# tpy001/VFMSeg

Hardware: AMD Instinct MI355X
Metric: train images/sec @512x512 DINOv2-L+LoRA (dg_lora_dinov2_ms_masked, 1024^2 sample = LR+HR 512^2 passes) (higher is better)
Workload: dtype bf16; 1 GPU; configs[1]: dg_lora_dinov2_ms_masked.py, synthetic 1024^2 19-class samples -> 2x512^2 passes, bs=2/GPU, full train step (fwd+bwd+allreduce+AdamW), LoRA dropout on; global_batch=2, parallelism=dp1

## Files before the change

include/vfmseg_hip.h:

```cpp
#ifndef VFMSEG_HIP_H
#define VFMSEG_HIP_H
#include <stdint.h>

#ifdef __cplusplus
extern "C" {
#endif

enum { VFM_F32 = 0, VFM_BF16 = 1, VFM_U8 = 2, VFM_I64 = 3,
       VFM_SPLIT3 = 4  };
enum { VFM_OK = 0, VFM_E_INVAL = -1, VFM_E_SHAPE = -2, VFM_E_ALIGN = -3, VFM_E_HIP = -4, VFM_E_UNSUPPORTED = -5 };
enum { VFM_EP_NONE = 0, VFM_EP_GELU = 1, VFM_EP_RELU = 2, VFM_EP_MUL_GELU_GRAD = 3, VFM_EP_MUL = 4,
       VFM_EP_QGELU = 5 , VFM_EP_MUL_QGELU_GRAD = 6,
       VFM_EP_GELU_DGELU = 7  };
enum { VFM_ACT_NONE = 0, VFM_ACT_GELU = 1, VFM_ACT_RELU = 2, VFM_ACT_QGELU = 3 };

const char* vfm_last_error(void);
int vfm_abi_version(void);
int vfm_half_kind(void);

int vfm_cast(const void* src, int src_dt, long ld_src, void* dst, int dst_dt, long ld_dst, long rows, long cols,
             const float* colscale, void* stream);
int vfm_split3(const float* src, long stride_r, long stride_c, void* dst, long ld_dst, long rows, long K, int pattern, void* stream);
int vfm_transpose(const void* src, int src_dt, long ld_src, void* dst, int dst_dt, long ld_dst, long rows, long cols,
                  long pad_rows, void* stream);
int vfm_strided_copy(const void* src, int src_dt, void* dst, int dst_dt, long n0, long n1, long n2, long n3, long s0,
                     long s1, long s2, long s3, long d0, long d1, long d2, long d3, int accumulate, void* stream);
typedef struct vfm_copy_job {
  const float* src; void* dst; long dst_dt; long accumulate;
  long n[4], s[4], d[4];
  long nsum, sum_stride;
} vfm_copy_job;
int vfm_strided_copy_batch(const vfm_copy_job* table_dev, int njobs, long max_elems, void* stream);
int vfm_axpby(const float* x, float a, float* y, float b, long n, void* stream);
int vfm_scale_by_device_scalar(float* y, const float* scalar, long n, void* stream);
int vfm_colsum(const void* x, int dt, long ld, long rows, long cols, float* out, int accumulate, float* ws, void* stream);
typedef struct vfm_lora_site {
  const float* A; const float* B;
  void* a; void* at; void* w; void* wt;
  long r, K, N, Kw, ld_a, ld_at, ld_w, ld_wt;
} vfm_lora_site;
int vfm_lora_pack(const vfm_lora_site* table_dev, int nsites, long max_elems, int dt, void* stream);
int vfm_slab_reduce(const float* slabs, int kch, long P, long Q, long rows_used, float alpha, float* dst, long sp, long sq,
                    int accumulate, void* stream);
int vfm_dropout_mask(void* out, int dt, long n, float p, uint64_t seed, uint64_t offset, void* stream);
int vfm_mul_mask(const void* src, int src_dt, long ld_src, const void* mask, int mask_dt, long mask_ld,
                 long rows_per_group, void* dst, int dst_dt, long ld_dst, long rows, long cols, void* stream);
int vfm_geglu_fwd(const void* h, int h_dt, long ld_h, void* out, int out_dt, long ld_out, long rows, long C, void* stream);
int vfm_geglu_bwd(const void* h, int h_dt, long ld_h, const void* dout, int do_dt, long ld_do, void* dh, int dh_dt,
                  long ld_dh, long rows, long C, void* stream);
int vfm_swiglu_fwd(const void* h, int h_dt, long ld_h, void* out, int out_dt, long ld_out, long rows, long C, void* stream);
int vfm_swiglu_bwd(const void* h, int h_dt, long ld_h, const void* dout, int do_dt, long ld_do, void* dh, int dh_dt,
                   long ld_dh, long rows, long C, void* stream);
int vfm_rope(void* x, int dt, long ld, long rows, int np, int ncols, int d, const float* cos_t, const float* sin_t,
             int inverse, void* stream);
int vfm_act_grad_mul(const void* dy, int dy_dt, long ld_dy, const void* pre, int pre_dt, long ld_pre, void* out, int out_dt,
                     long ld_out, long rows, long cols, int act, void* stream);
int vfm_mask_token_fwd(const float* x, const uint8_t* keep, const float* token, float* out, long rows, long C, void* stream);
int vfm_mask_token_bwd(const float* dout, const uint8_t* keep, float* dx, float* dtoken, float* ws ,
                       long rows, long C, void* stream);

int vfm_layernorm_fwd(const float* x, long ld_x, const float* w, const float* b, float eps, void* y, int y_dt, long ld_y,
                      float* stats, long rows, long C, void* stream);
int vfm_layernorm_fwd_split3(const float* x, long ld_x, const float* w, const float* b, float eps, float* y, long ld_y, void* y3, long ld3,
                             long plane, float* stats, long rows, long C, void* stream);
int vfm_layernorm_dropout_fwd(const float* x, long ld_x, const float* w, const float* b, float eps, void* y, long ld_y,
                              float* stats, void* y_drop, long ld_yd, void* mask, long ld_mask, float p, uint64_t seed,
                              uint64_t offset, long rows, long C, void* stream);
int vfm_layernorm_bwd_scaled(const void* dy, int dy_dt, long ld_dy, const float* x, long ld_x, const float* w,
                             const float* stats, float* dx, long ld_dx, int accumulate_dx, void* t_out, long ld_t,
                             const float* t_scale, long rows, long C, void* stream);
int vfm_layernorm_bwd(const void* dy, int dy_dt, long ld_dy, const float* x, long ld_x, const float* w,
                      const float* stats, float* dx, long ld_dx, int accumulate_dx, float* dw, float* db, float* ws,
                      long rows, long C, void* stream);
int vfm_groupnorm_fwd(const float* x, const float* w, const float* b, float eps, int G, int act, void* y, int y_dt,
                      float* stats, float* ws, long B, long P, long C, void* stream);
int vfm_groupnorm_bwd(const void* dy, int dy_dt, const float* x, const float* w, const float* b, const float* stats,
                      int G, int act, float* dx, float* dw, float* db, float* ws, long B, long P, long C, void* stream);
int vfm_bn_moments(const float* x, long rows, long C, float* sums, float* ws, void* stream);
int vfm_bn_finalize(const float* sums, float count, float* mean_var, float* running_mean, float* running_var,
                    float momentum, long C, void* stream);
int vfm_bn_apply(const float* x, const float* mean_var, const float* w, const float* b, float eps, int act, void* y,
                 int y_dt, long rows, long C, void* stream);
int vfm_bn_bwd_reduce(const void* dy, int dy_dt, const float* x, const float* mean_var, const float* w, const float* b,
                      float eps, int act, float* sums_dy, float* ws, long rows, long C, void* stream);
int vfm_bn_bwd_apply(const void* dy, int dy_dt, const float* x, const float* mean_var, const float* w, const float* b,
                     float eps, int act, const float* sums_dy, float total_rows, float* dx, long rows, long C,
                     void* stream);

typedef struct vfm_gemm_desc {
  const void* A; const void* B; void* C;
  int in_dt; int c_dt;
  long M, N, K;
  long sa_m, sa_k, sb_n, sb_k, ldc;
  float alpha;
  const float* bias; long bias_mod;
  const float* colscale;
  const void* residual; int r_dt; long ldr;
  int ep_mode; const void* aux; int aux_dt; long ld_aux;
  void* C2; int c2_dt; long ldc2;
  long batch, stride_a, stride_b, stride_c;
  long c_plane;
  long kb_rows;
} vfm_gemm_desc;
int vfm_gemm(const vfm_gemm_desc* d, void* stream);
int vfm_tune(const char* key, int value);

typedef struct vfm_attn_desc {
  const void* q; const void* k; const void* v; void* o;
  int dt; long ldq, ldk, ldv, ldo;
  int B, H, d;
  int nq_main, nq_extra, nk_main, nk_extra;
  float scale;
  float* lse;
  const void* dout; long ld_do;
  void* dq; void* dk; void* dv; long ld_dq, ld_dk, ld_dv;
  float* delta;
} vfm_attn_desc;
int vfm_attn_fwd(const vfm_attn_desc* d, void* stream);
int vfm_attn_bwd(const vfm_attn_desc* d, void* stream);
int vfm_attn_fwd_x3(const vfm_attn_desc* d, long lo_off, void* stream);
int vfm_attn_fwd_x3_split(const vfm_attn_desc* d, long lo_off, void* o3, long ld3, long plane, void* stream);
int vfm_attn_bwd_x3(const vfm_attn_desc* d, const void* q3, const void* k3, const void* v3, long ld3, long lo_off, const void* do3,
                    long ld_do3, long lo_off_do3, void* stream);

int vfm_sam_relpos_table(const float* rel_pos, int L, int d, int S, float* out, void* stream);
int vfm_sam_attn_prep(const void* qkv, int dt, long ld, const float* bias, const float* rh, const float* rw, void* q_aug,
                      void* k_aug, void* v_win, int nimg, int G, int S, int H, int d, int Dq, int NP,
                      int rows_per_batch , float scale, void* stream);
int vfm_softmax_rows(const float* scores, long ld_s, void* out, int out_dt, long ld_o, long rows, int n, int npad, void* stream);
int vfm_sam_attn_merge(const void* o_win, int dt, void* out, long ld, int nimg, int G, int S, int H, int d, int NP, void* stream);
int vfm_sam_attn_bwd_prep(const void* dao, long ld_dao, const void* qkv, long ld_qkv, const float* bias, int dt, void* dow,
                          void* dowT, void* vp, void* qsT, int nimg, int G, int S, int H, int d, int dp, int NP, float scale,
                          void* stream);
int vfm_softmax_rows_batched(const float* scores, long ld_s, void* out, int out_dt, long ld_o, long rows, int n, int npad,
                             int rows_per_batch, int valid_rows, void* stream);
int vfm_softmax_rows_bwd(const void* p, const float* dp, long ld_dp, void* ds, int dt, long ld_p, long rows, int n, int npad,
                         int rows_per_batch, int valid_rows, void* stream);
int vfm_sam_attn_bwd_merge(const void* dqa, const void* dkT, const void* dvT, int dt, const float* rh, const float* rw, void* dqkv,
                           long ld, int nimg, int G, int S, int H, int d, int dp, int NP, int Dq, float scale, void* stream);

int vfm_rein_mix_fwd(const float* x, long ld_x, const void* t, const void* vt, void* u, long ld_u, void* p, long ld_p, void* x16,
                     long ld_x16, long rows, int D, int m, float c, void* stream);
int vfm_rein_mix_bwd(const void* du, long ld_du, const void* p, long ld_p, const void* v, const void* tt, void* ds, long ld_ds,
                     float* dx, long ld_dx, long rows, int D, int m, float c, void* stream);

int vfm_sam_attn_flash_fwd(const void* qkv, long ld, const float* bias, const void* tbl_h, const void* tbl_w, void* out, long ldo,
                           int nimg, int G, int S, int H, int d, float scale, void* stream);
int vfm_sam_attn_flash_fwd_train(const void* qkv, long ld, const float* bias, const void* tbl_h, const void* tbl_w, void* out, long ldo,
                                 int nimg, int G, int S, int H, int d, float scale, float* lse, void* qext, void* stream);
long vfm_sam_attn_flash_stat_rows(int nimg, int G, int S, int H);
int vfm_sam_attn_flash_bwd(const void* qkv, long ld, const float* bias, const void* tbl_h, const void* tbl_w, const void* out,
                           const void* dout, long ldo, const float* lse, const void* qext, float* dsum, void* dqkv, long ldg,
                           int nimg, int G, int S, int H, int d, float scale, void* stream);

int vfm_patchify(const float* img, long stride_b, long stride_c, long stride_y, int y0, int x0, int h, int w, int P,
                 void* out, int out_dt, long ld_out, int B, void* stream);
int vfm_assemble_tokens(const float* patch_tok, const float* cls, const float* pos, float* x, int B, int np, int C,
                        void* stream);

int vfm_resize_bilinear(const void* in, int in_dt, int in_nchw, int B, int Hi, int Wi, int C, long in_ld_c, void* out,
                        int out_dt, int out_mode, long out_ld_c, int Hv, int Wv, int y0, int x0, int hc, int wc,
                        float scale_y, float scale_x, void* stream);
int vfm_resize_bicubic(const float* in, int Hi, int Wi, int C, float* out, int Ho, int Wo, float scale_y, float scale_x,
                       void* stream);
int vfm_label_resize(const int64_t* in, int B, int Hi, int Wi, int64_t* out, int Hv, int Wv, int y0, int x0, int hc,
                     int wc, void* stream);
int vfm_unblock(const float* x, float* y, int B, int H, int W, int C, int levels, int inverse, void* stream);
int vfm_upsample_ce(const float* logits_low, const int64_t* label, int B, int h, int w, int C, int H, int W,
                    int ignore_index, float* loss_parts, int32_t* counts, float* dlogits, void* stream);
int vfm_ce_finish(const float* loss_parts, long n, float scale, int32_t* counts, float eps, float* loss, float* acc, void* stream);
int vfm_reduce_sum(const float* x, long n, float scale, float* out, void* stream);

int vfm_preprocess_u8(const uint8_t* img, int H, int W, float* out, int Hp, int Wp, const float* mean3, const float* std3,
                      int bgr_to_rgb, float pad_val, void* stream);
int vfm_conf_gate(const float* logits, int B, int C, int H, int W, int y0, int x0, int hc, int wc, float thr,
                  int32_t* count, void* stream);
int vfm_slide_accumulate(const float* crop, int crop_nchw, int B, int h, int w, int C, float* preds, float* count,
                         int H, int W, int y0, int x0, int hc, int wc, void* stream);
typedef struct vfm_slide_win {
  const float* crop;
  int nchw, h, w;
  int y0, x0, hc, wc;
} vfm_slide_win;
int vfm_slide_gather(const vfm_slide_win* wins, int nwin, int B, int C, float* preds, int H, int W, void* stream);
int vfm_conf_gate_windows(const float* logits, int B, int C, int H, int W, const int* boxes, int nwin, float thr, int32_t* counts,
                          void* stream);
int vfm_slide_finalize(float* preds, const float* count, uint8_t* argmax, int B, int C, int H, int W, void* stream);

int vfm_confusion_hist(const uint8_t* pred, const void* label, int label_dt, long n, int num_classes, int ignore_index,
                       int64_t* hist, void* stream);

int vfm_adamw(float* p, float* g, float* m, float* v, long n, const long* seg_start, const float* seg_lr_mult,
              const float* seg_wd, int n_seg, float lr, float beta1, float beta2, float eps, int step, float grad_scale,
              int zero_grad, int vec4, void* stream);
int vfm_adamw_guarded(float* p, float* g, float* m, float* v, long n, const long* seg_start, const float* seg_lr_mult,
                      const float* seg_wd, int n_seg, float lr, float beta1, float beta2, float eps, int step, float grad_scale,
                      int zero_grad, int vec4, const int* skip, const float* amp_state, void* stream);
int vfm_amp_update(const int* flag, float* amp_state, float growth, float backoff, int interval, int dynamic, void* stream);

enum { VFM_OP_GEMM = 0, VFM_OP_LN_FWD = 1, VFM_OP_LN_DROPOUT_FWD = 2, VFM_OP_LN_BWD_SCALED = 3, VFM_OP_ATTN_FWD = 4, VFM_OP_ATTN_BWD = 5,
       VFM_OP_CAST = 6, VFM_OP_STRIDED_COPY = 7 };
enum { VFM_PROF_NONE = 0, VFM_PROF_GEMM = 1, VFM_PROF_GEMM_TN = 2, VFM_PROF_ATTN_FWD = 3, VFM_PROF_ATTN_BWD = 4 };
typedef struct vfm_plan_op {
  int kind;
  int prof_kind;
  double flops;
  union {
    vfm_gemm_desc gemm;
    vfm_attn_desc attn;
    struct { const float* x; long ld_x; const float* w; const float* b; float eps; void* y; int y_dt; long ld_y; float* stats;
             long rows, C; } ln_fwd;
    struct { const float* x; long ld_x; const float* w; const float* b; float eps; void* y; long ld_y; float* stats; void* y_drop;
             long ld_yd; void* mask; long ld_mask; float p; uint64_t offset; long rows, C; } ln_drop;
    struct { const void* dy; int dy_dt; long ld_dy; const float* x; long ld_x; const float* w; const float* stats; float* dx;
             long ld_dx; int accumulate_dx; void* t_out; long ld_t; const float* t_scale; long rows, C; } ln_bwd;
    struct { const void* src; int src_dt; long ld_src; void* dst; int dst_dt; long ld_dst; long rows, cols; const float* colscale; } cast;
    struct { const void* src; int src_dt; void* dst; int dst_dt; long n[4]; long ss[4]; long ds[4]; int accumulate; } copy;
  } u;
} vfm_plan_op;
int vfm_run_plan(const vfm_plan_op* ops, int n, uint64_t seed, uint64_t rng_base, void* stream);
int vfm_prof_config(int every);
int vfm_prof_read(double* out, int cap);

#ifdef __cplusplus
}
#endif
#endif
```

vfmseg_amd/backbones.py:

```python
import math

import os

import torch
import torch.nn as nn

from .precision import is_half
from . import ops
from .precision import compute_dtype
from .registry import MODELS

R_PAD = 64

BACKWARD_EVENTS = {"heads_done": None, "block_done": None, "backbone_done": None}
_PENDING_BACKWARD = [0]


class _Lin(nn.Module):
    def __init__(self, i, o, bias=True):
        super().__init__()
        self.in_features, self.out_features = i, o
        self.weight = nn.Parameter(torch.empty(o, i))
        self.bias = nn.Parameter(torch.zeros(o)) if bias else None
        nn.init.trunc_normal_(self.weight, std=0.02)
# ... 171 lines not shown
                raise NotImplementedError(f"init_cfg type {init_cfg.get('type')!r}: only dict(type='Pretrained', checkpoint=...) is read")
            self.load_pretrained_base(ck)

    def load_pretrained_base(self, checkpoint):
        sd = torch.load(checkpoint, map_location="cpu") if isinstance(checkpoint, (str, os.PathLike)) else checkpoint
        sd = sd.get("state_dict", sd) if isinstance(sd, dict) else sd
        missing, _ = self.load_state_dict(sd, strict=False)
        missing = [k for k in missing if not k.startswith("reins.")]
        if missing:
            raise RuntimeError(f"pretrained backbone {checkpoint if isinstance(checkpoint, (str, os.PathLike)) else '<state dict>'}: "
                               f"{len(missing)} base parameters not found (first: {missing[:3]}; the file holds e.g. {list(sd)[:3]})")
        self.pretrained = checkpoint if isinstance(checkpoint, (str, os.PathLike)) else "<state dict>"
        self.engine().invalidate()

    def train(self, mode=True):
        nn.Module.train(self, False)
        self._rein_train = bool(mode)
        if mode:
            for n, p in self.named_parameters():
                p.requires_grad = "reins" in n
            for p in self.reins.inert_params():
                p.requires_grad = False
            self.reins.train(True)
        return self

    def adapter_training(self):
        return self._rein_train

    def state_dict(self, *args, destination=None, prefix="", keep_vars=False):
        if args:
            args = list(args) + [None] * (3 - len(args))
            destination, prefix, keep_vars = args[0], args[1] or "", bool(args[2])
        state = super().state_dict(destination=destination, prefix=prefix, keep_vars=keep_vars)
        for k in [k for k in state.keys() if k.startswith(prefix) and "rein" not in k[len(prefix):]]:
            state.pop(k)
        return state

    def forward(self, x):
        xcat, (hp, wp) = self.forward_tokens([(x, None)], training=self._rein_train)
        b, d = x.shape[0], self.embed_dim
        v = xcat.view(b, hp, wp, len(self.out_indices), d)
        return tuple(v[:, :, :, i].permute(0, 3, 1, 2) for i in range(len(self.out_indices)))


class _Holder(nn.Module):
    def __init__(self, m):
        super().__init__()
        self.model = m


class _PeftModel(nn.Module):
    def __init__(self, m):
        super().__init__()
        self.base_model = _Holder(m)


@MODELS.register_module()
class LoRABackbone(nn.Module):

    def __init__(self, backbone, checkpoint=None, Lora_config=None, init_cfg=None, **kw):
        super().__init__()
        vit = MODELS.build(backbone)
        cfg = Lora_config or {}
        self.lora_targets = list(cfg.get("target_modules", ["qkv"]))
        for name, mod in list(vit.named_modules()):
            if isinstance(mod, _Lin) and any(name == t or name.endswith("." + t) for t in self.lora_targets):
                parent = vit
                parts = name.split(".")
                for p_ in parts[:-1]:
                    parent = getattr(parent, p_)
                setattr(parent, parts[-1], LoraLinear(mod, cfg.get("r", 32), cfg.get("lora_alpha", 32), cfg.get("lora_dropout", 0.0)))
        if not vit.engine().lora_on():
            raise NotImplementedError(f"target_modules={self.lora_targets}: no adapter site the {type(vit).__name__} HIP engine fuses")
        self.model = _PeftModel(vit)
        self._lora_train = False
        if checkpoint is not None:
            self.load_pretrained_backbone(checkpoint, self.lora_targets)
        self.train(True)

    @property
    def vit(self):
        return self.model.base_model.model

    def load_pretrained_backbone(self, checkpoint, target_modules):
        sd = torch.load(checkpoint, map_location="cpu") if isinstance(checkpoint, str) else checkpoint
        new = {}
        for name, w in sd.items():
            for t in target_modules:
                if t in name:
                    name = name.replace(t, t + ".base_layer")
            new[name] = w
        self.vit.load_state_dict(new, strict=False)
        self.vit.engine().invalidate()

    def train(self, mode=True):
        super().train(False)
        self._lora_train = bool(mode)
        for n, p in self.named_parameters():
            p.requires_grad = ("lora" in n) if mode else p.requires_grad
        if mode:
            for p in getattr(self.vit.engine(), "inert_params", lambda: [])():
                p.requires_grad = False
        return self

    def forward_tokens(self, jobs, seed=None):
        return self.vit.forward_tokens(jobs, training=self._lora_train, seed=seed)

    def forward(self, x):
        xcat, (hp, wp) = self.forward_tokens([(x, None)])
        b, d, nt = x.shape[0], self.vit.embed_dim, len(self.vit.out_indices)
        v = xcat.view(b, hp, wp, nt, d)
        return tuple(v[:, :, :, i].permute(0, 3, 1, 2) for i in range(nt))


class Packed:

    def __init__(self, w_f32, cd, k_pad=None):
        n, k = w_f32.shape
        k_pad = k_pad or k
        self.n, self.k = n, k_pad
        self.w = ops.empty_ld(n, k_pad, cd, w_f32.device, zero=True)
        ops.cast(w_f32, self.w[:, :k])
        self.wt = None
        if is_half(cd):
            self.wt = ops.empty_ld(k_pad, n, cd, w_f32.device, zero=True)
            ops.transpose(w_f32, self.wt[:k], pad_rows=n)

    def fwd(self, a, out, **epi):
        return ops.gemm(a, self.w, out, **epi)

    def dgrad(self, dy, out, **epi):
        if self.wt is not None:
            return ops.gemm(dy, self.wt, out, **epi)
        return ops.gemm(dy, self.w, out, trans_b=True, **epi)


def wgrad(dy, x, grad_out, alpha=1.0, n_rows=None, accumulate=True):
    M = dy.shape[0]
    res = grad_out if accumulate else None
    if is_half(dy.dtype):
        mp = (M + 63) // 64 * 64
        dyt = torch.empty(dy.shape[1], mp, dtype=dy.dtype, device=dy.device)
        xt = torch.empty(x.shape[1], mp, dtype=x.dtype, device=x.device)
        ops.transpose(dy, dyt, pad_rows=mp)
        ops.transpose(x, xt, pad_rows=mp)
        ops.gemm(dyt, xt, grad_out, alpha=alpha, residual=res)
    else:
        ops.gemm(dy, x, grad_out, alpha=alpha, residual=res, trans_a=True, trans_b=True)
    return grad_out


class _DinoTrainPlan:

    def __init__(self, eng, P, nimg, Np):
        v = eng.vit
        cd, dev = P["cd"], P["dev"]
        D, H = v.embed_dim, v.num_heads
        nL = len(v.blocks)
        M, Mp = nimg * Np + nimg, nimg * Np
        Lp0 = P["layers"][0]
        kq, hid = Lp0["qkv"].k, Lp0["fc1"].n
        q0 = v.blocks[0].attn.qkv
        self.eng, self.P, self.nimg, self.Np, self.M, self.Mp, self.nL, self.D, self.H = eng, P, nimg, Np, M, Mp, nL, D, H
        self.busy = False
        e = lambda *sh, dt=cd: torch.empty(*sh, dtype=dt, device=dev)
        f32 = torch.float32
        self.X = e(nL + 1, M, D, dt=f32)
        self.A1, self.XD, self.MASK = e(nL, M, kq), e(nL, M, D), e(nL, M, D)
        self.ST1, self.ST2 = e(nL, M, 2, dt=f32), e(nL, M, 2, dt=f32)
        self.QKV, self.AO = e(nL, M, 3 * D), e(nL, M, D)
        self.LSE = e(nL, nimg, H, Np + 1, dt=f32)
        self.XMID, self.A2 = e(nL, M, D, dt=f32), e(nL, M, D)
        hld = hid + ops.ld_pad(hid, cd)
        self.HPRE = e(nL, M, hld)[:, :, :hid]
        self.G = e(M, hld)[:, :hid]
        self.hid, self.kq = hid, kq
        hd = D // H
        scale = hd ** -0.5
        f = self.fwd = ops.Plan("backbone")
        self.tap_ops = []
        self.nt = len(v.out_indices)
        xcat0 = e(Mp, self.nt * D)
        for li, (blk, Lp) in enumerate(zip(v.blocks, P["layers"])):
            q = blk.attn.qkv
            x, a1 = self.X[li], self.A1[li]
            f.layernorm_dropout_fwd(x, Lp["n1w"], Lp["n1b"], 1e-6, a1[:, :D], self.ST1[li], self.XD[li], self.MASK[li], q.p, li * M * D)
            f.gemm(self.XD[li], Lp["a"], a1[:, D:D + R_PAD], alpha=q.scaling)
            f.gemm(a1, Lp["qkv"].w, self.QKV[li], bias=Lp["qkv_b"])
            qkv = self.QKV[li]
            f.attn_fwd(qkv[:, :D], qkv[:, D:2 * D], qkv[:, 2 * D:], self.AO[li], self.LSE[li], nimg, H, hd, Np, 1, Np, 1, scale)
            f.gemm(self.AO[li], Lp["proj"].w, self.XMID[li], bias=Lp["proj_b"], colscale=Lp["g1"], residual=x)
            f.layernorm_fwd(self.XMID[li], Lp["n2w"], Lp["n2b"], 1e-6, self.A2[li], self.ST2[li])
            f.gemm(self.A2[li], Lp["fc1"].w, self.G, bias=Lp["fc1_b"], ep_mode=ops.EP_GELU_DGELU, c2=self.HPRE[li])
            f.gemm(self.G, Lp["fc2"].w, self.X[li + 1], bias=Lp["fc2_b"], colscale=Lp["g2"], residual=self.XMID[li])
            for i, oi in enumerate(v.out_indices):
                if oi == li:
                    self.tap_ops.append((f.cast(self.X[li + 1][:Mp], xcat0[:, i * D:(i + 1) * D]), i * D))
        self.bwd = None

    def eligible_backward(self):
        from .functional import direct_grad_target
        v = self.eng.vit
        return (os.environ.get("VFMSEG_LORA_WGRAD_BATCHED", "1") != "0" and
                all(direct_grad_target(b.attn.qkv.lora_A["default"].weight) is not None and
                    direct_grad_target(b.attn.qkv.lora_B["default"].weight) is not None for b in v.blocks))

    def run_forward(self, xcat, seed, rng0):
        esz = xcat.element_size()
        for idx, col in self.tap_ops:
            self.fwd.entry(idx).u.cast.dst = xcat.data_ptr() + col * esz
        self.fwd.run(seed, rng0)

    def _build_backward(self, dxcat):
        v, P = self.eng.vit, self.P
        cd, dev = P["cd"], P["dev"]
        D, H, nL, M, Mp, nimg, Np = self.D, self.H, self.nL, self.M, self.Mp, self.nimg, self.Np
        hd = D // H
        scale = hd ** -0.5
        e = lambda *sh, dt=cd: torch.empty(*sh, dtype=dt, device=dev)
        self.DX = e(M, D, dt=torch.float32)
        self.T, self.DN, self.DAO = e(M, D), e(M, D), e(M, D)
        self.DH = e(M, self.hid + ops.ld_pad(self.hid, cd))[:, :self.hid]
        self.DQKV, self.DA1 = e(nL, M, 3 * D), e(nL, M, self.kq)
        half = nL // 2
        skip_l0 = os.environ.get("VFMSEG_PLAN_SKIP_L0", "1") != "0"
        self.half = half
        self.dx_sig = (tuple(dxcat.shape), tuple(dxcat.stride()), dxcat.dtype)
        plans, self.tap_src = [], []

        def add_tap(pl, pn, li):
            for i, oi in enumerate(v.out_indices):
                if oi == li:
                    src = dxcat[:, i * D:(i + 1) * D]
                    self.tap_src.append((pn, pl.strided_copy(src, self.DX, (Mp, D), (src.stride(0), 1), (D, 1), accumulate=True), i * D))

        for pn, (hi, lo) in enumerate(((nL, half), (half, 0)) if half > 0 else ((nL, 0),)):
            pl = ops.Plan("backbone")
            for li in range(hi - 1, lo - 1, -1):
                blk, Lp = v.blocks[li], P["layers"][li]
                q = blk.attn.qkv
                if li == nL - 1:
                    add_tap(pl, pn, li)
                    pl.cast(self.DX, self.T, Lp["g2"])
                pl.gemm(self.T, Lp["fc2"].wt, self.DH, ep_mode=ops.EP_MUL, aux=self.HPRE[li])
                pl.gemm(self.DH, Lp["fc1"].wt, self.DN)
                pl.layernorm_bwd_scaled(self.DN, self.XMID[li], Lp["n2w"], self.ST2[li], self.DX, self.T, Lp["g1"], accumulate_dx=True)
                pl.gemm(self.T, Lp["proj"].wt, self.DAO)
                qkv, dqkv, da1 = self.QKV[li], self.DQKV[li], self.DA1[li]
                pl.attn_bwd(qkv[:, :D], qkv[:, D:2 * D], qkv[:, 2 * D:], self.AO[li], self.LSE[li], self.DAO, dqkv[:, :D], dqkv[:, D:2 * D],
                            dqkv[:, 2 * D:], nimg, H, hd, Np, 1, Np, 1, scale)
                if li == 0 and skip_l0:
                    pl.gemm(dqkv, Lp["qkv"].wt[D:D + R_PAD], da1[:, D:D + R_PAD])
                    continue
                pl.gemm(dqkv, Lp["qkv"].wt, da1)
                pl.gemm(da1[:, D:D + R_PAD], Lp["at"], da1[:, :D], alpha=q.scaling, residual=da1[:, :D], ep_mode=ops.EP_MUL, aux=self.MASK[li])
                if li > 0:
                    add_tap(pl, pn, li - 1)
                    pl.layernorm_bwd_scaled(da1[:, :D], self.X[li], Lp["n1w"], self.ST1[li], self.DX, self.T, P["layers"][li - 1]["g2"],
                                            accumulate_dx=True)
                else:
                    pl.layernorm_bwd_scaled(da1[:, :D], self.X[li], Lp["n1w"], self.ST1[li], self.DX, self.T, Lp["g2"], accumulate_dx=True)
            plans.append((pl, lo, hi))
        self.bwd = plans

    def run_backward(self, ctx, dxcat):
        sig = (tuple(dxcat.shape), tuple(dxcat.stride()), dxcat.dtype)
        if self.bwd is None or self.dx_sig != sig:
            self._build_backward(dxcat)
        esz = dxcat.element_size()
        for pn, idx, col in self.tap_src:
            self.bwd[pn][0].entry(idx).u.copy.src = dxcat.data_ptr() + col * esz
        self.DX.zero_()
        for pl, lo, hi in self.bwd:
            pl.run()
            self.eng._lora_wgrads_batched(self.P, ctx, self.DA1, self.DQKV, lo, hi, self.M, self.D)
            if BACKWARD_EVENTS["block_done"] is not None:
                for lj in range(hi - 1, lo - 1, -1):
                    BACKWARD_EVENTS["block_done"](lj)


class DinoEngine:
    def __init__(self, vit):
        self.vit = vit
        self._packed = None
        self._pos_cache = {}

    def invalidate(self):
        self._packed = None
        self._pos_cache = {}

    def lora_on(self):
        return isinstance(self.vit.blocks[0].attn.qkv, LoraLinear)

    def rein_on(self):
        return getattr(self.vit, "reins", None) is not None

    def trainable(self):
        out = []
        if self.lora_on():
            for blk in self.vit.blocks:
                out += [blk.attn.qkv.lora_A["default"].weight, blk.attn.qkv.lora_B["default"].weight]
        if self.rein_on():
            out += self.vit.reins.live_params()
        return out

    def packed(self):
        cd = compute_dtype()
        dev = self.vit.pos_embed.device
        if self._packed is not None and self._packed["cd"] == cd and self._packed["dev"] == dev:
            return self._packed
        v = self.vit
        D = v.embed_dim
        P = dict(cd=cd, dev=dev, layers=[])
        with torch.no_grad():
            pw = v.patch_embed.proj.weight.detach().reshape(D, -1)
            P["pe"] = Packed(pw, cd)
            P["pe_b"] = v.patch_embed.proj.bias.detach().float().contiguous()
            P["cls"] = v.cls_token.detach().reshape(D).float().contiguous()
            for blk in v.blocks:
                qkv = blk.attn.qkv
                base = qkv.base_layer if isinstance(qkv, LoraLinear) else qkv
                kq = D + (R_PAD if isinstance(qkv, LoraLinear) else 0)
                Lp = dict(
                    qkv=Packed(base.weight.detach(), cd, k_pad=kq),
                    qkv_b=base.bias.detach().float().contiguous() if base.bias is not None else None,
                    proj=Packed(blk.attn.proj.weight.detach(), cd),
                    proj_b=blk.attn.proj.bias.detach().float().contiguous() if blk.attn.proj.bias is not None else None,
                    fc1=Packed(blk.mlp.fc1.weight.detach(), cd),
                    fc1_b=blk.mlp.fc1.bias.detach().float().contiguous() if blk.mlp.fc1.bias is not None else None,
                    fc2=Packed(blk.mlp.fc2.weight.detach(), cd),
                    fc2_b=blk.mlp.fc2.bias.detach().float().contiguous() if blk.mlp.fc2.bias is not None else None,
                    g1=blk.ls1.gamma.detach().float().contiguous(), g2=blk.ls2.gamma.detach().float().contiguous(),
                    n1w=blk.norm1.weight.detach().float().contiguous(), n1b=blk.norm1.bias.detach().float().contiguous(),
                    n2w=blk.norm2.weight.detach().float().contiguous(), n2b=blk.norm2.bias.detach().float().contiguous(),
                )
                if isinstance(qkv, LoraLinear):
                    Lp["a"] = torch.zeros(R_PAD, D, dtype=cd, device=dev)
                    Lp["at"] = torch.zeros(D, R_PAD, dtype=cd, device=dev)
                P["layers"].append(Lp)
        self._packed = P
        return P

    def refresh_lora(self, P):
        D = self.vit.embed_dim
        sites = []
        for blk, Lp in zip(self.vit.blocks, P["layers"]):
            q = blk.attn.qkv
            if isinstance(q, LoraLinear):
                A, Bm = q.lora_A["default"].weight.detach(), q.lora_B["default"].weight.detach()
                sites.append((A, Bm, Lp["a"], Lp["at"], Lp["qkv"].w, Lp["qkv"].wt, q.r, A.shape[1], Bm.shape[0], D))
        _refresh_sites(P, sites)

    def merged_qkv(self, P):
        from .optim import PARAM_EPOCH
        key = [PARAM_EPOCH[0]]
        for blk in self.vit.blocks:
            q = blk.attn.qkv
            A, Bm = q.lora_A["default"].weight, q.lora_B["default"].weight
            key += [A._version, Bm._version, A.data_ptr(), Bm.data_ptr()]
        key = tuple(key)
        if P.get("merged_key") == key:
            return P["merged"]
        D, cd, dev = self.vit.embed_dim, P["cd"], P["dev"]
        merged = []
        with torch.no_grad():
            for blk in self.vit.blocks:
                q = blk.attn.qkv
                A, Bm = q.lora_A["default"].weight.detach().float(), q.lora_B["default"].weight.detach().float()
                w = q.base_layer.weight.detach().float()
                weff = torch.empty_like(w)
                ops.gemm(Bm.contiguous(), A.contiguous(), weff, alpha=q.scaling, residual=w, trans_b=True)
                wp = ops.empty_ld(w.shape[0], D, cd, dev)
                ops.cast(weff, wp)
                merged.append(wp)
        P["merged"], P["merged_key"] = merged, key
        return merged

    def pos_tokens(self, hp, wp):
        v = self.vit
        n = v.pos_embed.shape[1] - 1
        s = int(math.sqrt(n))
        if hp == s and wp == s:
            return v.pos_embed.detach().reshape(n + 1, -1).float().contiguous()
        key = (hp, wp)
        if key not in self._pos_cache:
            D = v.embed_dim
            pe = v.pos_embed.detach().reshape(n + 1, D).float().contiguous()
            out = torch.empty(1 + hp * wp, D, dtype=torch.float32, device=pe.device)
            ops.cast(pe[:1], out[:1])
            sy, sx = s / (hp + 0.1), s / (wp + 0.1)
            assert int(s * ((hp + 0.1) / s)) == hp and int(s * ((wp + 0.1) / s)) == wp
            ops.resize_bicubic(pe[1:], s, s, D, out[1:], hp, wp, sy, sx)
            self._pos_cache[key] = out
        return self._pos_cache[key]

    def forward(self, jobs, training, seed, need_grad=False):
        v, P = self.vit, self.packed()
        cd = P["cd"]
        dev = P["dev"]
        D, H, ps = v.embed_dim, v.num_heads, v.patch_size
        lora = self.lora_on()
        rein = self._rein_pack(P) if self.rein_on() else None
        merged = None
        from .precision import split3 as _x3_mode
        x3 = _x3_mode() and not is_half(cd)
        if (lora and not training and not torch.is_grad_enabled() and (is_half(cd) or x3)
                and os.environ.get("VFMSEG_MERGE_LORA_EVAL", "1") != "0"):
            merged = self.merged_qkv(P)
        elif lora:
            self.refresh_lora(P)
        sizes = []
        for img, box in jobs:
            y0, y1, x0, x1 = box if box is not None else (0, img.shape[2], 0, img.shape[3])
            sizes.append(((y1 - y0) // ps, (x1 - x0) // ps))
        hp, wp = sizes[0]
        assert all(s == (hp, wp) for s in sizes), "all jobs of one backbone call must share the token grid"
        Np = hp * wp
        nimg = sum(j[0].shape[0] for j in jobs)
        Mp, M = nimg * Np, nimg * Np + nimg
        kpe = 3 * ps * ps
        A0 = torch.empty(Mp, kpe, dtype=cd, device=dev)
        r0 = 0
        for img, box in jobs:
            b = img.shape[0]
            ops.patchify(img, A0[r0 * Np:(r0 + b) * Np], box=box, patch=ps)
            r0 += b
        ptok = torch.empty(Mp, D, dtype=torch.float32, device=dev)
        P["pe"].fwd(A0, ptok, bias=P["pe_b"])
        plan = self._train_plan(P, nimg, Np, training, merged) if need_grad else None
        x = plan.X[0] if plan is not None else torch.empty(M, D, dtype=torch.float32, device=dev)
        ops.assemble_tokens(ptok, P["cls"], self.pos_tokens(hp, wp), x, nimg, Np, D)
        del ptok, A0
        nt = len(v.out_indices)
        from .precision import eval_heads_fp32
        tap_dt = torch.float32 if (not training and not need_grad and eval_heads_fp32()) else cd
        xcat = torch.empty(Mp, nt * D, dtype=tap_dt, device=dev)
        saved = []
        if lora and training:
            from .functional import draw_seed
            seed, rng0 = draw_seed(seed, len(v.blocks) * M * D)
        else:
            seed, rng0 = 0, 0
        if plan is not None:
            plan.run_forward(xcat, seed, rng0)
            plan.busy = True
            ctx = dict(saved=None, plan=plan, nimg=nimg, Np=Np, M=M, Mp=Mp, P=P, training=training, A1all=plan.A1, XDall=plan.XD)
            return xcat, (hp, wp), ctx
        nL = len(v.blocks)
        batched = lora and training and is_half(cd) and merged is None
        A1all = torch.empty(nL, M, P["layers"][0]["qkv"].k, dtype=cd, device=dev) if batched else None
        XDall = None
        hd = D // H
        scale = hd ** -0.5
        for li, (blk, Lp) in enumerate(zip(v.blocks, P["layers"])):
            S = {"x_in": x}
            kq = D if merged is not None else Lp["qkv"].k
            a1 = A1all[li] if batched else torch.empty(M, kq, dtype=cd, device=dev)
            st1 = torch.empty(M, 2, dtype=torch.float32, device=dev)
            q = blk.attn.qkv if lora else None
            fused_drop = lora and training and q.p > 0 and is_half(cd) and D % 256 == 0
            if fused_drop:
                mask = torch.empty(M, D, dtype=cd, device=dev)
                if batched and XDall is None:
                    XDall = torch.empty(nL, M, D, dtype=cd, device=dev)
                xd = XDall[li] if batched else torch.empty(M, D, dtype=cd, device=dev)
                ops.layernorm_dropout_fwd(x, Lp["n1w"], Lp["n1b"], 1e-6, a1[:, :D], st1, xd, mask, q.p, seed, offset=rng0 + li * M * D)
            else:
                so = "only" if (x3 and not training and not need_grad and kq == D) else None
                ops.layernorm_fwd(x, Lp["n1w"], Lp["n1b"], 1e-6, a1 if kq == D else a1[:, :D], st1, split_out=so)
            if lora and merged is None:
                if not fused_drop:
                    xd, mask = a1[:, :D], None
                    if training and q.p > 0:
                        mask = torch.empty(M, D, dtype=cd, device=dev)
                        ops.dropout_mask(mask, q.p, seed, offset=rng0 + li * M * D)
                        xd = torch.empty(M, D, dtype=cd, device=dev)
                        ops.mul_mask(a1[:, :D], mask, xd)
                ops.gemm(xd, Lp["a"], a1[:, D:D + R_PAD], alpha=q.scaling)
                S.update(xd=xd if mask is not None else None, mask=mask)
            qkv = torch.empty(M, 3 * D, dtype=cd, device=dev)
            if merged is not None:
                ops.gemm(a1, merged[li], qkv, bias=Lp["qkv_b"])
            else:
                Lp["qkv"].fwd(a1, qkv, bias=Lp["qkv_b"])
            ao = torch.empty(M, D, dtype=cd, device=dev)
            lse = torch.empty(nimg, H, Np + 1, dtype=torch.float32, device=dev)
            so = "only" if (x3 and not training and not need_grad) else None
            ops.attn_fwd(qkv[:, :D], qkv[:, D:2 * D], qkv[:, 2 * D:], ao, lse, nimg, H, hd, Np, 1, Np, 1, scale, keep_split=training, o_split=so)
            xm = torch.empty(M, D, dtype=torch.float32, device=dev)
            Lp["proj"].fwd(ao, xm, bias=Lp["proj_b"], colscale=Lp["g1"], residual=x)
            a2 = torch.empty(M, D, dtype=cd, device=dev)
            st2 = torch.empty(M, 2, dtype=torch.float32, device=dev)
            ops.layernorm_fwd(xm, Lp["n2w"], Lp["n2b"], 1e-6, a2, st2, split_out=so)
            hid = Lp["fc1"].n
            g = ops.empty_ld(M, hid, cd, dev)
            if training and (lora or (rein is not None and need_grad)):
                hpre = torch.empty(M, hid, dtype=cd, device=dev)
                Lp["fc1"].fwd(a2, g, bias=Lp["fc1_b"], ep_mode=ops.EP_GELU_DGELU, c2=hpre)
            else:
                hpre = None
                Lp["fc1"].fwd(a2, g, bias=Lp["fc1_b"], ep_mode=ops.EP_GELU, **({"c_split": so} if so else {}))
            xo = torch.empty(M, D, dtype=torch.float32, device=dev)
            Lp["fc2"].fwd(g, xo, bias=Lp["fc2_b"], colscale=Lp["g2"], residual=xm)
            S.update(a1=a1, st1=st1, qkv=qkv, ao=ao, lse=lse, x_mid=xm, a2=a2, st2=st2, hpre=hpre, g=g)
            saved.append(S)
            x = xo
            if rein is not None:
                x = self._rein_forward(rein, li, x, Mp, S if (training and need_grad) else None)
            for i, oi in enumerate(v.out_indices):
                if oi == li:
                    ops.cast(x[:Mp], xcat[:, i * D:(i + 1) * D])
        ctx = dict(saved=saved, nimg=nimg, Np=Np, M=M, Mp=Mp, P=P, training=training, A1all=A1all, XDall=XDall, rein=rein)
        return xcat, (hp, wp), ctx

    def _train_plan(self, P, nimg, Np, training, merged):
        v = self.vit
        if (not training or merged is not None or not self.lora_on() or self.rein_on() or not is_half(P["cd"])
                or os.environ.get("VFMSEG_PLAN", "1") == "0" or v.embed_dim % 256 != 0):
            return None
        q0 = v.blocks[0].attn.qkv
        if not all(isinstance(b.attn.qkv, LoraLinear) and b.attn.qkv.p > 0 and b.attn.qkv.p == q0.p and b.attn.qkv.scaling == q0.scaling
                   for b in v.blocks):
            return None
        plans = P.setdefault("plans", {})
        pl = plans.get((nimg, Np))
        if pl is None:
            pl = plans[(nimg, Np)] = _DinoTrainPlan(self, P, nimg, Np)
        if pl.busy or not pl.eligible_backward():
            return None
        return pl

    def backward(self, ctx, dxcat):
        if ctx.get("plan") is not None:
            plan = ctx["plan"]
            try:
                plan.run_backward(ctx, dxcat)
            finally:
                plan.busy = False
            return [None] * (2 * len(self.vit.blocks))
        v, P = self.vit, ctx["P"]
        cd, dev = P["cd"], P["dev"]
        D, H = v.embed_dim, v.num_heads
        hd = D // H
        scale = hd ** -0.5
        M, Mp, nimg, Np = ctx["M"], ctx["Mp"], ctx["nimg"], ctx["Np"]
        dx = torch.zeros(M, D, dtype=torch.float32, device=dev)
        grads = [None] * (2 * len(v.blocks) if self.lora_on() else 0)
        nL = len(v.blocks)
        rein = ctx.get("rein")
        rein_acc = self._rein_backward_begin(rein) if rein is not None else None
        from .functional import direct_grad_target
        wg_batched = (ctx.get("A1all") is not None and self.lora_on() and os.environ.get("VFMSEG_LORA_WGRAD_BATCHED", "1") != "0" and
                      all(direct_grad_target(b.attn.qkv.lora_A["default"].weight) is not None and
                          direct_grad_target(b.attn.qkv.lora_B["default"].weight) is not None for b in v.blocks) and
                      (ctx.get("XDall") is not None or all(S_["mask"] is None for S_ in ctx["saved"])))
        if wg_batched:
            kq_all = ctx["A1all"].shape[2]
            DA1all = torch.empty(nL, M, kq_all, dtype=cd, device=dev)
            DQKVall = torch.empty(nL, M, 3 * D, dtype=cd, device=dev)
        half = nL // 2
        fuse_t = is_half(cd) and D % 256 == 0
        fuse_t1 = fuse_t and rein is None
        def add_tap(li):
            for i, oi in enumerate(v.out_indices):
                if oi == li:
                    src = dxcat[:, i * D:(i + 1) * D]
                    ops.strided_copy(src, dx, (Mp, D), (src.stride(0), 1), (D, 1), accumulate=True)
        t = None
        for li in range(len(v.blocks) - 1, -1, -1):
            blk, Lp, S = v.blocks[li], P["layers"][li], ctx["saved"][li]
            q = blk.attn.qkv
            if t is None:
                add_tap(li)
                if rein is not None:
                    self._rein_backward(rein, rein_acc, li, dx, Mp, S)
                t = torch.empty(M, D, dtype=cd, device=dev)
                ops.cast(dx, t, Lp["g2"])
            hid = Lp["fc1"].n
            dh = ops.empty_ld(M, hid, cd, dev)
            Lp["fc2"].dgrad(t, dh, ep_mode=ops.EP_MUL, aux=S["hpre"])
            dn = torch.empty(M, D, dtype=cd, device=dev)
            Lp["fc1"].dgrad(dh, dn)
            if fuse_t:
                ops.layernorm_bwd_scaled(dn, S["x_mid"], Lp["n2w"], S["st2"], dx, t, Lp["g1"], accumulate_dx=True)
            else:
                ops.layernorm_bwd(dn, S["x_mid"], Lp["n2w"], S["st2"], dx, accumulate_dx=True)
                ops.cast(dx, t, Lp["g1"])
            del dh
            dao = torch.empty(M, D, dtype=cd, device=dev)
            Lp["proj"].dgrad(t, dao)
            dqkv = DQKVall[li] if wg_batched else torch.empty(M, 3 * D, dtype=cd, device=dev)
            qkv = S["qkv"]
            ops.attn_bwd(qkv[:, :D], qkv[:, D:2 * D], qkv[:, 2 * D:], S["ao"], S["lse"], dao, dqkv[:, :D], dqkv[:, D:2 * D],
                         dqkv[:, 2 * D:], nimg, H, hd, Np, 1, Np, 1, scale)
            kq = Lp["qkv"].k
            da1 = DA1all[li] if wg_batched else torch.empty(M, kq, dtype=cd, device=dev)
            Lp["qkv"].dgrad(dqkv, da1)
            if isinstance(q, LoraLinear) and wg_batched:
                ep = dict(ep_mode=ops.EP_MUL, aux=S["mask"]) if S["mask"] is not None else {}
                ops.gemm(da1[:, D:D + R_PAD], Lp["at"], da1[:, :D], alpha=q.scaling, residual=da1[:, :D], **ep)
            elif isinstance(q, LoraLinear):
                r = q.r
                A, Bm = q.lora_A["default"].weight, q.lora_B["default"].weight
                a1 = S["a1"]
                xd = S["xd"] if S["xd"] is not None else a1[:, :D]
                from .functional import direct_grad_target
                tB, tA = direct_grad_target(Bm), direct_grad_target(A)
                gBt = torch.empty(R_PAD, Bm.shape[0], dtype=torch.float32, device=dev)
                gAp = torch.empty(R_PAD, A.shape[1], dtype=torch.float32, device=dev)
                doneB = _wgrad_small_t(a1[:, D:D + R_PAD], dqkv, gBt, scatter=None if tB is None else (tB, r, 1, r))
                doneA = _wgrad_small_t(da1[:, D:D + R_PAD], xd, gAp, alpha=q.scaling,
                                       scatter=None if tA is None else (tA, r, A.shape[1], 1))
                if doneB is True:
                    pass
                elif tB is not None:
                    ops.strided_copy(gBt, tB, (Bm.shape[0], r), (1, gBt.stride(0)), (r, 1), accumulate=True)
                else:
                    gB = torch.empty_like(Bm, dtype=torch.float32)
                    ops.strided_copy(gBt, gB, (Bm.shape[0], r), (1, gBt.stride(0)), (r, 1))
                    grads[2 * li + 1] = gB
                if doneA is True:
                    pass
                elif tA is not None:
                    ops.axpby(gAp[:r].reshape(-1), 1.0, tA.view(-1), 1.0)
                else:
                    grads[2 * li] = gAp[:r]
                ep = dict(ep_mode=ops.EP_MUL, aux=S["mask"]) if S["mask"] is not None else {}
                ops.gemm(da1[:, D:D + R_PAD], Lp["at"], da1[:, :D], alpha=q.scaling, residual=da1[:, :D], **ep)
            if fuse_t1 and li > 0:
                add_tap(li - 1)
                ops.layernorm_bwd_scaled(da1[:, :D], S["x_in"], Lp["n1w"], S["st1"], dx, t, P["layers"][li - 1]["g2"],
                                         accumulate_dx=True)
            else:
                ops.layernorm_bwd(da1[:, :D], S["x_in"], Lp["n1w"], S["st1"], dx, accumulate_dx=True)
                t = None
            ctx["saved"][li] = None
            if wg_batched:
                if li == half or li == 0:
                    lo, hi = (half, nL) if li == half and half > 0 else (0, half if half > 0 else nL)
                    self._lora_wgrads_batched(P, ctx, DA1all, DQKVall, lo, hi, M, D)
                    if BACKWARD_EVENTS["block_done"] is not None:
                        for lj in range(hi - 1, lo - 1, -1):
                            BACKWARD_EVENTS["block_done"](lj)
            elif BACKWARD_EVENTS["block_done"] is not None:
                BACKWARD_EVENTS["block_done"](li)
        if rein is not None:
            grads += self._rein_backward_end(rein, rein_acc)
        return grads

    def _rein_fused(self, P):
        r = self.vit.reins
        return (is_half(P["cd"]) and os.environ.get("VFMSEG_REIN_FUSED", "0") == "1" and self.vit.embed_dim % 256 == 0
                and r.token_length <= ops.REIN_TOK)

    def _rein_pack(self, P):
        from .optim import PARAM_EPOCH
        r = self.vit.reins
        cd, dev = P["cd"], P["dev"]
        D, nL, m = self.vit.embed_dim, r.num_layers, r.token_length
        live = r.live_params()
        key = (PARAM_EPOCH[0], self._rein_fused(P)) + tuple(x for p_ in live for x in (p_._version, p_.data_ptr()))
        R = P.get("rein")
        if R is not None and R["key"] == key:
            return R
        TP = (max(m, ops.REIN_TOK) + 63) // 64 * 64
        if R is None or R["TP"] != TP:
            z = lambda *sh, dt=cd: torch.zeros(*sh, dtype=dt, device=dev)
            R = P["rein"] = dict(TP=TP, T32=z(nL, TP, D, dt=torch.float32), T=z(nL, TP, D), V=z(nL, TP, D), TT=None, VT=None,
                                 scalevec=torch.empty(D, dtype=torch.float32, device=dev))
        R["key"], R["m"], R["c"], R["fused"] = key, m, float(D) ** -0.5, self._rein_fused(P)
        with torch.no_grad():
            T32 = R["T32"]
            toks = [p_.detach() for p_ in r.token_params()]
            if len(toks) == 2:
                ops.gemm(toks[0], toks[1], T32[:, :m], trans_b=True)
            else:
                ops.strided_copy(toks[0], T32, (nL, m, D), (m * D, D, 1), (TP * D, D, 1))
            if cd != torch.float32:
                ops.cast(T32.view(nL * TP, D), R["T"].view(nL * TP, D))
            else:
                R["T"] = T32
            Wt, Wd = r.mlp_token2feat, r.mlp_delta_f
            R["wt"], R["wd"] = Packed(Wt.weight.detach(), cd), Packed(Wd.weight.detach(), cd)
            R["bt"], R["bd"] = Wt.bias.detach(), Wd.bias.detach()
            vtmp = torch.empty(nL * TP, D, dtype=torch.float32, device=dev)
            R["wt"].fwd(R["T"].view(nL * TP, D), vtmp, bias=R["bt"])
            vt3 = vtmp.view(nL, TP, D)
            ops.strided_copy(vt3[:, 1:m], R["V"][:, 1:m], (nL, m - 1, D), (TP * D, D, 1), (TP * D, D, 1))
            if R["fused"]:
                if R["TT"] is None:
                    R["TT"], R["VT"] = torch.zeros(nL, D, TP, dtype=cd, device=dev), torch.zeros(nL, D, TP, dtype=cd, device=dev)
                ops.strided_copy(T32, R["TT"], (nL, D, m), (TP * D, 1, D), (D * TP, TP, 1))
                ops.strided_copy(vt3[:, 1:m], R["VT"][:, :, 1:m], (nL, D, m - 1), (TP * D, 1, D), (D * TP, TP, 1))
            ops.strided_copy(r.scale.detach().reshape(1), R["scalevec"], (D,), (0,), (1,))
        return R

    def _rein_forward(self, R, li, x, Mp, S):
        cd, dev = R["T"].dtype, x.device
        D, m, TP = x.shape[1], R["m"], R["TP"]
        xp = x[:Mp]
        u = torch.empty(Mp, D, dtype=cd, device=dev)
        p = torch.empty(Mp, TP, dtype=cd, device=dev) if S is not None else None
        x16 = None
        if R["fused"]:
            x16 = torch.empty(Mp, D, dtype=cd, device=dev) if S is not None else None
            ops.rein_mix_fwd(xp, R["T"][li], R["VT"][li], u, m, R["c"], p=p, x16=x16)
        else:
            if cd != torch.float32:
                x16 = torch.empty(Mp, D, dtype=cd, device=dev)
                ops.cast(xp, x16)
            sc = torch.empty(Mp, TP, dtype=torch.float32, device=dev)
            ops.gemm(x16 if x16 is not None else xp, R["T"][li], sc, alpha=R["c"])
            if p is None:
                p = torch.empty(Mp, TP, dtype=cd, device=dev)
            ops.softmax_rows(sc, p, m)
            ops.gemm(p, R["V"][li], u, residual=xp, trans_b=True)
        if S is None:
            xn = x
        else:
            xn = torch.empty_like(x)
            ops.cast(x[Mp:], xn[Mp:])
            S.update(rein_u=u, rein_p=p, rein_x=x16 if x16 is not None else xp)
        R["wd"].fwd(u, xn[:Mp], bias=R["bd"], colscale=R["scalevec"], residual=xp)
        return xn

    def _rein_backward_begin(self, R):
        dev = R["T"].device
        nL, TP, D = R["T"].shape
        z = lambda *sh: torch.zeros(*sh, dtype=torch.float32, device=dev)
        return dict(dT=z(nL, TP, D), dV=z(nL, TP, D), Gm=z(D, D), gb=z(D))

    @staticmethod
    def _tn(xs, y, out, alpha=1.0, accumulate=False):
        if is_half(xs.dtype):
            ops.gemm_tn_batched(xs.unsqueeze(0), y.unsqueeze(0), out.unsqueeze(0), xs.shape[0], alpha=alpha, accumulate=accumulate)
        else:
            ops.gemm(xs, y, out, alpha=alpha, residual=out if accumulate else None, trans_a=True, trans_b=True)

    def _rein_backward(self, R, acc, li, dx, Mp, S):
        cd, dev = R["T"].dtype, dx.device
        D, m, TP, c = dx.shape[1], R["m"], R["TP"], R["c"]
        u, p, xs = S["rein_u"], S["rein_p"], S["rein_x"]
        g = torch.empty(Mp, D, dtype=cd, device=dev)
        ops.cast(dx[:Mp], g)
        self._tn(g, u, acc["Gm"], accumulate=True)
        ops.colsum(g, acc["gb"], accumulate=True)
        du = torch.empty(Mp, D, dtype=cd, device=dev)
        R["wd"].dgrad(g, du, colscale=R["scalevec"])
        ds = torch.empty(Mp, TP, dtype=cd, device=dev)
        if R["fused"]:
            ops.rein_mix_bwd(du, p, R["V"][li], R["TT"][li], ds, dx[:Mp], m, c)
            a = 1.0
        else:
            dp = torch.empty(Mp, TP, dtype=torch.float32, device=dev)
            ops.gemm(du, R["V"][li], dp)
            ops.softmax_rows_bwd(p, dp, ds, m, 1, 1)
            ops.gemm(ds, R["T"][li], dx[:Mp], alpha=c, residual=dx[:Mp], trans_b=True)
            ops.strided_copy(du, dx[:Mp], (Mp, D), (du.stride(0), 1), (dx.stride(0), 1), accumulate=True)
            a = c
        self._tn(ds, xs, acc["dT"][li], alpha=a)
        self._tn(p, du, acc["dV"][li])
        S["rein_u"] = S["rein_p"] = S["rein_x"] = None

    def _rein_backward_end(self, R, acc):
        from .functional import direct_grad_target
        r = self.vit.reins
        cd, dev = R["T"].dtype, R["T"].device
        nL, TP, D = R["T"].shape
        m = R["m"]
        z = lambda *sh, dt=torch.float32: torch.zeros(*sh, dtype=dt, device=dev)
        dvz = z(nL, TP, D, dt=cd)
        ops.strided_copy(acc["dV"][:, 1:m], dvz[:, 1:m], (nL, m - 1, D), (TP * D, D, 1), (TP * D, D, 1))
        dvz2, T2 = dvz.view(nL * TP, D), R["T"].view(nL * TP, D)
        gWt, gbt = z(D, D), z(D)
        self._tn(dvz2, T2, gWt)
        ops.colsum(dvz2, gbt)
        back = torch.empty(nL * TP, D, dtype=torch.float32, device=dev)
        R["wt"].dgrad(dvz2, back)
        dT = acc["dT"]
        ops.strided_copy(back.view(nL, TP, D)[:, 1:m], dT[:, 1:m], (nL, m - 1, D), (TP * D, D, 1), (TP * D, D, 1), accumulate=True)
        toks = r.token_params()
        if len(toks) == 2:
# ... 168 lines not shown
```

vfmseg_amd/csrc/elementwise.hip:

```cpp
#include "common.h"

thread_local char g_vfm_err[512] = {0};

extern "C" const char* vfm_last_error(void) { return g_vfm_err; }
extern "C" int vfm_abi_version(void) { return 4; }
extern "C" int vfm_half_kind(void) { return VFM_HALF_KIND; }

template <typename TI, typename TO>
__global__ void k_cast(const TI* __restrict__ src, long ld_src, TO* __restrict__ dst, long ld_dst, long rows, long cols,
                       const float* __restrict__ colscale) {
  const long cols4 = cols >> 2;
  const long total = rows * cols4;
  for (long i = blockIdx.x * (long)blockDim.x + threadIdx.x; i < total; i += (long)gridDim.x * blockDim.x) {
    const long r = i / cols4, c = (i - r * cols4) << 2;
    float v[4];
#pragma unroll
    for (int j = 0; j < 4; ++j) v[j] = ld_f32(src + r * ld_src + c + j);
    if (colscale) {
#pragma unroll
      for (int j = 0; j < 4; ++j) v[j] *= colscale[c + j];
    }
#pragma unroll
    for (int j = 0; j < 4; ++j) st_f32(dst + r * ld_dst + c + j, v[j]);
  }
  const long tail0 = cols4 << 2;
  const long ntail = cols - tail0;
  if (ntail) {
    for (long i = blockIdx.x * (long)blockDim.x + threadIdx.x; i < rows * ntail; i += (long)gridDim.x * blockDim.x) {
      const long r = i / ntail, c = tail0 + (i - r * ntail);
      float v = ld_f32(src + r * ld_src + c);
      if (colscale) v *= colscale[c];
      st_f32(dst + r * ld_dst + c, v);
    }
  }
}

extern "C" int vfm_cast(const void* src, int src_dt, long ld_src, void* dst, int dst_dt, long ld_dst, long rows, long cols,
                        const float* colscale, void* stream) {
  VFM_CHECK(rows >= 0 && cols >= 0 && ld_src >= cols && ld_dst >= cols, VFM_E_SHAPE, "vfm_cast: bad shape");
  if (rows == 0 || cols == 0) return VFM_OK;
  hipStream_t s = (hipStream_t)stream;
  const long total = rows * ((cols + 3) / 4);
  const int grid = (int)((total + 255) / 256 > 4096 ? 4096 : (total + 255) / 256);
#define L(TI, TO) hipLaunchKernelGGL((k_cast<TI, TO>), dim3(grid), dim3(256), 0, s, (const TI*)src, ld_src, (TO*)dst, ld_dst, rows, cols, colscale)
  if (src_dt == VFM_F32 && dst_dt == VFM_F32) L(float, float);
  else if (src_dt == VFM_F32 && dst_dt == VFM_BF16) L(float, bf16_t);
  else if (src_dt == VFM_BF16 && dst_dt == VFM_F32) L(bf16_t, float);
  else if (src_dt == VFM_BF16 && dst_dt == VFM_BF16) L(bf16_t, bf16_t);
  else VFM_FAIL(VFM_E_INVAL, "vfm_cast: dtype");
#undef L
  VFM_LAUNCH_CHECK();
  return VFM_OK;
}

__global__ void k_split3(const float* __restrict__ src, long sr, long sc, bf16_t* __restrict__ dst, long ld_dst, long rows, long K, long Kp,
                         int pattern) {
  const long per_row = Kp / 4;
  const long total = rows * per_row;
  for (long i = (long)blockIdx.x * blockDim.x + threadIdx.x; i < total; i += (long)gridDim.x * blockDim.x) {
    const long r = i / per_row, c = (i % per_row) * 4;
    float v[4];
    if (sc == 1 && c + 3 < K && ((reinterpret_cast<uintptr_t>(src + r * sr + c) & 15) == 0)) {
      const float4 f = *reinterpret_cast<const float4*>(src + r * sr + c);
      v[0] = f.x, v[1] = f.y, v[2] = f.z, v[3] = f.w;
    } else {
#pragma unroll
      for (int e = 0; e < 4; ++e) v[e] = (c + e < K) ? src[r * sr + (c + e) * sc] : 0.f;
    }
    ushort4 hi, lo;
    bf16_t* ph = &hi.x;
    bf16_t* pl = &lo.x;
#pragma unroll
    for (int e = 0; e < 4; ++e) {
      ph[e] = f32_to_bf16(v[e]);
      pl[e] = f32_to_bf16(v[e] - bf16_to_f32(ph[e]));
    }
    bf16_t* d = dst + r * ld_dst + c;
    *reinterpret_cast<ushort4*>(d) = hi;
    *reinterpret_cast<ushort4*>(d + Kp) = pattern == 0 ? hi : lo;
    *reinterpret_cast<ushort4*>(d + 2 * Kp) = pattern == 0 ? lo : hi;
  }
}

extern "C" int vfm_split3(const float* src, long stride_r, long stride_c, void* dst, long ld_dst, long rows, long K, int pattern, void* stream) {
  const long Kp = (K + 63) / 64 * 64;
  VFM_CHECK(rows >= 0 && K > 0 && ld_dst >= 3 * Kp && ld_dst % 4 == 0 && ((uintptr_t)dst % 8) == 0 && (pattern == 0 || pattern == 1), VFM_E_SHAPE,
            "vfm_split3: dst must hold rows x 3 ceil64(K) bf16 (ld %% 4 == 0, 8-byte aligned)");
  if (rows == 0) return VFM_OK;
  const long total = rows * (Kp / 4);
  const int grid = (int)((total + 255) / 256 > 8192 ? 8192 : (total + 255) / 256);
  hipLaunchKernelGGL(k_split3, dim3(grid), dim3(256), 0, (hipStream_t)stream, src, stride_r, stride_c, (bf16_t*)dst, ld_dst, rows, K, Kp, pattern);
  VFM_LAUNCH_CHECK();
  return VFM_OK;
}

template <typename TI, typename TO>
__global__ void k_transpose(const TI* __restrict__ src, long ld_src, TO* __restrict__ dst, long ld_dst, long rows, long cols,
                            long pad_rows) {
  __shared__ float tile[64][65];
  const long r0 = (long)blockIdx.y * 64, c0 = (long)blockIdx.x * 64;
  const int tx = threadIdx.x & 63, ty = threadIdx.x >> 6;
  for (int i = ty; i < 64; i += 4) {
    const long r = r0 + i, c = c0 + tx;
    tile[i][tx] = (r < rows && c < cols) ? ld_f32(src + r * ld_src + c) : 0.f;
  }
  __syncthreads();
  for (int i = ty; i < 64; i += 4) {
    const long c = c0 + i, r = r0 + tx;
    if (c < cols && r < pad_rows) st_f32(dst + c * ld_dst + r, tile[tx][i]);
  }
}

extern "C" int vfm_transpose(const void* src, int src_dt, long ld_src, void* dst, int dst_dt, long ld_dst, long rows, long cols,
                             long pad_rows, void* stream) {
  VFM_CHECK(pad_rows >= rows && ld_dst >= pad_rows && ld_src >= cols, VFM_E_SHAPE, "vfm_transpose: bad shape");
  if (cols == 0 || pad_rows == 0) return VFM_OK;
  hipStream_t s = (hipStream_t)stream;
  dim3 grid(cdiv(cols, 64), cdiv(pad_rows, 64));
#define L(TI, TO) hipLaunchKernelGGL((k_transpose<TI, TO>), grid, dim3(256), 0, s, (const TI*)src, ld_src, (TO*)dst, ld_dst, rows, cols, pad_rows)
  if (src_dt == VFM_F32 && dst_dt == VFM_F32) L(float, float);
  else if (src_dt == VFM_F32 && dst_dt == VFM_BF16) L(float, bf16_t);
  else if (src_dt == VFM_BF16 && dst_dt == VFM_F32) L(bf16_t, float);
  else if (src_dt == VFM_BF16 && dst_dt == VFM_BF16) L(bf16_t, bf16_t);
  else VFM_FAIL(VFM_E_INVAL, "vfm_transpose: dtype");
#undef L
  VFM_LAUNCH_CHECK();
  return VFM_OK;
}

template <typename TI, typename TO>
__global__ void k_strided_copy(const TI* __restrict__ src, TO* __restrict__ dst, long n0, long n1, long n2, long n3, long s0,
                               long s1, long s2, long s3, long d0, long d1, long d2, long d3, int accumulate) {
  const long total = n0 * n1 * n2 * n3;
  for (long i = blockIdx.x * (long)blockDim.x + threadIdx.x; i < total; i += (long)gridDim.x * blockDim.x) {
    long t = i;
    const long i3 = t % n3; t /= n3;
    const long i2 = t % n2; t /= n2;
    const long i1 = t % n1; t /= n1;
    const float v = ld_f32(src + t * s0 + i1 * s1 + i2 * s2 + i3 * s3);
    TO* q = dst + t * d0 + i1 * d1 + i2 * d2 + i3 * d3;
    st_f32(q, accumulate ? ld_f32(q) + v : v);
  }
}

extern "C" int vfm_strided_copy(const void* src, int src_dt, void* dst, int dst_dt, long n0, long n1, long n2, long n3,
                                long s0, long s1, long s2, long s3, long d0, long d1, long d2, long d3, int accumulate,
                                void* stream) {
  const long total = n0 * n1 * n2 * n3;
  if (total == 0) return VFM_OK;
  hipStream_t s = (hipStream_t)stream;
  const int grid = (int)((total + 255) / 256 > 4096 ? 4096 : (total + 255) / 256);
#define L(TI, TO) hipLaunchKernelGGL((k_strided_copy<TI, TO>), dim3(grid), dim3(256), 0, s, (const TI*)src, (TO*)dst, n0, n1, n2, n3, s0, s1, s2, s3, d0, d1, d2, d3, accumulate)
  if (src_dt == VFM_F32 && dst_dt == VFM_F32) L(float, float);
  else if (src_dt == VFM_F32 && dst_dt == VFM_BF16) L(float, bf16_t);
  else if (src_dt == VFM_BF16 && dst_dt == VFM_F32) L(bf16_t, float);
  else if (src_dt == VFM_BF16 && dst_dt == VFM_BF16) L(bf16_t, bf16_t);
  else VFM_FAIL(VFM_E_INVAL, "vfm_strided_copy: dtype");
#undef L
// ... 680 lines not shown
```

vfmseg_amd/csrc/norm.hip:

```cpp
#include "common.h"

__device__ __forceinline__ float act_f(float v, int act) {
  return act == VFM_ACT_GELU ? gelu_f(v) : (act == VFM_ACT_RELU ? fmaxf(v, 0.f) : v);
}
__device__ __forceinline__ float act_grad_f(float v, int act) {
  return act == VFM_ACT_GELU ? gelu_grad_f(v) : (act == VFM_ACT_RELU ? (v > 0.f ? 1.f : 0.f) : 1.f);
}

template <typename TO, int MAXPL>
__global__ void k_ln_fwd(const float* __restrict__ x, long ld_x, const float* __restrict__ w, const float* __restrict__ b,
                         float eps, TO* __restrict__ y, long ld_y, float* __restrict__ stats, long rows, int C) {
  const int lane = threadIdx.x & 63;
  const long row = (long)blockIdx.x * (blockDim.x >> 6) + (threadIdx.x >> 6);
  if (row >= rows) return;
  const float* xr = x + row * ld_x;
  float v[MAXPL];
  float s = 0.f;
#pragma unroll
  for (int i = 0; i < MAXPL; ++i) {
    const int c = i * 64 + lane;
    v[i] = c < C ? xr[c] : 0.f;
    s += v[i];
  }
  const float mean = wave_sum(s) / C;
  float q = 0.f;
#pragma unroll
  for (int i = 0; i < MAXPL; ++i) {
    const int c = i * 64 + lane;
    const float d = c < C ? v[i] - mean : 0.f;
    q += d * d;
  }
  const float rstd = rsqrtf(wave_sum(q) / C + eps);
  if (stats && lane == 0) {
    stats[row * 2] = mean;
    stats[row * 2 + 1] = rstd;
  }
#pragma unroll
  for (int i = 0; i < MAXPL; ++i) {
    const int c = i * 64 + lane;
    if (c < C) st_f32(y + row * ld_y + c, (v[i] - mean) * rstd * w[c] + b[c]);
  }
}


struct LnDrop {
  void* yd; long ld_yd; void* mask; long ld_mask; float p, keep_scale; uint64_t seed, offset;
};
struct Split3Out {
  bf16_t* y3; long ld3; long plane;
};
__device__ __forceinline__ void store_split4(const Split3Out& so, long row, int c0, float4 o) {
  const bf16_t h0 = f32_to_bf16(o.x), h1 = f32_to_bf16(o.y), h2 = f32_to_bf16(o.z), h3 = f32_to_bf16(o.w);
  const ushort4 hi = {h0, h1, h2, h3};
  const ushort4 lo = {f32_to_bf16(o.x - bf16_to_f32(h0)), f32_to_bf16(o.y - bf16_to_f32(h1)), f32_to_bf16(o.z - bf16_to_f32(h2)),
                      f32_to_bf16(o.w - bf16_to_f32(h3))};
  bf16_t* p = so.y3 + row * so.ld3 + c0;
  *reinterpret_cast<ushort4*>(p) = hi;
  *reinterpret_cast<ushort4*>(p + so.plane) = hi;
  *reinterpret_cast<ushort4*>(p + 2 * so.plane) = lo;
}
template <typename TO, int NV, bool DROP = false, bool SPLIT = false>
__global__ void k_ln_fwd_v4(const float* __restrict__ x, long ld_x, const float* __restrict__ w, const float* __restrict__ b,
                            float eps, TO* __restrict__ y, long ld_y, float* __restrict__ stats, long rows, int C, LnDrop dr = LnDrop(),
                            Split3Out so = Split3Out()) {
  const int lane = threadIdx.x & 63;
  const long row = (long)blockIdx.x * (blockDim.x >> 6) + (threadIdx.x >> 6);
  if (row >= rows) return;
  const float* xr = x + row * ld_x;
  float4 v[NV];
  float s = 0.f;
#pragma unroll
  for (int i = 0; i < NV; ++i) {
    v[i] = *reinterpret_cast<const float4*>(xr + (i * 64 + lane) * 4);
    s += (v[i].x + v[i].y) + (v[i].z + v[i].w);
  }
  const float mean = wave_sum(s) / C;
  float q = 0.f;
#pragma unroll
  for (int i = 0; i < NV; ++i) {
    const float a = v[i].x - mean, bb = v[i].y - mean, c = v[i].z - mean, d = v[i].w - mean;
    q += (a * a + bb * bb) + (c * c + d * d);
  }
  const float rstd = rsqrtf(wave_sum(q) / C + eps);
  if (stats && lane == 0) {
    stats[row * 2] = mean;
    stats[row * 2 + 1] = rstd;
  }
#pragma unroll
  for (int i = 0; i < NV; ++i) {
    const int c0 = (i * 64 + lane) * 4;
    const float4 ww = *reinterpret_cast<const float4*>(w + c0);
    const float4 bv = *reinterpret_cast<const float4*>(b + c0);
    float4 o;
    o.x = (v[i].x - mean) * rstd * ww.x + bv.x;
    o.y = (v[i].y - mean) * rstd * ww.y + bv.y;
    o.z = (v[i].z - mean) * rstd * ww.z + bv.z;
    o.w = (v[i].w - mean) * rstd * ww.w + bv.w;
    if constexpr (sizeof(TO) == 2) {
      ushort4 p = {f32_to_bf16(o.x), f32_to_bf16(o.y), f32_to_bf16(o.z), f32_to_bf16(o.w)};
      *reinterpret_cast<ushort4*>(y + row * ld_y + c0) = p;
      if constexpr (DROP) {
        const uint64_t e0 = dr.offset + (uint64_t)row * C + c0;
        const bf16_t ks = f32_to_bf16(dr.keep_scale);
        const float ksf = bf16_to_f32(ks);
        ushort4 mk, yd;
        const bool k0 = (hash_u32(dr.seed, e0) >> 8) * (1.0f / 16777216.0f) >= dr.p;
        const bool k1 = (hash_u32(dr.seed, e0 + 1) >> 8) * (1.0f / 16777216.0f) >= dr.p;
        const bool k2 = (hash_u32(dr.seed, e0 + 2) >> 8) * (1.0f / 16777216.0f) >= dr.p;
        const bool k3 = (hash_u32(dr.seed, e0 + 3) >> 8) * (1.0f / 16777216.0f) >= dr.p;
        mk.x = k0 ? ks : 0, mk.y = k1 ? ks : 0, mk.z = k2 ? ks : 0, mk.w = k3 ? ks : 0;
        yd.x = k0 ? f32_to_bf16(bf16_to_f32(p.x) * ksf) : f32_to_bf16(bf16_to_f32(p.x) * 0.f);
        yd.y = k1 ? f32_to_bf16(bf16_to_f32(p.y) * ksf) : f32_to_bf16(bf16_to_f32(p.y) * 0.f);
        yd.z = k2 ? f32_to_bf16(bf16_to_f32(p.z) * ksf) : f32_to_bf16(bf16_to_f32(p.z) * 0.f);
        yd.w = k3 ? f32_to_bf16(bf16_to_f32(p.w) * ksf) : f32_to_bf16(bf16_to_f32(p.w) * 0.f);
        *reinterpret_cast<ushort4*>((bf16_t*)dr.mask + row * dr.ld_mask + c0) = mk;
        *reinterpret_cast<ushort4*>((bf16_t*)dr.yd + row * dr.ld_yd + c0) = yd;
      }
    } else {
      if (!SPLIT || y != nullptr) *reinterpret_cast<float4*>(y + row * ld_y + c0) = o;
      if constexpr (SPLIT) store_split4(so, row, c0, o);
    }
  }
}

template <typename TD, int NV>
__global__ void k_ln_bwd_v4(const TD* __restrict__ dy, long ld_dy, const float* __restrict__ x, long ld_x,
                            const float* __restrict__ w, const float* __restrict__ stats, float* __restrict__ dx, long ld_dx,
                            int accumulate_dx, long rows, int C, bf16_t* __restrict__ t_out = nullptr, long ld_t = 0,
                            const float* __restrict__ t_scale = nullptr) {
  const int lane = threadIdx.x & 63;
  const long row = (long)blockIdx.x * (blockDim.x >> 6) + (threadIdx.x >> 6);
  if (row >= rows) return;
  const float mean = stats[row * 2], rstd = stats[row * 2 + 1];
  float4 g[NV], xh[NV];
  float s1 = 0.f, s2 = 0.f;
#pragma unroll
  for (int i = 0; i < NV; ++i) {
    const int c0 = (i * 64 + lane) * 4;
    float4 d;
    if constexpr (sizeof(TD) == 2) {
      const ushort4 p = *reinterpret_cast<const ushort4*>(dy + row * ld_dy + c0);
      d = make_float4(bf16_to_f32(p.x), bf16_to_f32(p.y), bf16_to_f32(p.z), bf16_to_f32(p.w));
    } else {
      d = *reinterpret_cast<const float4*>(dy + row * ld_dy + c0);
    }
    const float4 xv = *reinterpret_cast<const float4*>(x + row * ld_x + c0);
    const float4 ww = *reinterpret_cast<const float4*>(w + c0);
    xh[i] = make_float4((xv.x - mean) * rstd, (xv.y - mean) * rstd, (xv.z - mean) * rstd, (xv.w - mean) * rstd);
    g[i] = make_float4(d.x * ww.x, d.y * ww.y, d.z * ww.z, d.w * ww.w);
    s1 += (g[i].x + g[i].y) + (g[i].z + g[i].w);
    s2 += (g[i].x * xh[i].x + g[i].y * xh[i].y) + (g[i].z * xh[i].z + g[i].w * xh[i].w);
  }
  s1 = wave_sum(s1) / C;
  s2 = wave_sum(s2) / C;
#pragma unroll
  for (int i = 0; i < NV; ++i) {
    const int c0 = (i * 64 + lane) * 4;
    float4 o = make_float4(rstd * (g[i].x - s1 - xh[i].x * s2), rstd * (g[i].y - s1 - xh[i].y * s2),
                           rstd * (g[i].z - s1 - xh[i].z * s2), rstd * (g[i].w - s1 - xh[i].w * s2));
    float4* p = reinterpret_cast<float4*>(dx + row * ld_dx + c0);
    if (accumulate_dx) {
      const float4 old = *p;
      o.x += old.x, o.y += old.y, o.z += old.z, o.w += old.w;
    }
    *p = o;
    if (t_out) {
      const float4 ts = *reinterpret_cast<const float4*>(t_scale + c0);
      const ushort4 tv = {f32_to_bf16(o.x * ts.x), f32_to_bf16(o.y * ts.y), f32_to_bf16(o.z * ts.z), f32_to_bf16(o.w * ts.w)};
      *reinterpret_cast<ushort4*>(t_out + row * ld_t + c0) = tv;
    }
  }
}

template <typename TO, int MAXP2>
__global__ void k_ln_fwd_v2(const float* __restrict__ x, long ld_x, const float* __restrict__ w, const float* __restrict__ b, float eps,
                            TO* __restrict__ y, long ld_y, float* __restrict__ stats, long rows, int C) {
  const int lane = threadIdx.x & 63;
  const long row = (long)blockIdx.x * (blockDim.x >> 6) + (threadIdx.x >> 6);
  if (row >= rows) return;
  const float* xr = x + row * ld_x;
  float2 v[MAXP2];
  float s = 0.f;
#pragma unroll
  for (int i = 0; i < MAXP2; ++i) {
    const int c = (i * 64 + lane) * 2;
    v[i] = c < C ? *reinterpret_cast<const float2*>(xr + c) : make_float2(0.f, 0.f);
    s += v[i].x + v[i].y;
  }
  const float mean = wave_sum(s) / C;
  float q = 0.f;
#pragma unroll
  for (int i = 0; i < MAXP2; ++i) {
    const int c = (i * 64 + lane) * 2;
    if (c < C) {
      const float a = v[i].x - mean, bb = v[i].y - mean;
      q += a * a + bb * bb;
    }
  }
  const float rstd = rsqrtf(wave_sum(q) / C + eps);
  if (stats && lane == 0) {
    stats[row * 2] = mean;
    stats[row * 2 + 1] = rstd;
  }
#pragma unroll
  for (int i = 0; i < MAXP2; ++i) {
    const int c = (i * 64 + lane) * 2;
    if (c < C) {
      const float2 ww = *reinterpret_cast<const float2*>(w + c), bv = *reinterpret_cast<const float2*>(b + c);
      const float o0 = (v[i].x - mean) * rstd * ww.x + bv.x, o1 = (v[i].y - mean) * rstd * ww.y + bv.y;
      if constexpr (sizeof(TO) == 2) {
        const ushort2 pk = {f32_to_bf16(o0), f32_to_bf16(o1)};
        *reinterpret_cast<ushort2*>(y + row * ld_y + c) = pk;
      } else {
        *reinterpret_cast<float2*>(y + row * ld_y + c) = make_float2(o0, o1);
      }
    }
  }
}

template <typename TO, int MAXP4>
__global__ void k_ln_fwd_v4t(const float* __restrict__ x, long ld_x, const float* __restrict__ w, const float* __restrict__ b, float eps,
                             TO* __restrict__ y, long ld_y, float* __restrict__ stats, long rows, int C) {
  const int lane = threadIdx.x & 63;
  const long row = (long)blockIdx.x * (blockDim.x >> 6) + (threadIdx.x >> 6);
  if (row >= rows) return;
  const float* xr = x + row * ld_x;
  float v[MAXP4][4];
  float s = 0.f;
#pragma unroll
  for (int i = 0; i < MAXP4; ++i) {
    const int c = (i * 64 + lane) * 4;
    const float4 t = c < C ? *reinterpret_cast<const float4*>(xr + c) : make_float4(0.f, 0.f, 0.f, 0.f);
    v[i][0] = t.x, v[i][1] = t.y, v[i][2] = t.z, v[i][3] = t.w;
#pragma unroll
    for (int e = 0; e < 4; ++e)
      if (c + e < C) s += v[i][e];
  }
  const float mean = wave_sum(s) / C;
  float q = 0.f;
#pragma unroll
  for (int i = 0; i < MAXP4; ++i) {
    const int c = (i * 64 + lane) * 4;
#pragma unroll
    for (int e = 0; e < 4; ++e)
      if (c + e < C) q += (v[i][e] - mean) * (v[i][e] - mean);
  }
  const float rstd = rsqrtf(wave_sum(q) / C + eps);
  if (stats && lane == 0) {
    stats[row * 2] = mean;
    stats[row * 2 + 1] = rstd;
  }
#pragma unroll
  for (int i = 0; i < MAXP4; ++i) {
    const int c = (i * 64 + lane) * 4;
    if (c < C) {
      if (c + 4 <= C) {
        const float4 ww = *reinterpret_cast<const float4*>(w + c), bv = *reinterpret_cast<const float4*>(b + c);
        const float o0 = (v[i][0] - mean) * rstd * ww.x + bv.x, o1 = (v[i][1] - mean) * rstd * ww.y + bv.y;
        const float o2 = (v[i][2] - mean) * rstd * ww.z + bv.z, o3 = (v[i][3] - mean) * rstd * ww.w + bv.w;
        if constexpr (sizeof(TO) == 2) {
          const ushort4 pk = {f32_to_bf16(o0), f32_to_bf16(o1), f32_to_bf16(o2), f32_to_bf16(o3)};
          *reinterpret_cast<ushort4*>(y + row * ld_y + c) = pk;
        } else {
          *reinterpret_cast<float4*>(y + row * ld_y + c) = make_float4(o0, o1, o2, o3);
        }
      } else {
#pragma unroll
        for (int e = 0; e < 4; ++e)
          if (c + e < C) {
            const float o = (v[i][e] - mean) * rstd * w[c + e] + b[c + e];
            if constexpr (sizeof(TO) == 2) y[row * ld_y + c + e] = f32_to_bf16(o);
            else y[row * ld_y + c + e] = o;
          }
      }
    }
  }
}

extern "C" int vfm_layernorm_fwd_split3(const float* x, long ld_x, const float* w, const float* b, float eps, float* y, long ld_y, void* y3,
                                        long ld3, long plane, float* stats, long rows, long C, void* stream) {
  const int nv = (int)(C / 256);
  VFM_CHECK(C > 0 && C % 256 == 0 && (nv == 1 || nv == 2 || nv == 4 || nv == 5 || nv == 8) && ld_x >= C && ld_x % 4 == 0 && (uintptr_t)x % 16 == 0 &&
                (uintptr_t)w % 16 == 0 && (uintptr_t)b % 16 == 0,
            VFM_E_SHAPE, "vfm_layernorm_fwd_split3: C=%ld must be 256, 512, 1024, 1280 or 2048 with 16-byte aligned rows", C);
  VFM_CHECK(y3 && (uintptr_t)y3 % 8 == 0 && plane >= C && plane % 4 == 0 && ld3 >= 3 * plane && ld3 % 4 == 0 && (!y || (ld_y >= C && ld_y % 4 == 0 && (uintptr_t)y % 16 == 0)),
            VFM_E_ALIGN, "vfm_layernorm_fwd_split3: y3 [rows, >= 3 plane] bf16 with plane >= C, 8-byte aligned; y (optional fp32 copy) 16-byte aligned");
  if (rows == 0) return VFM_OK;
  hipStream_t s = (hipStream_t)stream;
  dim3 grid(cdiv(rows, 4)), blk(256);
  Split3Out so;
  so.y3 = (bf16_t*)y3, so.ld3 = ld3, so.plane = plane;
#define LVS(NV) hipLaunchKernelGGL((k_ln_fwd_v4<float, NV, false, true>), grid, blk, 0, s, x, ld_x, w, b, eps, y, ld_y, stats, rows, (int)C, LnDrop(), so)
  if (nv == 1) LVS(1); else if (nv == 2) LVS(2); else if (nv == 4) LVS(4); else if (nv == 5) LVS(5); else LVS(8);
#undef LVS
  VFM_LAUNCH_CHECK();
  return VFM_OK;
}

extern "C" int vfm_layernorm_fwd(const float* x, long ld_x, const float* w, const float* b, float eps, void* y, int y_dt,
                                 long ld_y, float* stats, long rows, long C, void* stream) {
  VFM_CHECK(C > 0 && C <= 3072 && ld_x >= C && ld_y >= C, VFM_E_SHAPE, "vfm_layernorm_fwd: C=%ld unsupported", C);
  if (rows == 0) return VFM_OK;
  hipStream_t s = (hipStream_t)stream;
  dim3 grid(cdiv(rows, 4)), blk(256);
  const int nvq = (int)(C / 256);
  const bool v4 = (C % 256 == 0) && (nvq == 1 || nvq == 2 || nvq == 4 || nvq == 5 || nvq == 8) && (ld_x % 4 == 0) && (ld_y % 4 == 0) && ((uintptr_t)x % 16 == 0) &&
                  ((uintptr_t)y % 8 == 0) && ((uintptr_t)w % 16 == 0) && ((uintptr_t)b % 16 == 0);
  if (v4) {
#define LV(TO, NV) hipLaunchKernelGGL((k_ln_fwd_v4<TO, NV>), grid, blk, 0, s, x, ld_x, w, b, eps, (TO*)y, ld_y, stats, rows, (int)C)
    const int nv = (int)(C / 256);
    if (y_dt == VFM_BF16) { if (nv == 1) LV(bf16_t, 1); else if (nv == 4) LV(bf16_t, 4); else if (nv == 5) LV(bf16_t, 5); else if (nv == 2) LV(bf16_t, 2); else LV(bf16_t, 8); }
    else if (y_dt == VFM_F32) { if (nv == 1) LV(float, 1); else if (nv == 4) LV(float, 4); else if (nv == 5) LV(float, 5); else if (nv == 2) LV(float, 2); else LV(float, 8); }
    else VFM_FAIL(VFM_E_INVAL, "vfm_layernorm_fwd: dtype");
#undef LV
    if (!(nv == 1 || nv == 2 || nv == 4 || nv == 5 || nv == 8)) VFM_FAIL(VFM_E_SHAPE, "vfm_layernorm_fwd: C=%ld", C);
    VFM_LAUNCH_CHECK();
    return VFM_OK;
  }
  if (C > 1024 && C <= 2816 && ld_x % 4 == 0 && ld_y % 4 == 0 && ld_x >= (C + 3) / 4 * 4 && ld_y >= (C + 3) / 4 * 4 && (uintptr_t)x % 16 == 0 &&
      (uintptr_t)y % 16 == 0 && (uintptr_t)w % 16 == 0 && (uintptr_t)b % 16 == 0) {
    if (y_dt == VFM_BF16) hipLaunchKernelGGL((k_ln_fwd_v4t<bf16_t, 11>), grid, blk, 0, s, x, ld_x, w, b, eps, (bf16_t*)y, ld_y, stats, rows, (int)C);
    else if (y_dt == VFM_F32) hipLaunchKernelGGL((k_ln_fwd_v4t<float, 11>), grid, blk, 0, s, x, ld_x, w, b, eps, (float*)y, ld_y, stats, rows, (int)C);
    else VFM_FAIL(VFM_E_INVAL, "vfm_layernorm_fwd: dtype");
    VFM_LAUNCH_CHECK();
    return VFM_OK;
  }
  if (C > 1024 && C % 2 == 0 && ld_x % 2 == 0 && ld_y % 2 == 0 && (uintptr_t)x % 8 == 0 && (uintptr_t)y % 8 == 0 && (uintptr_t)w % 8 == 0 &&
      (uintptr_t)b % 8 == 0) {
    if (y_dt == VFM_BF16) hipLaunchKernelGGL((k_ln_fwd_v2<bf16_t, 24>), grid, blk, 0, s, x, ld_x, w, b, eps, (bf16_t*)y, ld_y, stats, rows, (int)C);
    else if (y_dt == VFM_F32) hipLaunchKernelGGL((k_ln_fwd_v2<float, 24>), grid, blk, 0, s, x, ld_x, w, b, eps, (float*)y, ld_y, stats, rows, (int)C);
    else VFM_FAIL(VFM_E_INVAL, "vfm_layernorm_fwd: dtype");
    VFM_LAUNCH_CHECK();
    return VFM_OK;
  }
#define L(TO, PL) hipLaunchKernelGGL((k_ln_fwd<TO, PL>), grid, blk, 0, s, x, ld_x, w, b, eps, (TO*)y, ld_y, stats, rows, (int)C)
  const int pl = (int)((C + 63) / 64);
  if (y_dt == VFM_BF16) { if (pl <= 4) L(bf16_t, 4); else if (pl <= 16) L(bf16_t, 16); else if (pl <= 32) L(bf16_t, 32); else L(bf16_t, 48); }
  else if (y_dt == VFM_F32) { if (pl <= 4) L(float, 4); else if (pl <= 16) L(float, 16); else if (pl <= 32) L(float, 32); else L(float, 48); }
  else VFM_FAIL(VFM_E_INVAL, "vfm_layernorm_fwd: dtype");
#undef L
  VFM_LAUNCH_CHECK();
  return VFM_OK;
}

extern "C" int vfm_layernorm_dropout_fwd(const float* x, long ld_x, const float* w, const float* b, float eps, void* y, long ld_y,
                                         float* stats, void* y_drop, long ld_yd, void* mask, long ld_mask, float p, uint64_t seed,
                                         uint64_t offset, long rows, long C, void* stream) {
  VFM_CHECK(p >= 0.f && p < 1.f, VFM_E_INVAL, "vfm_layernorm_dropout_fwd: p");
  const long nv = C / 256;
  VFM_CHECK(C % 256 == 0 && (nv == 1 || nv == 2 || nv == 4 || nv == 5 || nv == 8), VFM_E_SHAPE, "vfm_layernorm_dropout_fwd: C=%ld", C);
  VFM_CHECK(ld_x % 4 == 0 && ld_y % 4 == 0 && ld_yd % 4 == 0 && ld_mask % 4 == 0 && (uintptr_t)x % 16 == 0 && (uintptr_t)y % 8 == 0 &&
                (uintptr_t)y_drop % 8 == 0 && (uintptr_t)mask % 8 == 0 && (uintptr_t)w % 16 == 0 && (uintptr_t)b % 16 == 0,
            VFM_E_ALIGN, "vfm_layernorm_dropout_fwd: alignment");
  if (rows == 0) return VFM_OK;
  hipStream_t s = (hipStream_t)stream;
  dim3 blk(256), grid(cdiv(rows, 4));
  LnDrop dr{y_drop, ld_yd, mask, ld_mask, p, 1.0f / (1.0f - p), seed, offset};
#define LVD(NV) hipLaunchKernelGGL((k_ln_fwd_v4<bf16_t, NV, true>), grid, blk, 0, s, x, ld_x, w, b, eps, (bf16_t*)y, ld_y, stats, rows, (int)C, dr)
  if (nv == 1) LVD(1); else if (nv == 2) LVD(2); else if (nv == 4) LVD(4); else if (nv == 5) LVD(5); else LVD(8);
#undef LVD
  VFM_LAUNCH_CHECK();
  return VFM_OK;
}

template <typename TD, int MAXPL, bool NEED_W>
__global__ void k_ln_bwd(const TD* __restrict__ dy, long ld_dy, const float* __restrict__ x, long ld_x,
                         const float* __restrict__ w, const float* __restrict__ stats, float* __restrict__ dx, long ld_dx,
                         int accumulate_dx, float* __restrict__ ws, long rows, int C) {
  const int lane = threadIdx.x & 63, wv = threadIdx.x >> 6, nw = blockDim.x >> 6;
  float pdw[NEED_W ? MAXPL : 1], pdb[NEED_W ? MAXPL : 1];
#pragma unroll
  for (int i = 0; i < (NEED_W ? MAXPL : 1); ++i) pdw[i] = pdb[i] = 0.f;
  for (long row = (long)blockIdx.x * nw + wv; row < rows; row += (long)gridDim.x * nw) {
    const float mean = stats[row * 2], rstd = stats[row * 2 + 1];
    float g[MAXPL], xh[MAXPL];
    float s1 = 0.f, s2 = 0.f;
#pragma unroll
    for (int i = 0; i < MAXPL; ++i) {
      const int c = i * 64 + lane;
      if (c < C) {
        const float d = ld_f32(dy + row * ld_dy + c);
        xh[i] = (x[row * ld_x + c] - mean) * rstd;
        g[i] = d * w[c];
        s1 += g[i];
        s2 += g[i] * xh[i];
        if constexpr (NEED_W) {
          pdw[i] += d * xh[i];
          pdb[i] += d;
        }
      } else {
        g[i] = xh[i] = 0.f;
      }
    }
    s1 = wave_sum(s1) / C;
    s2 = wave_sum(s2) / C;
#pragma unroll
    for (int i = 0; i < MAXPL; ++i) {
      const int c = i * 64 + lane;
      if (c < C) {
        const float v = rstd * (g[i] - s1 - xh[i] * s2);
        float* p = dx + row * ld_dx + c;
        *p = accumulate_dx ? *p + v : v;
      }
    }
  }
  if constexpr (NEED_W) {
    extern __shared__ float sh[];
#pragma unroll
    for (int i = 0; i < MAXPL; ++i) {
      const int c = i * 64 + lane;
      if (c < C) {
        sh[(wv * 2 + 0) * C + c] = pdw[i];
        sh[(wv * 2 + 1) * C + c] = pdb[i];
      }
    }
    __syncthreads();
    for (int c = threadIdx.x; c < 2 * C; c += blockDim.x) {
      const int which = c / C, cc = c - which * C;
      float a = 0.f;
      for (int k = 0; k < nw; ++k) a += sh[(k * 2 + which) * C + cc];
      ws[((long)blockIdx.x * 2 + which) * C + cc] = a;
    }
  }
}
__global__ void k_ln_bwd_fin(const float* __restrict__ ws, int parts, int C, float* __restrict__ dw, float* __restrict__ db) {
  __shared__ float sh[2][4][64];
  const int tx = threadIdx.x & 63, ty = threadIdx.x >> 6;
  const int c = blockIdx.x * 64 + tx;
  float a = 0.f, b = 0.f;
  if (c < C) {
#pragma unroll 8
    for (int p = ty; p < parts; p += 4) {
      a += ws[((long)p * 2 + 0) * C + c];
      b += ws[((long)p * 2 + 1) * C + c];
    }
  }
  sh[0][ty][tx] = a, sh[1][ty][tx] = b;
  __syncthreads();
  if (ty == 0 && c < C) {
    if (dw) dw[c] += (sh[0][0][tx] + sh[0][1][tx]) + (sh[0][2][tx] + sh[0][3][tx]);
    if (db) db[c] += (sh[1][0][tx] + sh[1][1][tx]) + (sh[1][2][tx] + sh[1][3][tx]);
  }
}

template <typename TD, int MAXP4>
__global__ void k_ln_bwd_v4t(const TD* __restrict__ dy, long ld_dy, const float* __restrict__ x, long ld_x, const float* __restrict__ w,
                             const float* __restrict__ stats, float* __restrict__ dx, long ld_dx, int accumulate_dx, long rows, int C) {
  const int lane = threadIdx.x & 63;
  const long row = (long)blockIdx.x * (blockDim.x >> 6) + (threadIdx.x >> 6);
  if (row >= rows) return;
  const float mean = stats[row * 2], rstd = stats[row * 2 + 1];
  float g[MAXP4][4], xh[MAXP4][4];
  float s1 = 0.f, s2 = 0.f;
#pragma unroll
  for (int i = 0; i < MAXP4; ++i) {
    const int c = (i * 64 + lane) * 4;
#pragma unroll
    for (int e = 0; e < 4; ++e) g[i][e] = xh[i][e] = 0.f;
    if (c < C) {
      float d[4];
      if constexpr (sizeof(TD) == 2) {
        const ushort4 pp = *reinterpret_cast<const ushort4*>(dy + row * ld_dy + c);
        d[0] = bf16_to_f32(pp.x), d[1] = bf16_to_f32(pp.y), d[2] = bf16_to_f32(pp.z), d[3] = bf16_to_f32(pp.w);
      } else {
        const float4 t = *reinterpret_cast<const float4*>(dy + row * ld_dy + c);
        d[0] = t.x, d[1] = t.y, d[2] = t.z, d[3] = t.w;
      }
      const float4 xv4 = *reinterpret_cast<const float4*>(x + row * ld_x + c);
      const float xv[4] = {xv4.x, xv4.y, xv4.z, xv4.w};
      float wv[4] = {0.f, 0.f, 0.f, 0.f};
      if (c + 4 <= C) {
        const float4 ww = *reinterpret_cast<const float4*>(w + c);
        wv[0] = ww.x, wv[1] = ww.y, wv[2] = ww.z, wv[3] = ww.w;
      } else {
#pragma unroll
        for (int e = 0; e < 4; ++e)
          if (c + e < C) wv[e] = w[c + e];
      }
#pragma unroll
      for (int e = 0; e < 4; ++e)
        if (c + e < C) {
          xh[i][e] = (xv[e] - mean) * rstd;
          g[i][e] = d[e] * wv[e];
          s1 += g[i][e];
          s2 += g[i][e] * xh[i][e];
        }
    }
  }
  s1 = wave_sum(s1) / C;
  s2 = wave_sum(s2) / C;
#pragma unroll
  for (int i = 0; i < MAXP4; ++i) {
    const int c = (i * 64 + lane) * 4;
    if (c < C) {
      float o[4];
#pragma unroll
      for (int e = 0; e < 4; ++e) o[e] = rstd * (g[i][e] - s1 - xh[i][e] * s2);
      if (c + 4 <= C) {
        float4* pp = reinterpret_cast<float4*>(dx + row * ld_dx + c);
        if (accumulate_dx) {
          const float4 old = *pp;
          o[0] += old.x, o[1] += old.y, o[2] += old.z, o[3] += old.w;
        }
        *pp = make_float4(o[0], o[1], o[2], o[3]);
      } else {
#pragma unroll
        for (int e = 0; e < 4; ++e)
          if (c + e < C) dx[row * ld_dx + c + e] = accumulate_dx ? dx[row * ld_dx + c + e] + o[e] : o[e];
      }
    }
  }
}

static int ln_bwd_impl(const void* dy, int dy_dt, long ld_dy, const float* x, long ld_x, const float* w, const float* stats,
                       float* dx, long ld_dx, int accumulate_dx, float* dw, float* db, float* ws, long rows, long C, void* t_out,
                       long ld_t, const float* t_scale, void* stream);
extern "C" int vfm_layernorm_bwd(const void* dy, int dy_dt, long ld_dy, const float* x, long ld_x, const float* w,
                                 const float* stats, float* dx, long ld_dx, int accumulate_dx, float* dw, float* db,
                                 float* ws, long rows, long C, void* stream) {
  return ln_bwd_impl(dy, dy_dt, ld_dy, x, ld_x, w, stats, dx, ld_dx, accumulate_dx, dw, db, ws, rows, C, nullptr, 0, nullptr, stream);
}
extern "C" int vfm_layernorm_bwd_scaled(const void* dy, int dy_dt, long ld_dy, const float* x, long ld_x, const float* w,
                                        const float* stats, float* dx, long ld_dx, int accumulate_dx, void* t_out, long ld_t,
                                        const float* t_scale, long rows, long C, void* stream) {
  VFM_CHECK(t_out && t_scale && ld_t % 4 == 0 && (uintptr_t)t_out % 8 == 0 && (uintptr_t)t_scale % 16 == 0, VFM_E_INVAL,
            "vfm_layernorm_bwd_scaled: t_out / t_scale");
  return ln_bwd_impl(dy, dy_dt, ld_dy, x, ld_x, w, stats, dx, ld_dx, accumulate_dx, nullptr, nullptr, nullptr, rows, C, t_out, ld_t,
                     t_scale, stream);
}
template <typename TD, int MAXP2>
__global__ void k_ln_bwd_v2(const TD* __restrict__ dy, long ld_dy, const float* __restrict__ x, long ld_x, const float* __restrict__ w,
                            const float* __restrict__ stats, float* __restrict__ dx, long ld_dx, int accumulate_dx, long rows, int C) {
  const int lane = threadIdx.x & 63;
  const long row = (long)blockIdx.x * (blockDim.x >> 6) + (threadIdx.x >> 6);
  if (row >= rows) return;
  const float mean = stats[row * 2], rstd = stats[row * 2 + 1];
  float2 g[MAXP2], xh[MAXP2];
  float s1 = 0.f, s2 = 0.f;
#pragma unroll
  for (int i = 0; i < MAXP2; ++i) {
    const int c = (i * 64 + lane) * 2;
    g[i] = xh[i] = make_float2(0.f, 0.f);
    if (c < C) {
      float2 d;
      if constexpr (sizeof(TD) == 2) {
        const ushort2 pp = *reinterpret_cast<const ushort2*>(dy + row * ld_dy + c);
        d = make_float2(bf16_to_f32(pp.x), bf16_to_f32(pp.y));
      } else {
        d = *reinterpret_cast<const float2*>(dy + row * ld_dy + c);
      }
      const float2 xv = *reinterpret_cast<const float2*>(x + row * ld_x + c);
      const float2 ww = *reinterpret_cast<const float2*>(w + c);
      xh[i] = make_float2((xv.x - mean) * rstd, (xv.y - mean) * rstd);
      g[i] = make_float2(d.x * ww.x, d.y * ww.y);
      s1 += g[i].x + g[i].y;
      s2 += g[i].x * xh[i].x + g[i].y * xh[i].y;
    }
  }
  s1 = wave_sum(s1) / C;
  s2 = wave_sum(s2) / C;
#pragma unroll
  for (int i = 0; i < MAXP2; ++i) {
    const int c = (i * 64 + lane) * 2;
    if (c < C) {
      float2 o = make_float2(rstd * (g[i].x - s1 - xh[i].x * s2), rstd * (g[i].y - s1 - xh[i].y * s2));
      float2* pp = reinterpret_cast<float2*>(dx + row * ld_dx + c);
      if (accumulate_dx) {
        const float2 old = *pp;
        o.x += old.x, o.y += old.y;
      }
      *pp = o;
    }
  }
}

static int ln_bwd_impl(const void* dy, int dy_dt, long ld_dy, const float* x, long ld_x, const float* w, const float* stats,
                       float* dx, long ld_dx, int accumulate_dx, float* dw, float* db, float* ws, long rows, long C, void* t_out,
                       long ld_t, const float* t_scale, void* stream) {
  VFM_CHECK(C > 0 && (C <= 1024 || (C <= 3072 && !(dw || db))), VFM_E_SHAPE, "vfm_layernorm_bwd: C=%ld unsupported", C);
  VFM_CHECK(!(dw || db) || ws, VFM_E_INVAL, "vfm_layernorm_bwd: ws required for dw/db");
  if (rows == 0) return VFM_OK;
  hipStream_t s = (hipStream_t)stream;
  const bool need_w = (dw || db);
  const int nv = (int)(C / 256);
  const bool v4 = !need_w && (C % 256 == 0) && (nv == 1 || nv == 2 || nv == 4 || nv == 5) && (ld_x % 4 == 0) && (ld_dx % 4 == 0) &&
                  (ld_dy % 4 == 0) && ((uintptr_t)x % 16 == 0) && ((uintptr_t)dx % 16 == 0) && ((uintptr_t)dy % 8 == 0) &&
                  ((uintptr_t)w % 16 == 0);
  if (v4) {
    dim3 grid(cdiv(rows, 4)), blk(256);
#define LV(TD, NV) hipLaunchKernelGGL((k_ln_bwd_v4<TD, NV>), grid, blk, 0, s, (const TD*)dy, ld_dy, x, ld_x, w, stats, dx, ld_dx, accumulate_dx, rows, (int)C, (bf16_t*)t_out, ld_t, t_scale)
    if (dy_dt == VFM_BF16) { if (nv == 1) LV(bf16_t, 1); else if (nv == 2) LV(bf16_t, 2); else if (nv == 4) LV(bf16_t, 4); else LV(bf16_t, 5); }
    else if (dy_dt == VFM_F32) { if (nv == 1) LV(float, 1); else if (nv == 2) LV(float, 2); else if (nv == 4) LV(float, 4); else LV(float, 5); }
    else VFM_FAIL(VFM_E_INVAL, "vfm_layernorm_bwd: dtype");
#undef LV
    VFM_LAUNCH_CHECK();
    return VFM_OK;
  }
  VFM_CHECK(!t_out, VFM_E_UNSUPPORTED, "vfm_layernorm_bwd_scaled: needs the vectorised path (C %% 256 == 0, aligned operands, no dw/db)");
  {
    const long cp = (C + 3) / 4 * 4;
    if (!need_w && C > 1024 && C <= 2816 && ld_x % 4 == 0 && ld_dx % 4 == 0 && ld_dy % 4 == 0 && ld_x >= cp && ld_dx >= cp && ld_dy >= cp &&
        (uintptr_t)x % 16 == 0 && (uintptr_t)dx % 16 == 0 && (uintptr_t)dy % 16 == 0 && (uintptr_t)w % 16 == 0) {
      dim3 grid(cdiv(rows, 4)), blk(256);
      if (dy_dt == VFM_BF16)
        hipLaunchKernelGGL((k_ln_bwd_v4t<bf16_t, 11>), grid, blk, 0, s, (const bf16_t*)dy, ld_dy, x, ld_x, w, stats, dx, ld_dx, accumulate_dx, rows, (int)C);
      else if (dy_dt == VFM_F32)
        hipLaunchKernelGGL((k_ln_bwd_v4t<float, 11>), grid, blk, 0, s, (const float*)dy, ld_dy, x, ld_x, w, stats, dx, ld_dx, accumulate_dx, rows, (int)C);
      else VFM_FAIL(VFM_E_INVAL, "vfm_layernorm_bwd: dtype");
      VFM_LAUNCH_CHECK();
      return VFM_OK;
    }
  }
  if (!need_w && C > 1024 && C % 2 == 0 && ld_x % 2 == 0 && ld_dx % 2 == 0 && ld_dy % 2 == 0 && (uintptr_t)x % 8 == 0 &&
      (uintptr_t)dx % 8 == 0 && (uintptr_t)dy % 8 == 0 && (uintptr_t)w % 8 == 0) {
    dim3 grid(cdiv(rows, 4)), blk(256);
    if (dy_dt == VFM_BF16)
      hipLaunchKernelGGL((k_ln_bwd_v2<bf16_t, 24>), grid, blk, 0, s, (const bf16_t*)dy, ld_dy, x, ld_x, w, stats, dx, ld_dx, accumulate_dx, rows, (int)C);
    else if (dy_dt == VFM_F32)
      hipLaunchKernelGGL((k_ln_bwd_v2<float, 24>), grid, blk, 0, s, (const float*)dy, ld_dy, x, ld_x, w, stats, dx, ld_dx, accumulate_dx, rows, (int)C);
    else VFM_FAIL(VFM_E_INVAL, "vfm_layernorm_bwd: dtype");
    VFM_LAUNCH_CHECK();
    return VFM_OK;
  }
  const int parts = need_w ? 128 : cdiv(rows, 4);
  const size_t shm = need_w ? (size_t)4 * 2 * C * sizeof(float) : 0;
  float* wsp = need_w ? ws : nullptr;
#define L(TD, PL, NW) hipLaunchKernelGGL((k_ln_bwd<TD, PL, NW>), dim3(parts), dim3(256), shm, s, (const TD*)dy, ld_dy, x, ld_x, w, stats, dx, ld_dx, accumulate_dx, wsp, rows, (int)C)
  const int pl = (int)((C + 63) / 64);
  if (need_w) {
    if (dy_dt == VFM_BF16) { if (pl <= 4) L(bf16_t, 4, true); else L(bf16_t, 16, true); }
    else if (dy_dt == VFM_F32) { if (pl <= 4) L(float, 4, true); else L(float, 16, true); }
    else VFM_FAIL(VFM_E_INVAL, "vfm_layernorm_bwd: dtype");
  } else {
    if (dy_dt == VFM_BF16) { if (pl <= 4) L(bf16_t, 4, false); else if (pl <= 16) L(bf16_t, 16, false); else L(bf16_t, 48, false); }
    else if (dy_dt == VFM_F32) { if (pl <= 4) L(float, 4, false); else if (pl <= 16) L(float, 16, false); else L(float, 48, false); }
    else VFM_FAIL(VFM_E_INVAL, "vfm_layernorm_bwd: dtype");
  }
#undef L
  if (need_w) hipLaunchKernelGGL(k_ln_bwd_fin, dim3(cdiv(C, 64)), dim3(256), 0, s, ws, parts, (int)C, dw, db);
  VFM_LAUNCH_CHECK();
  return VFM_OK;
}

template <int MODE, typename TD>
__global__ void k_chan_moments(const float* __restrict__ x, const TD* __restrict__ dy, const float* __restrict__ w,
                               const float* __restrict__ bb, const float* __restrict__ stats, int G, float eps, int act,
                               float* __restrict__ ws, long P, int C, int rows_per_chunk) {
  __shared__ float sh[2][4][64];
  const int tx = threadIdx.x & 63, ty = threadIdx.x >> 6;
  const int c = blockIdx.x * 64 + tx;
  const long b = blockIdx.z;
  const long r0 = (long)blockIdx.y * rows_per_chunk;
  long r1 = r0 + rows_per_chunk;
  if (r1 > P) r1 = P;
  float a1 = 0.f, a2 = 0.f;
  if (c < C) {
    float mean = 0.f, rstd = 1.f, wc = 1.f, bc = 0.f;
    if (MODE == 1) {
      if (G > 0) {
        const int g = c / (C / G);
        mean = stats[(b * G + g) * 2];
        rstd = stats[(b * G + g) * 2 + 1];
      } else {
        mean = stats[c];
        rstd = rsqrtf(stats[C + c] + eps);
      }
      wc = w[c];
      bc = bb[c];
    }
    const float* xp = x + (b * P) * C + c;
    for (long r = r0 + ty; r < r1; r += 4) {
      const float xv = xp[r * C];
      if (MODE == 0) {
        a1 += xv;
        a2 += xv * xv;
      } else {
        const float xh = (xv - mean) * rstd;
        float d = ld_f32(dy + (b * P + r) * C + c);
        if (act != VFM_ACT_NONE) d *= act_grad_f(xh * wc + bc, act);
        a1 += d;
        a2 += d * xh;
      }
    }
  }
  sh[0][ty][tx] = a1;
  sh[1][ty][tx] = a2;
  __syncthreads();
  if (ty == 0 && c < C) {
    const long slot = b * gridDim.y + blockIdx.y;
    ws[(slot * 2 + 0) * C + c] = sh[0][0][tx] + sh[0][1][tx] + sh[0][2][tx] + sh[0][3][tx];
    ws[(slot * 2 + 1) * C + c] = sh[1][0][tx] + sh[1][1][tx] + sh[1][2][tx] + sh[1][3][tx];
  }
}

static inline int pick_chunks(long P) {
  int n = (int)((P + 63) / 64);
  if (n > 64) n = 64;
  if (n < 1) n = 1;
  return n;
}

__device__ __forceinline__ double wave_sum_f64(double v) {
#pragma unroll
  for (int o = 32; o > 0; o >>= 1) v += __shfl_xor(v, o, 64);
  return v;
}
__global__ void k_gn_fin_fwd(const float* __restrict__ ws, int nchunk, int C, int G, long P, float eps,
                             float* __restrict__ stats, int BG) {
  const int i = blockIdx.x * (blockDim.x >> 6) + (threadIdx.x >> 6), lane = threadIdx.x & 63;
  if (i >= BG) return;
  const int b = i / G, g = i - b * G, cg = C / G;
  double s = 0.0, q = 0.0;
  for (int e = lane; e < nchunk * cg; e += 64) {
    const int k = e / cg, j = e - k * cg;
    const long slot = (long)b * nchunk + k;
    s += ws[(slot * 2 + 0) * C + g * cg + j];
    q += ws[(slot * 2 + 1) * C + g * cg + j];
  }
  s = wave_sum_f64(s), q = wave_sum_f64(q);
  if (lane) return;
  const double n = (double)P * cg;
  const double mean = s / n;
  double var = q / n - mean * mean;
  if (var < 0) var = 0;
  stats[i * 2] = (float)mean;
  stats[i * 2 + 1] = (float)(1.0 / sqrt(var + (double)eps));
}
template <typename TO>
__global__ void k_gn_apply(const float* __restrict__ x, const float* __restrict__ w, const float* __restrict__ b,
                           const float* __restrict__ stats, int G, int act, TO* __restrict__ y, long B, long P, int C) {
  const long total = B * P * C;
  const int cg = C / G;
  for (long i = blockIdx.x * (long)blockDim.x + threadIdx.x; i < total; i += (long)gridDim.x * blockDim.x) {
    const int c = (int)(i % C);
    const long bi = i / ((long)P * C);
    const int g = c / cg;
    const float mean = stats[(bi * G + g) * 2], rstd = stats[(bi * G + g) * 2 + 1];
    st_f32(y + i, act_f((x[i] - mean) * rstd * w[c] + b[c], act));
  }
}
extern "C" int vfm_groupnorm_fwd(const float* x, const float* w, const float* b, float eps, int G, int act, void* y, int y_dt,
                                 float* stats, float* ws_in, long B, long P, long C, void* stream) {
  VFM_CHECK(G > 0 && C % G == 0 && ws_in, VFM_E_SHAPE, "vfm_groupnorm_fwd: C %% G / ws");
  if (B * P * C == 0) return VFM_OK;
  hipStream_t s = (hipStream_t)stream;
  const int nchunk = pick_chunks(P);
  const int rpc = (int)((P + nchunk - 1) / nchunk);
  float* ws = ws_in + B * G * 2;
  hipLaunchKernelGGL((k_chan_moments<0, float>), dim3(cdiv(C, 64), nchunk, (unsigned)B), dim3(256), 0, s, x, (const float*)nullptr,
                     (const float*)nullptr, (const float*)nullptr, (const float*)nullptr, 0, 0.f, 0, ws, P, (int)C, rpc);
  hipLaunchKernelGGL(k_gn_fin_fwd, dim3(cdiv(B * G, 4)), dim3(256), 0, s, ws, nchunk, (int)C, G, P, eps, stats, (int)(B * G));
  const long total = B * P * C;
  const int grid = (int)((total + 255) / 256 > 8192 ? 8192 : (total + 255) / 256);
  if (y_dt == VFM_BF16) hipLaunchKernelGGL(k_gn_apply<bf16_t>, dim3(grid), dim3(256), 0, s, x, w, b, stats, G, act, (bf16_t*)y, B, P, (int)C);
  else if (y_dt == VFM_F32) hipLaunchKernelGGL(k_gn_apply<float>, dim3(grid), dim3(256), 0, s, x, w, b, stats, G, act, (float*)y, B, P, (int)C);
  else VFM_FAIL(VFM_E_INVAL, "vfm_groupnorm_fwd: dtype");
  VFM_LAUNCH_CHECK();
  return VFM_OK;
}

__global__ void k_gn_fin_bwd(const float* __restrict__ ws, int nchunk, int C, int G, const float* __restrict__ w,
                             float* __restrict__ gs, int BG) {
  const int i = blockIdx.x * (blockDim.x >> 6) + (threadIdx.x >> 6), lane = threadIdx.x & 63;
  if (i >= BG) return;
  const int b = i / G, g = i - b * G, cg = C / G;
  double s1 = 0.0, s2 = 0.0;
  for (int e = lane; e < nchunk * cg; e += 64) {
    const int k = e / cg, j = e - k * cg;
    const long slot = (long)b * nchunk + k;
    const int c = g * cg + j;
    s1 += (double)w[c] * ws[(slot * 2 + 0) * C + c];
    s2 += (double)w[c] * ws[(slot * 2 + 1) * C + c];
  }
  s1 = wave_sum_f64(s1), s2 = wave_sum_f64(s2);
  if (lane) return;
  gs[i * 2] = (float)s1;
  gs[i * 2 + 1] = (float)s2;
}
__global__ void k_chan_fin_wb(const float* __restrict__ ws, int slots, int C, float* __restrict__ dw, float* __restrict__ db) {
  __shared__ float sh[2][4][64];
  const int tx = threadIdx.x & 63, ty = threadIdx.x >> 6;
  const int c = blockIdx.x * 64 + tx;
  float a = 0.f, b = 0.f;
  if (c < C) {
#pragma unroll 8
    for (int k = ty; k < slots; k += 4) {
      b += ws[((long)k * 2 + 0) * C + c];
      a += ws[((long)k * 2 + 1) * C + c];
    }
  }
  sh[0][ty][tx] = a, sh[1][ty][tx] = b;
  __syncthreads();
// ... 165 lines not shown
```

vfmseg_amd/csrc/plan.hip:

```cpp
#include <vector>

#include "common.h"

namespace {
struct ProfRec {
  int kind;
  double flops;
  hipEvent_t e0, e1;
};
int g_prof_every = 0;
long g_prof_count = 0;
std::vector<ProfRec> g_prof_recs;
std::vector<hipEvent_t> g_prof_pool;

hipEvent_t prof_event() {
  if (!g_prof_pool.empty()) {
    hipEvent_t e = g_prof_pool.back();
    g_prof_pool.pop_back();
    return e;
  }
  hipEvent_t e = nullptr;
  if (hipEventCreate(&e) != hipSuccess) return nullptr;
  return e;
}

int run_one(const vfm_plan_op& o, uint64_t seed, uint64_t rng_base, void* s) {
  switch (o.kind) {
    case VFM_OP_GEMM: return vfm_gemm(&o.u.gemm, s);
    case VFM_OP_ATTN_FWD: return vfm_attn_fwd(&o.u.attn, s);
    case VFM_OP_ATTN_BWD: return vfm_attn_bwd(&o.u.attn, s);
    case VFM_OP_LN_FWD: {
      const auto& a = o.u.ln_fwd;
      return vfm_layernorm_fwd(a.x, a.ld_x, a.w, a.b, a.eps, a.y, a.y_dt, a.ld_y, a.stats, a.rows, a.C, s);
    }
    case VFM_OP_LN_DROPOUT_FWD: {
      const auto& a = o.u.ln_drop;
      return vfm_layernorm_dropout_fwd(a.x, a.ld_x, a.w, a.b, a.eps, a.y, a.ld_y, a.stats, a.y_drop, a.ld_yd, a.mask, a.ld_mask, a.p, seed,
                                       rng_base + a.offset, a.rows, a.C, s);
    }
    case VFM_OP_LN_BWD_SCALED: {
      const auto& a = o.u.ln_bwd;
      return vfm_layernorm_bwd_scaled(a.dy, a.dy_dt, a.ld_dy, a.x, a.ld_x, a.w, a.stats, a.dx, a.ld_dx, a.accumulate_dx, a.t_out, a.ld_t,
                                      a.t_scale, a.rows, a.C, s);
    }
    case VFM_OP_CAST: {
      const auto& a = o.u.cast;
      return vfm_cast(a.src, a.src_dt, a.ld_src, a.dst, a.dst_dt, a.ld_dst, a.rows, a.cols, a.colscale, s);
    }
    case VFM_OP_STRIDED_COPY: {
      const auto& a = o.u.copy;
      return vfm_strided_copy(a.src, a.src_dt, a.dst, a.dst_dt, a.n[0], a.n[1], a.n[2], a.n[3], a.ss[0], a.ss[1], a.ss[2], a.ss[3], a.ds[0],
                              a.ds[1], a.ds[2], a.ds[3], a.accumulate, s);
    }
    default: VFM_FAIL(VFM_E_INVAL, "vfm_run_plan: unknown op kind %d", o.kind);
  }
}
}

extern "C" int vfm_run_plan(const vfm_plan_op* ops, int n, uint64_t seed, uint64_t rng_base, void* stream) {
  VFM_CHECK(ops != nullptr || n == 0, VFM_E_INVAL, "vfm_run_plan: null plan");
  hipStream_t hs = (hipStream_t)stream;
  for (int i = 0; i < n; ++i) {
    const vfm_plan_op& o = ops[i];
    bool timed = false;
    ProfRec rec;
    if (g_prof_every > 0 && o.prof_kind != VFM_PROF_NONE && (++g_prof_count % g_prof_every) == 0 && g_prof_recs.size() < 65536) {
      rec.kind = o.prof_kind, rec.flops = o.flops, rec.e0 = prof_event(), rec.e1 = prof_event();
      timed = rec.e0 && rec.e1 && hipEventRecord(rec.e0, hs) == hipSuccess;
    }
    const int rc = run_one(o, seed, rng_base, stream);
    if (timed) {
      if (hipEventRecord(rec.e1, hs) == hipSuccess) g_prof_recs.push_back(rec);
    }
    if (rc != VFM_OK) {
      char msg[400];
      snprintf(msg, sizeof(msg), "%s", g_vfm_err);
      VFM_FAIL(rc, "vfm_run_plan: entry %d (kind %d) failed: %s", i, o.kind, msg);
    }
  }
  return VFM_OK;
}

extern "C" int vfm_prof_config(int every) {
  VFM_CHECK(every >= 0, VFM_E_INVAL, "vfm_prof_config: every >= 0");
  g_prof_every = every;
  g_prof_count = 0;
  return VFM_OK;
}

extern "C" int vfm_prof_read(double* out, int cap) {
  VFM_CHECK(out != nullptr || cap == 0, VFM_E_INVAL, "vfm_prof_read: null buffer");
  int n = 0;
  for (const ProfRec& r : g_prof_recs) {
    float ms = 0.f;
    if (hipEventSynchronize(r.e1) == hipSuccess && hipEventElapsedTime(&ms, r.e0, r.e1) == hipSuccess && n < cap) {
      out[3 * n] = (double)r.kind, out[3 * n + 1] = r.flops, out[3 * n + 2] = (double)ms;
      ++n;
    }
    g_prof_pool.push_back(r.e0), g_prof_pool.push_back(r.e1);
  }
  g_prof_recs.clear();
  return n;
}
```

vfmseg_amd/lib.py:

```python
import ctypes as C
import os

import torch

_HERE = os.path.dirname(os.path.abspath(__file__))
LIB_PATH = os.path.join(_HERE, "csrc", "libvfmseg_hip.so")
LIB_PATH_F16 = os.path.join(_HERE, "csrc", "libvfmseg_hip_f16.so")

F32, BF16, U8, I64, SPLIT3 = 0, 1, 2, 3, 4
ABI_VERSION = 4
EP_NONE, EP_GELU, EP_RELU, EP_MUL_GELU_GRAD, EP_MUL, EP_QGELU, EP_MUL_QGELU_GRAD, EP_GELU_DGELU = 0, 1, 2, 3, 4, 5, 6, 7
ACT_NONE, ACT_GELU, ACT_RELU, ACT_QGELU = 0, 1, 2, 3

vp, ci, cl, cf, u64 = C.c_void_p, C.c_int, C.c_long, C.c_float, C.c_uint64


class GemmDesc(C.Structure):
    _fields_ = [
        ("A", vp), ("B", vp), ("C", vp),
        ("in_dt", ci), ("c_dt", ci),
        ("M", cl), ("N", cl), ("K", cl),
        ("sa_m", cl), ("sa_k", cl), ("sb_n", cl), ("sb_k", cl), ("ldc", cl),
        ("alpha", cf),
        ("bias", vp), ("bias_mod", cl),
        ("colscale", vp),
        ("residual", vp), ("r_dt", ci), ("ldr", cl),
        ("ep_mode", ci), ("aux", vp), ("aux_dt", ci), ("ld_aux", cl),
        ("C2", vp), ("c2_dt", ci), ("ldc2", cl),
        ("batch", cl), ("stride_a", cl), ("stride_b", cl), ("stride_c", cl),
        ("c_plane", cl),
        ("kb_rows", cl),
    ]


class AttnDesc(C.Structure):
    _fields_ = [
        ("q", vp), ("k", vp), ("v", vp), ("o", vp),
        ("dt", ci), ("ldq", cl), ("ldk", cl), ("ldv", cl), ("ldo", cl),
        ("B", ci), ("H", ci), ("d", ci),
        ("nq_main", ci), ("nq_extra", ci), ("nk_main", ci), ("nk_extra", ci),
        ("scale", cf),
        ("lse", vp),
        ("dout", vp), ("ld_do", cl),
        ("dq", vp), ("dk", vp), ("dv", vp), ("ld_dq", cl), ("ld_dk", cl), ("ld_dv", cl),
        ("delta", vp),
    ]


class _LnFwd(C.Structure):
    _fields_ = [("x", vp), ("ld_x", cl), ("w", vp), ("b", vp), ("eps", cf), ("y", vp), ("y_dt", ci), ("ld_y", cl), ("stats", vp),
                ("rows", cl), ("C", cl)]


class _LnDrop(C.Structure):
    _fields_ = [("x", vp), ("ld_x", cl), ("w", vp), ("b", vp), ("eps", cf), ("y", vp), ("ld_y", cl), ("stats", vp), ("y_drop", vp),
                ("ld_yd", cl), ("mask", vp), ("ld_mask", cl), ("p", cf), ("offset", u64), ("rows", cl), ("C", cl)]


class _LnBwd(C.Structure):
    _fields_ = [("dy", vp), ("dy_dt", ci), ("ld_dy", cl), ("x", vp), ("ld_x", cl), ("w", vp), ("stats", vp), ("dx", vp), ("ld_dx", cl),
                ("accumulate_dx", ci), ("t_out", vp), ("ld_t", cl), ("t_scale", vp), ("rows", cl), ("C", cl)]


class _CastOp(C.Structure):
    _fields_ = [("src", vp), ("src_dt", ci), ("ld_src", cl), ("dst", vp), ("dst_dt", ci), ("ld_dst", cl), ("rows", cl), ("cols", cl),
                ("colscale", vp)]


class _CopyOp(C.Structure):
    _fields_ = [("src", vp), ("src_dt", ci), ("dst", vp), ("dst_dt", ci), ("n", cl * 4), ("ss", cl * 4), ("ds", cl * 4), ("accumulate", ci)]


class _PlanU(C.Union):
    _fields_ = [("gemm", GemmDesc), ("attn", AttnDesc), ("ln_fwd", _LnFwd), ("ln_drop", _LnDrop), ("ln_bwd", _LnBwd), ("cast", _CastOp),
                ("copy", _CopyOp)]


class PlanOp(C.Structure):
    _fields_ = [("kind", ci), ("prof_kind", ci), ("flops", C.c_double), ("u", _PlanU)]


OP_GEMM, OP_LN_FWD, OP_LN_DROPOUT_FWD, OP_LN_BWD_SCALED, OP_ATTN_FWD, OP_ATTN_BWD, OP_CAST, OP_STRIDED_COPY = range(8)
PROF_NONE, PROF_GEMM, PROF_GEMM_TN, PROF_ATTN_FWD, PROF_ATTN_BWD = range(5)
PROF_NAMES = {PROF_GEMM: "gemm", PROF_GEMM_TN: "gemm_tn", PROF_ATTN_FWD: "attn_fwd", PROF_ATTN_BWD: "attn_bwd"}


class SlideWin(C.Structure):
    _fields_ = [("crop", vp), ("nchw", ci), ("h", ci), ("w", ci), ("y0", ci), ("x0", ci), ("hc", ci), ("wc", ci)]


SIGNATURES = {
    "vfm_cast": [vp, ci, cl, vp, ci, cl, cl, cl, vp, vp],
    "vfm_split3": [vp, cl, cl, vp, cl, cl, cl, ci, vp],
    "vfm_transpose": [vp, ci, cl, vp, ci, cl, cl, cl, cl, vp],
    "vfm_strided_copy": [vp, ci, vp, ci] + [cl] * 12 + [ci, vp],
    "vfm_strided_copy_batch": [vp, ci, cl, vp],
    "vfm_axpby": [vp, cf, vp, cf, cl, vp],
    "vfm_scale_by_device_scalar": [vp, vp, cl, vp],
    "vfm_colsum": [vp, ci, cl, cl, cl, vp, ci, vp, vp],
    "vfm_preprocess_u8": [vp, ci, ci, vp, ci, ci, C.POINTER(C.c_float), C.POINTER(C.c_float), ci, cf, vp],
    "vfm_lora_pack": [vp, ci, cl, ci, vp],
    "vfm_slab_reduce": [vp, ci, cl, cl, cl, cf, vp, cl, cl, ci, vp],
    "vfm_dropout_mask": [vp, ci, cl, cf, u64, u64, vp],
    "vfm_mul_mask": [vp, ci, cl, vp, ci, cl, cl, vp, ci, cl, cl, cl, vp],
    "vfm_geglu_fwd": [vp, ci, cl, vp, ci, cl, cl, cl, vp],
    "vfm_geglu_bwd": [vp, ci, cl, vp, ci, cl, vp, ci, cl, cl, cl, vp],
    "vfm_swiglu_fwd": [vp, ci, cl, vp, ci, cl, cl, cl, vp],
    "vfm_swiglu_bwd": [vp, ci, cl, vp, ci, cl, vp, ci, cl, cl, cl, vp],
    "vfm_rope": [vp, ci, cl, cl, ci, ci, ci, vp, vp, ci, vp],
    "vfm_act_grad_mul": [vp, ci, cl, vp, ci, cl, vp, ci, cl, cl, cl, ci, vp],
    "vfm_mask_token_fwd": [vp, vp, vp, vp, cl, cl, vp],
    "vfm_mask_token_bwd": [vp, vp, vp, vp, vp, cl, cl, vp],
    "vfm_layernorm_fwd": [vp, cl, vp, vp, cf, vp, ci, cl, vp, cl, cl, vp],
    "vfm_layernorm_fwd_split3": [vp, cl, vp, vp, cf, vp, cl, vp, cl, cl, vp, cl, cl, vp],
    "vfm_layernorm_dropout_fwd": [vp, cl, vp, vp, cf, vp, cl, vp, vp, cl, vp, cl, cf, u64, u64, cl, cl, vp],
    "vfm_layernorm_bwd_scaled": [vp, ci, cl, vp, cl, vp, vp, vp, cl, ci, vp, cl, vp, cl, cl, vp],
    "vfm_layernorm_bwd": [vp, ci, cl, vp, cl, vp, vp, vp, cl, ci, vp, vp, vp, cl, cl, vp],
    "vfm_groupnorm_fwd": [vp, vp, vp, cf, ci, ci, vp, ci, vp, vp, cl, cl, cl, vp],
    "vfm_groupnorm_bwd": [vp, ci, vp, vp, vp, vp, ci, ci, vp, vp, vp, vp, cl, cl, cl, vp],
    "vfm_bn_moments": [vp, cl, cl, vp, vp, vp],
    "vfm_bn_finalize": [vp, cf, vp, vp, vp, cf, cl, vp],
    "vfm_bn_apply": [vp, vp, vp, vp, cf, ci, vp, ci, cl, cl, vp],
    "vfm_bn_bwd_reduce": [vp, ci, vp, vp, vp, vp, cf, ci, vp, vp, cl, cl, vp],
    "vfm_bn_bwd_apply": [vp, ci, vp, vp, vp, vp, cf, ci, vp, cf, vp, cl, cl, vp],
    "vfm_gemm": [C.POINTER(GemmDesc), vp],
    "vfm_tune": [C.c_char_p, ci],
    "vfm_attn_fwd": [C.POINTER(AttnDesc), vp],
    "vfm_attn_fwd_x3": [C.POINTER(AttnDesc), cl, vp],
    "vfm_attn_fwd_x3_split": [C.POINTER(AttnDesc), cl, vp, cl, cl, vp],
    "vfm_attn_bwd": [C.POINTER(AttnDesc), vp],
    "vfm_attn_bwd_x3": [C.POINTER(AttnDesc), vp, vp, vp, cl, cl, vp, cl, cl, vp],
    "vfm_sam_relpos_table": [vp, ci, ci, ci, vp, vp],
    "vfm_sam_attn_prep": [vp, ci, cl, vp, vp, vp, vp, vp, vp, ci, ci, ci, ci, ci, ci, ci, ci, cf, vp],
    "vfm_softmax_rows": [vp, cl, vp, ci, cl, cl, ci, ci, vp],
    "vfm_sam_attn_merge": [vp, ci, vp, cl, ci, ci, ci, ci, ci, ci, vp],
    "vfm_sam_attn_bwd_prep": [vp, cl, vp, cl, vp, ci, vp, vp, vp, vp, ci, ci, ci, ci, ci, ci, ci, cf, vp],
    "vfm_softmax_rows_batched": [vp, cl, vp, ci, cl, cl, ci, ci, ci, ci, vp],
    "vfm_softmax_rows_bwd": [vp, vp, cl, vp, ci, cl, cl, ci, ci, ci, ci, vp],
    "vfm_rein_mix_fwd": [vp, cl, vp, vp, vp, cl, vp, cl, vp, cl, cl, ci, ci, cf, vp],
    "vfm_rein_mix_bwd": [vp, cl, vp, cl, vp, vp, vp, cl, vp, cl, cl, ci, ci, cf, vp],
    "vfm_sam_attn_bwd_merge": [vp, vp, vp, ci, vp, vp, vp, cl, ci, ci, ci, ci, ci, ci, ci, ci, cf, vp],
    "vfm_sam_attn_flash_fwd": [vp, cl, vp, vp, vp, vp, cl, ci, ci, ci, ci, ci, cf, vp],
    "vfm_sam_attn_flash_fwd_train": [vp, cl, vp, vp, vp, vp, cl, ci, ci, ci, ci, ci, cf, vp, vp, vp],
    "vfm_sam_attn_flash_bwd": [vp, cl, vp, vp, vp, vp, vp, cl, vp, vp, vp, vp, cl, ci, ci, ci, ci, ci, cf, vp],
    "vfm_patchify": [vp, cl, cl, cl, ci, ci, ci, ci, ci, vp, ci, cl, ci, vp],
    "vfm_assemble_tokens": [vp, vp, vp, vp, ci, ci, ci, vp],
    "vfm_resize_bilinear": [vp, ci, ci, ci, ci, ci, ci, cl, vp, ci, ci, cl, ci, ci, ci, ci, ci, ci, cf, cf, vp],
    "vfm_resize_bicubic": [vp, ci, ci, ci, vp, ci, ci, cf, cf, vp],
    "vfm_label_resize": [vp, ci, ci, ci, vp, ci, ci, ci, ci, ci, ci, vp],
    "vfm_unblock": [vp, vp, ci, ci, ci, ci, ci, ci, vp],
    "vfm_upsample_ce": [vp, vp, ci, ci, ci, ci, ci, ci, ci, vp, vp, vp, vp],
    "vfm_reduce_sum": [vp, cl, cf, vp, vp],
    "vfm_ce_finish": [vp, cl, cf, vp, cf, vp, vp, vp],
    "vfm_conf_gate": [vp, ci, ci, ci, ci, ci, ci, ci, ci, cf, vp, vp],
    "vfm_slide_accumulate": [vp, ci, ci, ci, ci, ci, vp, vp, ci, ci, ci, ci, ci, ci, vp],
    "vfm_slide_finalize": [vp, vp, vp, ci, ci, ci, ci, vp],
    "vfm_slide_gather": [vp, ci, ci, ci, vp, ci, ci, vp],
    "vfm_conf_gate_windows": [vp, ci, ci, ci, ci, vp, ci, cf, vp, vp],
    "vfm_confusion_hist": [vp, vp, ci, cl, ci, ci, vp, vp],
    "vfm_adamw": [vp, vp, vp, vp, cl, vp, vp, vp, ci, cf, cf, cf, cf, ci, cf, ci, ci, vp],
    "vfm_adamw_guarded": [vp, vp, vp, vp, cl, vp, vp, vp, ci, cf, cf, cf, cf, ci, cf, ci, ci, vp, vp, vp],
    "vfm_amp_update": [vp, vp, cf, cf, ci, ci, vp],
    "vfm_run_plan": [C.POINTER(PlanOp), ci, u64, u64, vp],
    "vfm_prof_config": [ci],
    "vfm_prof_read": [C.POINTER(C.c_double), ci],
}

_lib = None
_libs = {}
_half = 0
HALF_DTYPES = (torch.bfloat16, torch.float16)


class HipLibraryMissing(RuntimeError):
    pass


def _open(kind):
    path = LIB_PATH_F16 if kind else LIB_PATH
    if not os.path.exists(path):
        raise HipLibraryMissing(
            f"{path} not found: build it with `python -m vfmseg_amd.csrc.build` (hipcc --offload-arch=gfx950)")
    lib = C.CDLL(path)
    lib.vfm_last_error.restype = C.c_char_p
    lib.vfm_abi_version.restype = ci
    lib.vfm_half_kind.restype = ci
    if lib.vfm_abi_version() < ABI_VERSION:
        raise HipLibraryMissing(f"{path} has ABI version {lib.vfm_abi_version()}, this binding needs {ABI_VERSION}: rebuild (python -m vfmseg_amd.csrc.build)")
    if lib.vfm_half_kind() != kind:
        raise HipLibraryMissing(f"{path} reports half kind {lib.vfm_half_kind()}, expected {kind}: stale build")
    for name, args in SIGNATURES.items():
        fn = getattr(lib, name)
        fn.argtypes = args
        fn.restype = ci
    return lib


def load():
    global _lib
    if _lib is not None:
        return _lib
    if _half not in _libs:
        _libs[_half] = _open(_half)
    _lib = _libs[_half]
    return _lib


def set_half(kind):
    global _half, _lib
    kind = {torch.bfloat16: 0, torch.float16: 1, "bf16": 0, "fp16": 1, "f16": 1}.get(kind, kind)
    assert kind in (0, 1)
    if kind != _half:
        _half, _lib = kind, None


def half_dtype():
    return torch.float16 if _half else torch.bfloat16


class HipError(RuntimeError):
    pass


def check(rc, name):
    if rc != 0:
        raise HipError(f"{name} failed ({rc}): {load().vfm_last_error().decode()}")


_raw_stream = getattr(torch._C, "_cuda_getCurrentRawStream", None)
_dev_index = None


def stream():
    global _dev_index
    if _raw_stream is not None:
        if _dev_index is None:
            _dev_index = torch.cuda.current_device()
        return _raw_stream(_dev_index)
    return torch.cuda.current_stream().cuda_stream


def set_device_index(i):
    global _dev_index
    _dev_index = i


def dt_of(t):
    if t.dtype == torch.float32:
        return F32
    if t.dtype == torch.bfloat16 or t.dtype == torch.float16:
        if (t.dtype == torch.float16) != bool(_half):
            raise TypeError(f"{t.dtype} tensor handed to the {'fp16' if _half else 'bf16'} library (precision mode and tensors disagree)")
        return BF16
    if t.dtype == torch.uint8 or t.dtype == torch.bool:
        return U8
    if t.dtype == torch.int64:
        return I64
    raise TypeError(f"unsupported dtype {t.dtype}")


def torch_dt(code):
    return torch.float32 if code == F32 else half_dtype()


def ptr(t):
    if t is None:
        return None
    if not t.is_cuda:
        raise HipError("vfmseg_amd ops need GPU tensors (no CPU fallback in the product path)")
    return t.data_ptr()
# ... 1 lines not shown
```

vfmseg_amd/ops.py:

```python
import ctypes as C
import os

import torch

from .precision import is_half
from . import lib as L
from .lib import (ACT_GELU, ACT_NONE, ACT_QGELU, ACT_RELU, BF16, EP_GELU, EP_GELU_DGELU, EP_MUL, EP_MUL_GELU_GRAD,
                  EP_MUL_QGELU_GRAD, EP_NONE, EP_QGELU, EP_RELU, F32)

_ws_cache = {}

PROFILE = None
REGION = ["heads"]


class region:
    def __init__(self, name):
        self.name = name

    def __enter__(self):
        REGION.append(self.name)

    def __exit__(self, *a):
        REGION.pop()
# ... 78 lines not shown
        self.table = torch.frombuffer(buf, dtype=torch.uint8).clone().to(jobs[0][1].device) if jobs else None

    def run(self):
        if self.n:
            lib = L.load()
            L.check(lib.vfm_strided_copy_batch(L.ptr(self.table), self.n, self.max_elems, L.stream()), "vfm_strided_copy_batch")


def permute_copy(src, perm, dst):
    v = src.permute(*perm)
    strided_copy(src, dst, list(v.shape), list(v.stride()), list(torch.empty(v.shape, device="meta").stride()))
    return dst


def axpby(x, a, y, b):
    lib = L.load()
    assert x.is_contiguous() and y.is_contiguous() and x.dtype == y.dtype == torch.float32 and x.numel() == y.numel()
    L.check(lib.vfm_axpby(L.ptr(x), float(a), L.ptr(y), float(b), x.numel(), L.stream()), "vfm_axpby")
    return y


def scale_by_device_scalar(y, scalar):
    lib = L.load()
    assert y.is_contiguous() and y.dtype == torch.float32
    L.check(lib.vfm_scale_by_device_scalar(L.ptr(y), L.ptr(scalar), y.numel(), L.stream()), "vfm_scale_by_device_scalar")
    return y


def colsum(x, out, accumulate=False):
    lib = L.load()
    rows, cols = x.shape
    ws = workspace(64 * cols, x.device)
    L.check(lib.vfm_colsum(L.ptr(x), L.dt_of(x), _ld(x), rows, cols, L.ptr(out), int(accumulate), L.ptr(ws), L.stream()),
            "vfm_colsum")
    return out


def dropout_mask(out, p, seed, offset=0):
    lib = L.load()
    assert out.is_contiguous()
    L.check(lib.vfm_dropout_mask(L.ptr(out), L.dt_of(out), out.numel(), float(p), int(seed), int(offset), L.stream()),
            "vfm_dropout_mask")
    return out


def mul_mask(src, mask, dst, rows_per_group=1):
    lib = L.load()
    L.check(lib.vfm_mul_mask(L.ptr(src), L.dt_of(src), _ld(src), L.ptr(mask), L.dt_of(mask), _ld(mask), rows_per_group,
                             L.ptr(dst), L.dt_of(dst), _ld(dst), src.shape[0], src.shape[1], L.stream()), "vfm_mul_mask")
    return dst


def geglu_fwd(h, out):
    lib = L.load()
    rows, c2 = h.shape
    L.check(lib.vfm_geglu_fwd(L.ptr(h), L.dt_of(h), _ld(h), L.ptr(out), L.dt_of(out), _ld(out), rows, c2 // 2, L.stream()),
            "vfm_geglu_fwd")
    return out


def geglu_bwd(h, dout, dh):
    lib = L.load()
    rows, c2 = h.shape
    L.check(lib.vfm_geglu_bwd(L.ptr(h), L.dt_of(h), _ld(h), L.ptr(dout), L.dt_of(dout), _ld(dout), L.ptr(dh), L.dt_of(dh),
                              _ld(dh), rows, c2 // 2, L.stream()), "vfm_geglu_bwd")
    return dh


def swiglu_fwd(h, out, C_):
    lib = L.load()
    L.check(lib.vfm_swiglu_fwd(L.ptr(h), L.dt_of(h), _ld(h), L.ptr(out), L.dt_of(out), _ld(out), h.shape[0], C_, L.stream()),
            "vfm_swiglu_fwd")
    return out


def swiglu_bwd(h, dout, dh, C_):
    lib = L.load()
    L.check(lib.vfm_swiglu_bwd(L.ptr(h), L.dt_of(h), _ld(h), L.ptr(dout), L.dt_of(dout), _ld(dout), L.ptr(dh), L.dt_of(dh),
                               _ld(dh), h.shape[0], C_, L.stream()), "vfm_swiglu_bwd")
    return dh


def rope(x, rows, np_, ncols, d, cos_t, sin_t, inverse=False):
    lib = L.load()
    L.check(lib.vfm_rope(L.ptr(x), L.dt_of(x), _ld(x), rows, np_, ncols, d, L.ptr(cos_t), L.ptr(sin_t), int(inverse), L.stream()),
            "vfm_rope")
    return x


def act_grad_mul(dy, pre, out, act):
    lib = L.load()
    L.check(lib.vfm_act_grad_mul(L.ptr(dy), L.dt_of(dy), _ld(dy), L.ptr(pre), L.dt_of(pre), _ld(pre), L.ptr(out),
                                 L.dt_of(out), _ld(out), dy.shape[0], dy.shape[1], act, L.stream()), "vfm_act_grad_mul")
    return out


def mask_token_fwd(x, keep, token, out):
    lib = L.load()
    L.check(lib.vfm_mask_token_fwd(L.ptr(x), L.ptr(keep), L.ptr(token), L.ptr(out), x.shape[0], x.shape[1], L.stream()),
            "vfm_mask_token_fwd")
    return out


def mask_token_bwd(dout, keep, dx, dtoken):
    lib = L.load()
    ws = workspace(64 * dout.shape[1], dout.device)
    L.check(lib.vfm_mask_token_bwd(L.ptr(dout), L.ptr(keep), L.ptr(dx), L.ptr(dtoken), L.ptr(ws), dout.shape[0], dout.shape[1],
                                   L.stream()), "vfm_mask_token_bwd")


def _split_key(t):
    return (t.data_ptr(), tuple(t.shape), tuple(t.stride()), t._version)


def _register_split_out(t, t3):
    try:
        t._vfm_split3_out = (_split_key(t), t3)
    except AttributeError:
        pass


def layernorm_fwd(x, w, b, eps, y, stats=None, split_out=None):
    lib = L.load()
    rows, c = x.shape
    if split_out and _split3_on() and y.dtype == torch.float32 and c % 256 == 0 and c // 256 in (1, 2, 4, 5, 8) and y.shape[1] == c:
        kp = (c + 63) // 64 * 64
        y3 = torch.empty(rows, 3 * kp, dtype=L.half_dtype(), device=x.device)
        L.check(lib.vfm_layernorm_fwd_split3(L.ptr(x), _ld(x), L.ptr(w), L.ptr(b), float(eps), None if split_out == "only" else L.ptr(y), _ld(y),
                                             L.ptr(y3), y3.stride(0), kp, L.ptr(stats), rows, c, L.stream()), "vfm_layernorm_fwd_split3")
        _register_split_out(y, y3)
        return y
    L.check(lib.vfm_layernorm_fwd(L.ptr(x), _ld(x), L.ptr(w), L.ptr(b), float(eps), L.ptr(y), L.dt_of(y), _ld(y),
                                  L.ptr(stats), rows, c, L.stream()), "vfm_layernorm_fwd")
    return y


def layernorm_dropout_fwd(x, w, b, eps, y, stats, y_drop, mask, p, seed, offset=0):
    lib = L.load()
    rows, c = x.shape
    assert is_half(y.dtype) and is_half(y_drop.dtype) and is_half(mask.dtype)
    L.check(lib.vfm_layernorm_dropout_fwd(L.ptr(x), _ld(x), L.ptr(w), L.ptr(b), float(eps), L.ptr(y), _ld(y), L.ptr(stats),
                                          L.ptr(y_drop), _ld(y_drop), L.ptr(mask), _ld(mask), float(p), int(seed), int(offset),
                                          rows, c, L.stream()), "vfm_layernorm_dropout_fwd")
    return y


def layernorm_bwd_scaled(dy, x, w, stats, dx, t_out, t_scale, accumulate_dx=False):
    lib = L.load()
    rows, c = x.shape
    assert is_half(t_out.dtype) and t_scale.dtype == torch.float32
    L.check(lib.vfm_layernorm_bwd_scaled(L.ptr(dy), L.dt_of(dy), _ld(dy), L.ptr(x), _ld(x), L.ptr(w), L.ptr(stats), L.ptr(dx),
                                         _ld(dx), int(accumulate_dx), L.ptr(t_out), _ld(t_out), L.ptr(t_scale), rows, c,
                                         L.stream()), "vfm_layernorm_bwd_scaled")
    return dx


def layernorm_bwd(dy, x, w, stats, dx, accumulate_dx=False, dw=None, db=None):
    lib = L.load()
    rows, c = x.shape
    ws = workspace(2 * 128 * c, x.device) if (dw is not None or db is not None) else None
    L.check(lib.vfm_layernorm_bwd(L.ptr(dy), L.dt_of(dy), _ld(dy), L.ptr(x), _ld(x), L.ptr(w), L.ptr(stats), L.ptr(dx),
                                  _ld(dx), int(accumulate_dx), L.ptr(dw), L.ptr(db), L.ptr(ws), rows, c, L.stream()),
            "vfm_layernorm_bwd")
    return dx


def groupnorm_fwd(x, w, b, eps, groups, act, y, stats, B, P):
    lib = L.load()
    c = x.shape[1]
    ws = workspace(B * groups * 2 + B * 64 * 2 * c, x.device)
    L.check(lib.vfm_groupnorm_fwd(L.ptr(x), L.ptr(w), L.ptr(b), float(eps), groups, act, L.ptr(y), L.dt_of(y), L.ptr(stats),
                                  L.ptr(ws), B, P, c, L.stream()), "vfm_groupnorm_fwd")
    return y


def groupnorm_bwd(dy, x, w, b, stats, groups, act, dx, dw, db, B, P):
    lib = L.load()
    c = x.shape[1]
    ws = workspace(B * groups * 2 + B * 64 * 2 * c, x.device)
    L.check(lib.vfm_groupnorm_bwd(L.ptr(dy), L.dt_of(dy), L.ptr(x), L.ptr(w), L.ptr(b), L.ptr(stats), groups, act, L.ptr(dx),
                                  L.ptr(dw), L.ptr(db), L.ptr(ws), B, P, c, L.stream()), "vfm_groupnorm_bwd")
    return dx


def bn_moments(x, sums):
    lib = L.load()
    rows, c = x.shape
    ws = workspace(64 * 2 * c, x.device)
    L.check(lib.vfm_bn_moments(L.ptr(x), rows, c, L.ptr(sums), L.ptr(ws), L.stream()), "vfm_bn_moments")
    return sums


def bn_finalize(sums, count, mean_var, running_mean=None, running_var=None, momentum=0.1):
    lib = L.load()
    L.check(lib.vfm_bn_finalize(L.ptr(sums), float(count), L.ptr(mean_var), L.ptr(running_mean), L.ptr(running_var),
                                float(momentum), sums.shape[1], L.stream()), "vfm_bn_finalize")
    return mean_var


def bn_apply(x, mean_var, w, b, eps, act, y):
    lib = L.load()
    rows, c = x.shape
    L.check(lib.vfm_bn_apply(L.ptr(x), L.ptr(mean_var), L.ptr(w), L.ptr(b), float(eps), act, L.ptr(y), L.dt_of(y), rows, c,
                             L.stream()), "vfm_bn_apply")
    return y


def bn_bwd_reduce(dy, x, mean_var, w, b, eps, act, sums_dy):
    lib = L.load()
    rows, c = x.shape
    ws = workspace(64 * 2 * c, x.device)
    L.check(lib.vfm_bn_bwd_reduce(L.ptr(dy), L.dt_of(dy), L.ptr(x), L.ptr(mean_var), L.ptr(w), L.ptr(b), float(eps), act,
                                  L.ptr(sums_dy), L.ptr(ws), rows, c, L.stream()), "vfm_bn_bwd_reduce")
    return sums_dy


def bn_bwd_apply(dy, x, mean_var, w, b, eps, act, sums_dy, total_rows, dx):
    lib = L.load()
    rows, c = x.shape
    L.check(lib.vfm_bn_bwd_apply(L.ptr(dy), L.dt_of(dy), L.ptr(x), L.ptr(mean_var), L.ptr(w), L.ptr(b), float(eps), act,
                                 L.ptr(sums_dy), float(total_rows), L.ptr(dx), rows, c, L.stream()), "vfm_bn_bwd_apply")
    return dx


def split3(x, pattern, trans=False, cache=False):
    if pattern == 0 and not trans:
        hit = getattr(x, "_vfm_split3_out", None)
        if hit is not None and hit[0] == _split_key(x):
            return hit[1]
    if cache:
        from .optim import PARAM_EPOCH
        key = (PARAM_EPOCH[0], x._version, x.data_ptr(), pattern, trans, tuple(x.shape), tuple(x.stride()))
        hit = getattr(x, "_vfm_split3", None)
        if hit is not None and hit[0] == key:
            return hit[1]
    rows, K = (x.shape[1], x.shape[0]) if trans else (x.shape[0], x.shape[1])
    sr, sc = (x.stride(1), x.stride(0)) if trans else (x.stride(0), x.stride(1))
    kp = (K + 63) // 64 * 64
    out = torch.empty(rows, 3 * kp, dtype=L.half_dtype(), device=x.device)
    L.check(L.load().vfm_split3(L.ptr(x), sr, sc, L.ptr(out), out.stride(0), rows, K, pattern, L.stream()), "vfm_split3")
    if cache:
        try:
            x._vfm_split3 = (key, out)
        except AttributeError:
            pass
    return out


def gemm(a, b, c, *, alpha=1.0, bias=None, bias_mod=0, colscale=None, residual=None, ep_mode=EP_NONE, aux=None, c2=None,
         trans_a=False, trans_b=False, kb_rows=0, c_split=None):
    if a.dtype == torch.float32 and b.dtype == torch.float32 and a.dim() == 2 and not kb_rows and _split3_on():
        a3 = split3(a, 0, trans=trans_a)
        b3 = split3(b, 1, trans=trans_b, cache=not b.requires_grad)
        c3 = None
        if (c_split == "only" and c.dtype == torch.float32 and c.dim() == 2 and c.shape[1] % 64 == 0 and residual is None and c2 is None
                and ep_mode in (EP_NONE, EP_GELU)):
            c3 = torch.empty(c.shape[0], 3 * c.shape[1], dtype=L.half_dtype(), device=c.device)
        gemm(a3, b3, c, alpha=alpha, bias=bias, bias_mod=bias_mod, colscale=colscale, residual=residual, ep_mode=ep_mode, aux=aux, c2=c2, c_split=c3)
        if c3 is not None:
            _register_split_out(c, c3)
        return c
    lib = L.load()
    d = gemm_desc(a, b, c, alpha=alpha, bias=bias, bias_mod=bias_mod, colscale=colscale, residual=residual, ep_mode=ep_mode, aux=aux, c2=c2,
                  trans_a=trans_a, trans_b=trans_b, kb_rows=kb_rows)
    if torch.is_tensor(c_split):
        d.C, d.c_dt, d.ldc, d.c_plane = L.ptr(c_split), L.SPLIT3, c_split.stride(0), c.shape[1]
    fin = PROFILE("gemm", 2.0 * d.M * d.N * d.K * d.batch, REGION[-1]) if (PROFILE is not None and is_half(a.dtype)) else None
    L.check(lib.vfm_gemm(C.byref(d), L.stream()), "vfm_gemm")
    if fin is not None:
        fin()
    return c


def gemm_desc(a, b, c, *, alpha=1.0, bias=None, bias_mod=0, colscale=None, residual=None, ep_mode=EP_NONE, aux=None, c2=None,
              trans_a=False, trans_b=False, kb_rows=0, d=None):
    d = L.GemmDesc() if d is None else d
    batched = a.dim() == 3
    a2 = a[0] if batched else a
    b2 = b[0] if batched else b
    c2d = c[0] if batched else c
    if trans_a:
        K, M = a2.shape
        d.sa_m, d.sa_k = a2.stride(1), a2.stride(0)
    else:
        M, K = a2.shape
        d.sa_m, d.sa_k = a2.stride(0), a2.stride(1)
    if trans_b:
        Kb, N = b2.shape
        d.sb_n, d.sb_k = b2.stride(1), b2.stride(0)
    else:
        N, Kb = b2.shape
        d.sb_n, d.sb_k = b2.stride(0), b2.stride(1)
    if kb_rows:
        assert trans_b and Kb == kb_rows and K >= Kb, "kb_rows: b holds the first kb_rows of the K (token) dimension"
        d.kb_rows = int(kb_rows)
    else:
        assert K == Kb, f"gemm K mismatch {K} vs {Kb}"
    assert a.dtype == b.dtype
    assert c2d.shape[0] == M and c2d.shape[1] == N and c2d.stride(1) == 1
    d.A, d.B, d.C = L.ptr(a), L.ptr(b), L.ptr(c)
    d.in_dt, d.c_dt = L.dt_of(a), L.dt_of(c)
    d.M, d.N, d.K = M, N, K
    d.ldc = c2d.stride(0)
    d.alpha = float(alpha)
    d.bias, d.bias_mod = L.ptr(bias), int(bias_mod)
    d.colscale = L.ptr(colscale)
    if residual is not None:
        r2 = residual[0] if batched else residual
        d.residual, d.r_dt, d.ldr = L.ptr(residual), L.dt_of(residual), r2.stride(0)
    d.ep_mode = ep_mode
    if aux is not None:
        d.aux, d.aux_dt, d.ld_aux = L.ptr(aux), L.dt_of(aux), aux.stride(0)
    if c2 is not None:
        d.C2, d.c2_dt, d.ldc2 = L.ptr(c2), L.dt_of(c2), c2.stride(0)
    if batched:
        d.batch, d.stride_a, d.stride_b, d.stride_c = a.shape[0], a.stride(0), b.stride(0), c.stride(0)
    else:
        d.batch = 1
    return d


class Plan:

    def __init__(self, region="backbone"):
        self.ops, self.keep, self.arr, self.region = [], [], None, region

    def _new(self, kind, prof=L.PROF_NONE, flops=0.0, *tensors):
        op = L.PlanOp()
        op.kind, op.prof_kind, op.flops = kind, prof, float(flops)
        self.ops.append(op)
        self.keep.extend(t for t in tensors if t is not None)
        self.arr = None
        return op

    def gemm(self, a, b, c, **kw):
        op = self._new(L.OP_GEMM, L.PROF_GEMM if is_half(a.dtype) else L.PROF_NONE, 0.0, a, b, c, kw.get("bias"), kw.get("colscale"),
                       kw.get("residual"), kw.get("aux"), kw.get("c2"))
        d = gemm_desc(a, b, c, d=op.u.gemm, **kw)
        op.flops = 2.0 * d.M * d.N * d.K * d.batch
        return len(self.ops) - 1

    def layernorm_fwd(self, x, w, b, eps, y, stats):
        op = self._new(L.OP_LN_FWD, L.PROF_NONE, 0.0, x, w, b, y, stats)
        u = op.u.ln_fwd
        u.x, u.ld_x, u.w, u.b, u.eps, u.y, u.y_dt, u.ld_y, u.stats = L.ptr(x), _ld(x), L.ptr(w), L.ptr(b), float(eps), L.ptr(y), L.dt_of(y), _ld(y), L.ptr(stats)
        u.rows, u.C = x.shape
        return len(self.ops) - 1

    def layernorm_dropout_fwd(self, x, w, b, eps, y, stats, y_drop, mask, p, offset):
        assert is_half(y.dtype) and is_half(y_drop.dtype) and is_half(mask.dtype)
        op = self._new(L.OP_LN_DROPOUT_FWD, L.PROF_NONE, 0.0, x, w, b, y, stats, y_drop, mask)
        u = op.u.ln_drop
        u.x, u.ld_x, u.w, u.b, u.eps, u.y, u.ld_y, u.stats = L.ptr(x), _ld(x), L.ptr(w), L.ptr(b), float(eps), L.ptr(y), _ld(y), L.ptr(stats)
        u.y_drop, u.ld_yd, u.mask, u.ld_mask, u.p, u.offset = L.ptr(y_drop), _ld(y_drop), L.ptr(mask), _ld(mask), float(p), int(offset)
        u.rows, u.C = x.shape
        return len(self.ops) - 1

    def layernorm_bwd_scaled(self, dy, x, w, stats, dx, t_out, t_scale, accumulate_dx=False):
        assert is_half(t_out.dtype) and t_scale.dtype == torch.float32
        op = self._new(L.OP_LN_BWD_SCALED, L.PROF_NONE, 0.0, dy, x, w, stats, dx, t_out, t_scale)
        u = op.u.ln_bwd
        u.dy, u.dy_dt, u.ld_dy, u.x, u.ld_x, u.w, u.stats = L.ptr(dy), L.dt_of(dy), _ld(dy), L.ptr(x), _ld(x), L.ptr(w), L.ptr(stats)
        u.dx, u.ld_dx, u.accumulate_dx, u.t_out, u.ld_t, u.t_scale = L.ptr(dx), _ld(dx), int(accumulate_dx), L.ptr(t_out), _ld(t_out), L.ptr(t_scale)
        u.rows, u.C = x.shape
        return len(self.ops) - 1

    def attn_fwd(self, q, k, v, o, lse, B, H, d, nq_main, nq_extra, nk_main, nk_extra, scale):
        fl = 4.0 * B * H * (nq_main + nq_extra) * (nk_main + nk_extra) * d
        op = self._new(L.OP_ATTN_FWD, L.PROF_ATTN_FWD if is_half(q.dtype) else L.PROF_NONE, fl, q, k, v, o, lse)
        C.memmove(C.byref(op.u.attn), C.byref(_attn_desc(q, k, v, o, B, H, d, nq_main, nq_extra, nk_main, nk_extra, scale, lse)), C.sizeof(L.AttnDesc))
        return len(self.ops) - 1

    def attn_bwd(self, q, k, v, o, lse, dout, dq, dk, dv, B, H, d, nq_main, nq_extra, nk_main, nk_extra, scale):
        fl = 10.0 * B * H * (nq_main + nq_extra) * (nk_main + nk_extra) * d
        delta = _attn_bwd_delta(q, B, H, nq_main + nq_extra)
        op = self._new(L.OP_ATTN_BWD, L.PROF_ATTN_BWD if is_half(q.dtype) else L.PROF_NONE, fl, q, k, v, o, lse, dout, dq, dk, dv, delta)
        a = _attn_desc(q, k, v, o, B, H, d, nq_main, nq_extra, nk_main, nk_extra, scale, lse)
        a.dout, a.ld_do = L.ptr(dout), dout.stride(0)
        a.dq, a.dk, a.dv = L.ptr(dq), L.ptr(dk), L.ptr(dv)
        a.ld_dq, a.ld_dk, a.ld_dv = dq.stride(0), dk.stride(0), dv.stride(0)
        a.delta = L.ptr(delta)
        C.memmove(C.byref(op.u.attn), C.byref(a), C.sizeof(L.AttnDesc))
        return len(self.ops) - 1

    def cast(self, src, dst, colscale=None):
        op = self._new(L.OP_CAST, L.PROF_NONE, 0.0, src, dst, colscale)
        u = op.u.cast
        u.src, u.src_dt, u.ld_src, u.dst, u.dst_dt, u.ld_dst = L.ptr(src), L.dt_of(src), _ld(src), L.ptr(dst), L.dt_of(dst), _ld(dst)
        u.rows, u.cols = src.shape
        u.colscale = L.ptr(colscale)
        return len(self.ops) - 1

    def strided_copy(self, src, dst, shape, sstr, dstr, accumulate=False):
        op = self._new(L.OP_STRIDED_COPY, L.PROF_NONE, 0.0, src, dst)
        u = op.u.copy
        k = 4 - len(shape)
        u.src, u.src_dt, u.dst, u.dst_dt = L.ptr(src), L.dt_of(src), L.ptr(dst), L.dt_of(dst)
        for i, (n, s_, d_) in enumerate(zip([1] * k + list(shape), [0] * k + list(sstr), [0] * k + list(dstr))):
            u.n[i], u.ss[i], u.ds[i] = n, s_, d_
        u.accumulate = int(accumulate)
        return len(self.ops) - 1

    def _array(self):
        if self.arr is None:
            self.arr = (L.PlanOp * len(self.ops))()
            for i, op in enumerate(self.ops):
                C.memmove(C.byref(self.arr[i]), C.byref(op), C.sizeof(L.PlanOp))
        return self.arr

    def entry(self, i):
        return self._array()[i]

    def run(self, seed=0, rng_base=0, start=0, count=None):
        arr = self._array()
        n = len(self.ops) - start if count is None else count
        first = C.cast(C.byref(arr, start * C.sizeof(L.PlanOp)), C.POINTER(L.PlanOp))
        L.check(L.load().vfm_run_plan(first, n, int(seed), int(rng_base), L.stream()), "vfm_run_plan")

    def __len__(self):
        return len(self.ops)


def prof_config(every):
    L.check(L.load().vfm_prof_config(int(every)), "vfm_prof_config")


def prof_read(cap=65536):
    buf = (C.c_double * (3 * cap))()
    n = L.load().vfm_prof_read(buf, cap)
    if n < 0:
        L.check(n, "vfm_prof_read")
    return [(L.PROF_NAMES.get(int(buf[3 * i]), "other"), buf[3 * i + 1], buf[3 * i + 2]) for i in range(n)]


class LoraPackTable:

    def __init__(self, sites, dt_tensor):
        import struct
        buf = bytearray()
        self.max_elems = 0
        self.keep = []
        for (A, B, a, at, w, wt, r, K, N, Kw) in sites:
            assert A.dtype == torch.float32 and B.dtype == torch.float32 and A.is_contiguous() and B.is_contiguous()
            self.keep += [A, B, a, at, w, wt]
            buf += struct.pack("6Q8q", A.data_ptr(), B.data_ptr(), a.data_ptr(), at.data_ptr(), w.data_ptr(),
                               wt.data_ptr() if wt is not None else 0, r, K, N, Kw, a.stride(0), at.stride(0), w.stride(0),
                               wt.stride(0) if wt is not None else 0)
            self.max_elems = max(self.max_elems, r * (K + N))
        self.n = len(sites)
        self.dt = L.dt_of(dt_tensor)
        dev = sites[0][2].device
        self.table = torch.frombuffer(buf, dtype=torch.uint8).clone().to(dev)
        self.ptrs = [s_[0].data_ptr() for s_ in sites] + [s_[1].data_ptr() for s_ in sites]

    def valid_for(self, sites):
        return self.n == len(sites) and self.ptrs == [s_[0].data_ptr() for s_ in sites] + [s_[1].data_ptr() for s_ in sites]

    def run(self):
        lib = L.load()
        L.check(lib.vfm_lora_pack(L.ptr(self.table), self.n, self.max_elems, self.dt, L.stream()), "vfm_lora_pack")


def slab_reduce(slabs, rows_used, dst, sp, sq, alpha=1.0, accumulate=False):
    lib = L.load()
    kch, P, Q = slabs.shape
    assert slabs.is_contiguous() and slabs.dtype == torch.float32 and dst.dtype == torch.float32
    L.check(lib.vfm_slab_reduce(L.ptr(slabs), kch, P, Q, int(rows_used), float(alpha), L.ptr(dst), int(sp), int(sq), int(accumulate),
                                L.stream()), "vfm_slab_reduce")
    return dst


def gemm_splitk_bt(at, y, slabs, kch):
    lib = L.load()
    d = L.GemmDesc()
    P, mp = at.shape
    M, Q = y.shape
    ck = mp // kch
    assert ck * kch == mp and ck % 64 == 0 and slabs.shape == (kch, P, Q)
    d.A, d.B, d.C = L.ptr(at), L.ptr(y), L.ptr(slabs)
    d.in_dt, d.c_dt = L.dt_of(at), L.dt_of(slabs)
    d.M, d.N, d.K = P, Q, ck
    d.sa_m, d.sa_k = at.stride(0), 1
    d.sb_n, d.sb_k = 1, y.stride(0)
    d.ldc = slabs.stride(1)
    d.alpha = 1.0
    d.batch, d.stride_a, d.stride_b, d.stride_c = kch, ck, ck * y.stride(0), slabs.stride(0)
    d.kb_rows = int(M)
    fin = PROFILE("gemm_tn", 2.0 * P * Q * mp, REGION[-1]) if PROFILE is not None else None
    L.check(lib.vfm_gemm(C.byref(d), L.stream()), "vfm_gemm")
    if fin is not None:
        fin()
    return slabs


def gemm_splitk_tn(xs, y, slabs, kch):
    lib = L.load()
    d = L.GemmDesc()
    M, P = xs.shape
    M2, Q = y.shape
    assert M == M2 and xs.stride(1) == 1 and y.stride(1) == 1
    mp = (M + 63) // 64 * 64
    ck = mp // kch
    assert ck * kch == mp and ck % 64 == 0 and slabs.shape == (kch, P, Q)
    d.A, d.B, d.C = L.ptr(xs), L.ptr(y), L.ptr(slabs)
    d.in_dt, d.c_dt = L.dt_of(xs), L.dt_of(slabs)
    d.M, d.N, d.K = P, Q, ck
    d.sa_m, d.sa_k = 1, xs.stride(0)
    d.sb_n, d.sb_k = 1, y.stride(0)
    d.ldc = slabs.stride(1)
    d.alpha = 1.0
    d.batch, d.stride_a, d.stride_b, d.stride_c = kch, ck * xs.stride(0), ck * y.stride(0), slabs.stride(0)
    d.kb_rows = int(M)
    fin = PROFILE("gemm_tn", 2.0 * P * Q * mp, REGION[-1]) if PROFILE is not None else None
    L.check(lib.vfm_gemm(C.byref(d), L.stream()), "vfm_gemm")
    if fin is not None:
        fin()
    return slabs


# ... 428 lines not shown
```

Baseline: 128.6 images/s.

## Fuse LoRA-A projection and dropout mask regeneration into layernorm kernels

Adds a fused forward kernel that computes layernorm, dropout and the rank-64 LoRA-A projection in one pass, and a fused backward kernel that regenerates the dropout mask from the RNG seed. In the same pass the backward kernel applies the LoRA-A transpose product, runs the layernorm backward and can fold in one feature-tap gradient add. This removes the separate LoRA GEMM launches, the stored per-layer dropout mask tensors and an extra strided copy. The cost is recomputing the mask and the small rank-64 matmul inside the norm kernels, which may add register pressure. The change is on by default via an environment flag, is wired into both the plan and eager paths, and bumps the ABI version.

```diff
diff --git a/include/vfmseg_hip.h b/include/vfmseg_hip.h
--- a/include/vfmseg_hip.h
+++ b/include/vfmseg_hip.h
@@ -69,6 +69,13 @@
 int vfm_layernorm_bwd_scaled(const void* dy, int dy_dt, long ld_dy, const float* x, long ld_x, const float* w,
                              const float* stats, float* dx, long ld_dx, int accumulate_dx, void* t_out, long ld_t,
                              const float* t_scale, long rows, long C, void* stream);
+int vfm_layernorm_dropout_lora_fwd(const float* x, long ld_x, const float* w, const float* b, float eps, void* y, long ld_y,
+                                   float* stats, void* y_drop, long ld_yd, void* t, long ld_t, const void* a, long ld_a, float alpha,
+                                   float p, uint64_t seed, uint64_t offset, long rows, long C, void* stream);
+int vfm_layernorm_bwd_lora(const void* dy, long ld_dy, const void* dt, long ld_dt, const void* at, long ld_at, float alpha, float p,
+                           uint64_t seed, uint64_t offset, const float* x, long ld_x, const float* w, const float* stats, float* dx,
+                           long ld_dx, int accumulate_dx, const void* tap, long ld_tap, long tap_rows, void* t_out, long ld_t,
+                           const float* t_scale, long rows, long C, void* stream);
 int vfm_layernorm_bwd(const void* dy, int dy_dt, long ld_dy, const float* x, long ld_x, const float* w,
                       const float* stats, float* dx, long ld_dx, int accumulate_dx, float* dw, float* db, float* ws,
                       long rows, long C, void* stream);
@@ -199,7 +206,7 @@
 int vfm_amp_update(const int* flag, float* amp_state, float growth, float backoff, int interval, int dynamic, void* stream);
 
 enum { VFM_OP_GEMM = 0, VFM_OP_LN_FWD = 1, VFM_OP_LN_DROPOUT_FWD = 2, VFM_OP_LN_BWD_SCALED = 3, VFM_OP_ATTN_FWD = 4, VFM_OP_ATTN_BWD = 5,
-       VFM_OP_CAST = 6, VFM_OP_STRIDED_COPY = 7 };
+       VFM_OP_CAST = 6, VFM_OP_STRIDED_COPY = 7, VFM_OP_LN_DROPOUT_LORA_FWD = 8, VFM_OP_LN_BWD_LORA = 9 };
 enum { VFM_PROF_NONE = 0, VFM_PROF_GEMM = 1, VFM_PROF_GEMM_TN = 2, VFM_PROF_ATTN_FWD = 3, VFM_PROF_ATTN_BWD = 4 };
 typedef struct vfm_plan_op {
   int kind;
@@ -216,6 +223,11 @@
              long ld_dx; int accumulate_dx; void* t_out; long ld_t; const float* t_scale; long rows, C; } ln_bwd;
     struct { const void* src; int src_dt; long ld_src; void* dst; int dst_dt; long ld_dst; long rows, cols; const float* colscale; } cast;
     struct { const void* src; int src_dt; void* dst; int dst_dt; long n[4]; long ss[4]; long ds[4]; int accumulate; } copy;
+    struct { const float* x; long ld_x; const float* w; const float* b; float eps; void* y; long ld_y; float* stats; void* y_drop;
+             long ld_yd; void* t; long ld_t; const void* a; long ld_a; float alpha; float p; uint64_t offset; long rows, C; } ln_lora_fwd;
+    struct { const void* dy; long ld_dy; const void* dt; long ld_dt; const void* at; long ld_at; float alpha; float p; uint64_t offset;
+             const float* x; long ld_x; const float* w; const float* stats; float* dx; long ld_dx; int accumulate_dx; const void* tap;
+             long ld_tap; long tap_rows; void* t_out; long ld_t; const float* t_scale; long rows, C; } ln_lora_bwd;
   } u;
 } vfm_plan_op;
 int vfm_run_plan(const vfm_plan_op* ops, int n, uint64_t seed, uint64_t rng_base, void* stream);
diff --git a/vfmseg_amd/backbones.py b/vfmseg_amd/backbones.py
--- a/vfmseg_amd/backbones.py
+++ b/vfmseg_amd/backbones.py
@@ -347,7 +347,7 @@
 
 class _DinoTrainPlan:
 
-    def __init__(self, eng, P, nimg, Np):
+    def __init__(self, eng, P, nimg, Np, fz=0):
         v = eng.vit
         cd, dev = P["cd"], P["dev"]
         D, H = v.embed_dim, v.num_heads
@@ -361,7 +361,11 @@
         e = lambda *sh, dt=cd: torch.empty(*sh, dtype=dt, device=dev)
         f32 = torch.float32
         self.X = e(nL + 1, M, D, dt=f32)
-        self.A1, self.XD, self.MASK = e(nL, M, kq), e(nL, M, D), e(nL, M, D)
+        self.A1, self.XD = e(nL, M, kq), e(nL, M, D)
+        self.fz, self.p = fz, q0.p
+        nmask = nL if not fz & 2 else (0 if fz & 1 else 1)
+        self.MASK = e(nmask, M, D) if nmask else None
+        self.mask_of = lambda li: self.MASK[li if nmask == nL else 0]
         self.ST1, self.ST2 = e(nL, M, 2, dt=f32), e(nL, M, 2, dt=f32)
         self.QKV, self.AO = e(nL, M, 3 * D), e(nL, M, D)
         self.LSE = e(nL, nimg, H, Np + 1, dt=f32)
@@ -379,8 +383,12 @@
         for li, (blk, Lp) in enumerate(zip(v.blocks, P["layers"])):
             q = blk.attn.qkv
             x, a1 = self.X[li], self.A1[li]
-            f.layernorm_dropout_fwd(x, Lp["n1w"], Lp["n1b"], 1e-6, a1[:, :D], self.ST1[li], self.XD[li], self.MASK[li], q.p, li * M * D)
-            f.gemm(self.XD[li], Lp["a"], a1[:, D:D + R_PAD], alpha=q.scaling)
+            if fz & 1:
+                f.layernorm_dropout_lora_fwd(x, Lp["n1w"], Lp["n1b"], 1e-6, a1[:, :D], self.ST1[li], self.XD[li], a1[:, D:D + R_PAD], Lp["a"],
+                                             q.scaling, q.p, li * M * D)
+            else:
+                f.layernorm_dropout_fwd(x, Lp["n1w"], Lp["n1b"], 1e-6, a1[:, :D], self.ST1[li], self.XD[li], self.mask_of(li), q.p, li * M * D)
+                f.gemm(self.XD[li], Lp["a"], a1[:, D:D + R_PAD], alpha=q.scaling)
             f.gemm(a1, Lp["qkv"].w, self.QKV[li], bias=Lp["qkv_b"])
             qkv = self.QKV[li]
             f.attn_fwd(qkv[:, :D], qkv[:, D:2 * D], qkv[:, 2 * D:], self.AO[li], self.LSE[li], nimg, H, hd, Np, 1, Np, 1, scale)
@@ -405,6 +413,8 @@
         for idx, col in self.tap_ops:
             self.fwd.entry(idx).u.cast.dst = xcat.data_ptr() + col * esz
         self.fwd.run(seed, rng0)
+        if self.fz & 1 and not self.fz & 2:
+            ops.dropout_mask(self.MASK, self.p, seed, offset=rng0)
 
     def _build_backward(self, dxcat):
         v, P = self.eng.vit, self.P
@@ -422,12 +432,28 @@
         self.half = half
         self.dx_sig = (tuple(dxcat.shape), tuple(dxcat.stride()), dxcat.dtype)
         plans, self.tap_src = [], []
-
-        def add_tap(pl, pn, li):
+        fz = self.fz
+
+        def add_tap(pl, pn, li, keep=0):
             for i, oi in enumerate(v.out_indices):
                 if oi == li:
+                    if keep > 0:
+                        keep -= 1
+                        continue
                     src = dxcat[:, i * D:(i + 1) * D]
-                    self.tap_src.append((pn, pl.strided_copy(src, self.DX, (Mp, D), (src.stride(0), 1), (D, 1), accumulate=True), i * D))
+                    self.tap_src.append((pn, pl.strided_copy(src, self.DX, (Mp, D), (src.stride(0), 1), (D, 1), accumulate=True), i * D, "copy"))
+
+        def ln1_bwd_lora(pl, pn, li, t_scale, tap_li):
+            Lp, da1, q = P["layers"][li], self.DA1[li], v.blocks[li].attn.qkv
+            taps = [i for i, oi in enumerate(v.out_indices) if oi == tap_li] if tap_li is not None else []
+            fold = taps[0] if (taps and fz & 4) else None
+            if tap_li is not None:
+                add_tap(pl, pn, tap_li, keep=0 if fold is None else 1)
+            src = dxcat[:, fold * D:(fold + 1) * D] if fold is not None else None
+            idx = pl.layernorm_bwd_lora(da1[:, :D], da1[:, D:D + R_PAD], Lp["at"], q.scaling, q.p, li * M * D, self.X[li], Lp["n1w"],
+                                        self.ST1[li], self.DX, self.T, t_scale, accumulate_dx=True, tap=src)
+            if fold is not None:
+                self.tap_src.append((pn, idx, fold * D, "ln"))
 
         for pn, (hi, lo) in enumerate(((nL, half), (half, 0)) if half > 0 else ((nL, 0),)):
             pl = ops.Plan("backbone")
@@ -448,7 +474,13 @@
                     pl.gemm(dqkv, Lp["qkv"].wt[D:D + R_PAD], da1[:, D:D + R_PAD])
                     continue
                 pl.gemm(dqkv, Lp["qkv"].wt, da1)
-                pl.gemm(da1[:, D:D + R_PAD], Lp["at"], da1[:, :D], alpha=q.scaling, residual=da1[:, :D], ep_mode=ops.EP_MUL, aux=self.MASK[li])
+                if fz & 2:
+                    if li > 0:
+                        ln1_bwd_lora(pl, pn, li, P["layers"][li - 1]["g2"], li - 1)
+                    else:
+                        ln1_bwd_lora(pl, pn, li, Lp["g2"], None)
+                    continue
+                pl.gemm(da1[:, D:D + R_PAD], Lp["at"], da1[:, :D], alpha=q.scaling, residual=da1[:, :D], ep_mode=ops.EP_MUL, aux=self.mask_of(li))
                 if li > 0:
                     add_tap(pl, pn, li - 1)
                     pl.layernorm_bwd_scaled(da1[:, :D], self.X[li], Lp["n1w"], self.ST1[li], self.DX, self.T, P["layers"][li - 1]["g2"],
@@ -463,11 +495,15 @@
         if self.bwd is None or self.dx_sig != sig:
             self._build_backward(dxcat)
         esz = dxcat.element_size()
-        for pn, idx, col in self.tap_src:
-            self.bwd[pn][0].entry(idx).u.copy.src = dxcat.data_ptr() + col * esz
+        for pn, idx, col, kind in self.tap_src:
+            u = self.bwd[pn][0].entry(idx).u
+            if kind == "ln":
+                u.ln_lora_bwd.tap = dxcat.data_ptr() + col * esz
+            else:
+                u.copy.src = dxcat.data_ptr() + col * esz
         self.DX.zero_()
         for pl, lo, hi in self.bwd:
-            pl.run()
+            pl.run(ctx["seed"], ctx["rng0"])
             self.eng._lora_wgrads_batched(self.P, ctx, self.DA1, self.DQKV, lo, hi, self.M, self.D)
             if BACKWARD_EVENTS["block_done"] is not None:
                 for lj in range(hi - 1, lo - 1, -1):
@@ -639,7 +675,8 @@
         if plan is not None:
             plan.run_forward(xcat, seed, rng0)
             plan.busy = True
-            ctx = dict(saved=None, plan=plan, nimg=nimg, Np=Np, M=M, Mp=Mp, P=P, training=training, A1all=plan.A1, XDall=plan.XD)
+            ctx = dict(saved=None, plan=plan, nimg=nimg, Np=Np, M=M, Mp=Mp, P=P, training=training, A1all=plan.A1, XDall=plan.XD,
+                       seed=seed, rng0=rng0)
             return xcat, (hp, wp), ctx
         nL = len(v.blocks)
         batched = lora and training and is_half(cd) and merged is None
@@ -647,6 +684,7 @@
         XDall = None
         hd = D // H
         scale = hd ** -0.5
+        fz = ops.lora_ln_fused() if D in ops.LORA_LN_WIDTHS else 0
         for li, (blk, Lp) in enumerate(zip(v.blocks, P["layers"])):
             S = {"x_in": x}
             kq = D if merged is not None else Lp["qkv"].k
@@ -654,12 +692,21 @@
             st1 = torch.empty(M, 2, dtype=torch.float32, device=dev)
             q = blk.attn.qkv if lora else None
             fused_drop = lora and training and q.p > 0 and is_half(cd) and D % 256 == 0
+            fuse_lora = fused_drop and merged is None and fz & 1
             if fused_drop:
-                mask = torch.empty(M, D, dtype=cd, device=dev)
                 if batched and XDall is None:
                     XDall = torch.empty(nL, M, D, dtype=cd, device=dev)
                 xd = XDall[li] if batched else torch.empty(M, D, dtype=cd, device=dev)
-                ops.layernorm_dropout_fwd(x, Lp["n1w"], Lp["n1b"], 1e-6, a1[:, :D], st1, xd, mask, q.p, seed, offset=rng0 + li * M * D)
+                off = rng0 + li * M * D
+                S["drop"] = (q.p, seed, off)
+                mask = torch.empty(M, D, dtype=cd, device=dev) if not (fuse_lora and fz & 2 and li > 0 and rein is None) else None
+                if fuse_lora:
+                    ops.layernorm_dropout_lora_fwd(x, Lp["n1w"], Lp["n1b"], 1e-6, a1[:, :D], st1, xd, a1[:, D:D + R_PAD], Lp["a"], q.scaling,
+                                                   q.p, seed, offset=off)
+                    if mask is not None:
+                        ops.dropout_mask(mask, q.p, seed, offset=off)
+                else:
+                    ops.layernorm_dropout_fwd(x, Lp["n1w"], Lp["n1b"], 1e-6, a1[:, :D], st1, xd, mask, q.p, seed, offset=off)
             else:
                 so = "only" if (x3 and not training and not need_grad and kq == D) else None
                 ops.layernorm_fwd(x, Lp["n1w"], Lp["n1b"], 1e-6, a1 if kq == D else a1[:, :D], st1, split_out=so)
@@ -671,8 +718,9 @@
                         ops.dropout_mask(mask, q.p, seed, offset=rng0 + li * M * D)
                         xd = torch.empty(M, D, dtype=cd, device=dev)
                         ops.mul_mask(a1[:, :D], mask, xd)
-                ops.gemm(xd, Lp["a"], a1[:, D:D + R_PAD], alpha=q.scaling)
-                S.update(xd=xd if mask is not None else None, mask=mask)
+                if not fuse_lora:
+                    ops.gemm(xd, Lp["a"], a1[:, D:D + R_PAD], alpha=q.scaling)
+                S.update(xd=xd if (mask is not None or fused_drop) else None, mask=mask)
             qkv = torch.empty(M, 3 * D, dtype=cd, device=dev)
             if merged is not None:
                 ops.gemm(a1, merged[li], qkv, bias=Lp["qkv_b"])
@@ -705,7 +753,7 @@
             for i, oi in enumerate(v.out_indices):
                 if oi == li:
                     ops.cast(x[:Mp], xcat[:, i * D:(i + 1) * D])
-        ctx = dict(saved=saved, nimg=nimg, Np=Np, M=M, Mp=Mp, P=P, training=training, A1all=A1all, XDall=XDall, rein=rein)
+        ctx = dict(saved=saved, nimg=nimg, Np=Np, M=M, Mp=Mp, P=P, training=training, A1all=A1all, XDall=XDall, rein=rein, fz=fz)
         return xcat, (hp, wp), ctx
 
     def _train_plan(self, P, nimg, Np, training, merged):
@@ -718,9 +766,10 @@
                    for b in v.blocks):
             return None
         plans = P.setdefault("plans", {})
-        pl = plans.get((nimg, Np))
+        fz = ops.lora_ln_fused() if v.embed_dim in ops.LORA_LN_WIDTHS else 0
+        pl = plans.get((nimg, Np, fz))
         if pl is None:
-            pl = plans[(nimg, Np)] = _DinoTrainPlan(self, P, nimg, Np)
+            pl = plans[(nimg, Np, fz)] = _DinoTrainPlan(self, P, nimg, Np, fz)
         if pl.busy or not pl.eligible_backward():
             return None
         return pl
@@ -756,9 +805,13 @@
         half = nL // 2
         fuse_t = is_half(cd) and D % 256 == 0
         fuse_t1 = fuse_t and rein is None
-        def add_tap(li):
+        fz = ctx.get("fz", 0)
+        def add_tap(li, keep=0):
             for i, oi in enumerate(v.out_indices):
                 if oi == li:
+                    if keep > 0:
+                        keep -= 1
+                        continue
                     src = dxcat[:, i * D:(i + 1) * D]
                     ops.strided_copy(src, dx, (Mp, D), (src.stride(0), 1), (D, 1), accumulate=True)
         t = None
@@ -791,7 +844,10 @@
             kq = Lp["qkv"].k
             da1 = DA1all[li] if wg_batched else torch.empty(M, kq, dtype=cd, device=dev)
             Lp["qkv"].dgrad(dqkv, da1)
-            if isinstance(q, LoraLinear) and wg_batched:
+            ln_lora = bool(fz & 2) and isinstance(q, LoraLinear) and S.get("drop") is not None and fuse_t1 and li > 0
+            if isinstance(q, LoraLinear) and wg_batched and ln_lora:
+                pass
+            elif isinstance(q, LoraLinear) and wg_batched:
                 ep = dict(ep_mode=ops.EP_MUL, aux=S["mask"]) if S["mask"] is not None else {}
                 ops.gemm(da1[:, D:D + R_PAD], Lp["at"], da1[:, :D], alpha=q.scaling, residual=da1[:, :D], **ep)
             elif isinstance(q, LoraLinear):
@@ -820,9 +876,18 @@
                     ops.axpby(gAp[:r].reshape(-1), 1.0, tA.view(-1), 1.0)
                 else:
                     grads[2 * li] = gAp[:r]
-                ep = dict(ep_mode=ops.EP_MUL, aux=S["mask"]) if S["mask"] is not None else {}
-                ops.gemm(da1[:, D:D + R_PAD], Lp["at"], da1[:, :D], alpha=q.scaling, residual=da1[:, :D], **ep)
-            if fuse_t1 and li > 0:
+                if not ln_lora:
+                    ep = dict(ep_mode=ops.EP_MUL, aux=S["mask"]) if S["mask"] is not None else {}
+                    ops.gemm(da1[:, D:D + R_PAD], Lp["at"], da1[:, :D], alpha=q.scaling, residual=da1[:, :D], **ep)
+            if ln_lora:
+                taps = [i for i, oi in enumerate(v.out_indices) if oi == li - 1]
+                fold = taps[0] if (taps and fz & 4) else None
+                add_tap(li - 1, keep=0 if fold is None else 1)
+                p_, seed_, off_ = S["drop"]
+                ops.layernorm_bwd_lora(da1[:, :D], da1[:, D:D + R_PAD], Lp["at"], q.scaling, p_, seed_, off_, S["x_in"], Lp["n1w"], S["st1"],
+                                       dx, t, P["layers"][li - 1]["g2"], accumulate_dx=True,
+                                       tap=dxcat[:, fold * D:(fold + 1) * D] if fold is not None else None)
+            elif fuse_t1 and li > 0:
                 add_tap(li - 1)
                 ops.layernorm_bwd_scaled(da1[:, :D], S["x_in"], Lp["n1w"], S["st1"], dx, t, P["layers"][li - 1]["g2"],
                                          accumulate_dx=True)
diff --git a/vfmseg_amd/csrc/elementwise.hip b/vfmseg_amd/csrc/elementwise.hip
--- a/vfmseg_amd/csrc/elementwise.hip
+++ b/vfmseg_amd/csrc/elementwise.hip
@@ -3,7 +3,7 @@
 thread_local char g_vfm_err[512] = {0};
 
 extern "C" const char* vfm_last_error(void) { return g_vfm_err; }
-extern "C" int vfm_abi_version(void) { return 4; }
+extern "C" int vfm_abi_version(void) { return 5; }
 extern "C" int vfm_half_kind(void) { return VFM_HALF_KIND; }
 
 template <typename TI, typename TO>
diff --git a/vfmseg_amd/csrc/norm.hip b/vfmseg_amd/csrc/norm.hip
--- a/vfmseg_amd/csrc/norm.hip
+++ b/vfmseg_amd/csrc/norm.hip
@@ -59,13 +59,10 @@
   *reinterpret_cast<ushort4*>(p + so.plane) = hi;
   *reinterpret_cast<ushort4*>(p + 2 * so.plane) = lo;
 }
-template <typename TO, int NV, bool DROP = false, bool SPLIT = false>
-__global__ void k_ln_fwd_v4(const float* __restrict__ x, long ld_x, const float* __restrict__ w, const float* __restrict__ b,
-                            float eps, TO* __restrict__ y, long ld_y, float* __restrict__ stats, long rows, int C, LnDrop dr = LnDrop(),
-                            Split3Out so = Split3Out()) {
-  const int lane = threadIdx.x & 63;
-  const long row = (long)blockIdx.x * (blockDim.x >> 6) + (threadIdx.x >> 6);
-  if (row >= rows) return;
+template <typename TO, int NV, bool DROP, bool SPLIT, bool TILE>
+__device__ __forceinline__ void ln_fwd_row(const float* __restrict__ x, long ld_x, const float* __restrict__ w, const float* __restrict__ b,
+                                           float eps, TO* __restrict__ y, long ld_y, float* __restrict__ stats, const long row, const int lane,
+                                           int C, const LnDrop& dr, const Split3Out& so, bf16_t* tile) {
   const float* xr = x + row * ld_x;
   float4 v[NV];
   float s = 0.f;
@@ -113,14 +110,25 @@
         yd.y = k1 ? f32_to_bf16(bf16_to_f32(p.y) * ksf) : f32_to_bf16(bf16_to_f32(p.y) * 0.f);
         yd.z = k2 ? f32_to_bf16(bf16_to_f32(p.z) * ksf) : f32_to_bf16(bf16_to_f32(p.z) * 0.f);
         yd.w = k3 ? f32_to_bf16(bf16_to_f32(p.w) * ksf) : f32_to_bf16(bf16_to_f32(p.w) * 0.f);
-        *reinterpret_cast<ushort4*>((bf16_t*)dr.mask + row * dr.ld_mask + c0) = mk;
+        if constexpr (!TILE) *reinterpret_cast<ushort4*>((bf16_t*)dr.mask + row * dr.ld_mask + c0) = mk;
         *reinterpret_cast<ushort4*>((bf16_t*)dr.yd + row * dr.ld_yd + c0) = yd;
+        if constexpr (TILE) *reinterpret_cast<ushort4*>(tile + c0) = yd;
       }
     } else {
       if (!SPLIT || y != nullptr) *reinterpret_cast<float4*>(y + row * ld_y + c0) = o;
       if constexpr (SPLIT) store_split4(so, row, c0, o);
     }
   }
+}
+
+template <typename TO, int NV, bool DROP = false, bool SPLIT = false>
+__global__ void k_ln_fwd_v4(const float* __restrict__ x, long ld_x, const float* __restrict__ w, const float* __restrict__ b,
+                            float eps, TO* __restrict__ y, long ld_y, float* __restrict__ stats, long rows, int C, LnDrop dr = LnDrop(),
+                            Split3Out so = Split3Out()) {
+  const int lane = threadIdx.x & 63;
+  const long row = (long)blockIdx.x * (blockDim.x >> 6) + (threadIdx.x >> 6);
+  if (row >= rows) return;
+  ln_fwd_row<TO, NV, DROP, SPLIT, false>(x, ld_x, w, b, eps, y, ld_y, stats, row, lane, C, dr, so, nullptr);
 }
 
 template <typename TD, int NV>
@@ -348,7 +356,7 @@
                                          uint64_t offset, long rows, long C, void* stream) {
   VFM_CHECK(p >= 0.f && p < 1.f, VFM_E_INVAL, "vfm_layernorm_dropout_fwd: p");
   const long nv = C / 256;
-  VFM_CHECK(C % 256 == 0 && (nv == 1 || nv == 2 || nv == 4 || nv == 5 || nv == 8), VFM_E_SHAPE, "vfm_layernorm_dropout_fwd: C=%ld", C);
+  VFM_CHECK(C % 256 == 0 && (nv == 1 || nv == 2 || nv == 3 || nv == 4 || nv == 5 || nv == 8), VFM_E_SHAPE, "vfm_layernorm_dropout_fwd: C=%ld", C);
   VFM_CHECK(ld_x % 4 == 0 && ld_y % 4 == 0 && ld_yd % 4 == 0 && ld_mask % 4 == 0 && (uintptr_t)x % 16 == 0 && (uintptr_t)y % 8 == 0 &&
                 (uintptr_t)y_drop % 8 == 0 && (uintptr_t)mask % 8 == 0 && (uintptr_t)w % 16 == 0 && (uintptr_t)b % 16 == 0,
             VFM_E_ALIGN, "vfm_layernorm_dropout_fwd: alignment");
@@ -357,7 +365,7 @@
   dim3 blk(256), grid(cdiv(rows, 4));
   LnDrop dr{y_drop, ld_yd, mask, ld_mask, p, 1.0f / (1.0f - p), seed, offset};
 #define LVD(NV) hipLaunchKernelGGL((k_ln_fwd_v4<bf16_t, NV, true>), grid, blk, 0, s, x, ld_x, w, b, eps, (bf16_t*)y, ld_y, stats, rows, (int)C, dr)
-  if (nv == 1) LVD(1); else if (nv == 2) LVD(2); else if (nv == 4) LVD(4); else if (nv == 5) LVD(5); else LVD(8);
+  if (nv == 1) LVD(1); else if (nv == 2) LVD(2); else if (nv == 3) LVD(3); else if (nv == 4) LVD(4); else if (nv == 5) LVD(5); else LVD(8);
 #undef LVD
   VFM_LAUNCH_CHECK();
   return VFM_OK;
@@ -583,14 +591,14 @@
   hipStream_t s = (hipStream_t)stream;
   const bool need_w = (dw || db);
   const int nv = (int)(C / 256);
-  const bool v4 = !need_w && (C % 256 == 0) && (nv == 1 || nv == 2 || nv == 4 || nv == 5) && (ld_x % 4 == 0) && (ld_dx % 4 == 0) &&
+  const bool v4 = !need_w && (C % 256 == 0) && (nv == 1 || nv == 2 || (nv == 3 && t_out) || nv == 4 || nv == 5) && (ld_x % 4 == 0) && (ld_dx % 4 == 0) &&
                   (ld_dy % 4 == 0) && ((uintptr_t)x % 16 == 0) && ((uintptr_t)dx % 16 == 0) && ((uintptr_t)dy % 8 == 0) &&
                   ((uintptr_t)w % 16 == 0);
   if (v4) {
     dim3 grid(cdiv(rows, 4)), blk(256);
 #define LV(TD, NV) hipLaunchKernelGGL((k_ln_bwd_v4<TD, NV>), grid, blk, 0, s, (const TD*)dy, ld_dy, x, ld_x, w, stats, dx, ld_dx, accumulate_dx, rows, (int)C, (bf16_t*)t_out, ld_t, t_scale)
-    if (dy_dt == VFM_BF16) { if (nv == 1) LV(bf16_t, 1); else if (nv == 2) LV(bf16_t, 2); else if (nv == 4) LV(bf16_t, 4); else LV(bf16_t, 5); }
-    else if (dy_dt == VFM_F32) { if (nv == 1) LV(float, 1); else if (nv == 2) LV(float, 2); else if (nv == 4) LV(float, 4); else LV(float, 5); }
+    if (dy_dt == VFM_BF16) { if (nv == 1) LV(bf16_t, 1); else if (nv == 2) LV(bf16_t, 2); else if (nv == 3) LV(bf16_t, 3); else if (nv == 4) LV(bf16_t, 4); else LV(bf16_t, 5); }
+    else if (dy_dt == VFM_F32) { if (nv == 1) LV(float, 1); else if (nv == 2) LV(float, 2); else if (nv == 3) LV(float, 3); else if (nv == 4) LV(float, 4); else LV(float, 5); }
     else VFM_FAIL(VFM_E_INVAL, "vfm_layernorm_bwd: dtype");
 #undef LV
     VFM_LAUNCH_CHECK();
@@ -638,6 +646,186 @@
   }
 #undef L
   if (need_w) hipLaunchKernelGGL(k_ln_bwd_fin, dim3(cdiv(C, 64)), dim3(256), 0, s, ws, parts, (int)C, dw, db);
+  VFM_LAUNCH_CHECK();
+  return VFM_OK;
+}
+
+typedef vfm_h h16x8 __attribute__((ext_vector_type(8)));
+typedef float f32x4m __attribute__((ext_vector_type(4)));
+constexpr int LL_ROWS = 16;
+
+__device__ __forceinline__ bool drop_keep(uint64_t seed, uint64_t e, float p) {
+  return (hash_u32(seed, e) >> 8) * (1.0f / 16777216.0f) >= p;
+}
+
+template <int NV>
+__global__ __launch_bounds__(1024) void k_ln_drop_lora_fwd(const float* __restrict__ x, long ld_x, const float* __restrict__ w,
+                                                           const float* __restrict__ b, float eps, bf16_t* __restrict__ y, long ld_y,
+                                                           float* __restrict__ stats, long rows, int C, LnDrop dr, bf16_t* __restrict__ t,
+                                                           long ld_t, const bf16_t* __restrict__ A, long ld_a, float alpha) {
+  constexpr int CC = NV * 256, LDP = CC + 8, KS = 2 * NV;
+  __shared__ __attribute__((aligned(16))) bf16_t sx[LL_ROWS * LDP];
+  __shared__ f32x4m sp[16 * 64];
+  const int lane = threadIdx.x & 63, wv = threadIdx.x >> 6;
+  const long row0 = (long)blockIdx.x * LL_ROWS, row = row0 + wv;
+  const int fr = lane & 15, fq = lane >> 4, ct = wv & 3, k0 = (wv >> 2) * (CC / 4);
+  h16x8 fa[KS];
+  {
+    const bf16_t* ap = A + (long)(ct * 16 + fr) * ld_a + k0 + 8 * fq;
+#pragma unroll
+    for (int j = 0; j < KS; ++j) fa[j] = *reinterpret_cast<const h16x8*>(ap + 32 * j);
+  }
+  if (row < rows) {
+    ln_fwd_row<bf16_t, NV, true, false, true>(x, ld_x, w, b, eps, y, ld_y, stats, row, lane, C, dr, Split3Out(), sx + wv * LDP);
+  } else {
+#pragma unroll
+    for (int i = 0; i < NV; ++i) *reinterpret_cast<ushort4*>(sx + wv * LDP + (i * 64 + lane) * 4) = make_ushort4(0, 0, 0, 0);
+  }
+  __syncthreads();
+  const bf16_t* xp = sx + fr * LDP + k0 + 8 * fq;
+  f32x4m acc0 = {0.f, 0.f, 0.f, 0.f}, acc1 = {0.f, 0.f, 0.f, 0.f};
+#pragma unroll
+  for (int j = 0; j < KS; j += 2) {
+    acc0 = VFM_MFMA16S(*reinterpret_cast<const h16x8*>(xp + 32 * j), fa[j], acc0);
+    acc1 = VFM_MFMA16S(*reinterpret_cast<const h16x8*>(xp + 32 * j + 32), fa[j + 1], acc1);
+  }
+  sp[wv * 64 + lane] = acc0 + acc1;
+  __syncthreads();
+  if (wv < 4) {
+    const f32x4m sum = (sp[wv * 64 + lane] + sp[(4 + wv) * 64 + lane]) + (sp[(8 + wv) * 64 + lane] + sp[(12 + wv) * 64 + lane]);
+#pragma unroll
+    for (int r = 0; r < 4; ++r) {
+      const long orow = row0 + fq * 4 + r;
+      if (orow < rows) t[orow * ld_t + wv * 16 + fr] = f32_to_bf16(alpha * sum[r]);
+    }
+  }
+}
+
+extern "C" int vfm_layernorm_dropout_lora_fwd(const float* x, long ld_x, const float* w, const float* b, float eps, void* y, long ld_y,
+                                              float* stats, void* y_drop, long ld_yd, void* t, long ld_t, const void* a, long ld_a,
+                                              float alpha, float p, uint64_t seed, uint64_t offset, long rows, long C, void* stream) {
+  VFM_CHECK(p >= 0.f && p < 1.f, VFM_E_INVAL, "vfm_layernorm_dropout_lora_fwd: p");
+  const long nv = C / 256;
+  VFM_CHECK(C > 0 && C % 256 == 0 && nv <= 5, VFM_E_SHAPE, "vfm_layernorm_dropout_lora_fwd: C=%ld must be a multiple of 256 up to 1280", C);
+  VFM_CHECK(x && w && b && y && stats && y_drop && t && a && rows >= 0 && ld_x >= C && ld_y >= C && ld_yd >= C && ld_t >= 64 && ld_a >= C,
+            VFM_E_INVAL, "vfm_layernorm_dropout_lora_fwd: null operand or pitch below the row width");
+  VFM_CHECK(ld_x % 4 == 0 && ld_y % 4 == 0 && ld_yd % 4 == 0 && ld_a % 8 == 0 && (uintptr_t)x % 16 == 0 && (uintptr_t)y % 8 == 0 &&
+                (uintptr_t)y_drop % 8 == 0 && (uintptr_t)a % 16 == 0 && (uintptr_t)w % 16 == 0 && (uintptr_t)b % 16 == 0,
+            VFM_E_ALIGN, "vfm_layernorm_dropout_lora_fwd: alignment");
+  if (rows == 0) return VFM_OK;
+  hipStream_t s = (hipStream_t)stream;
+  dim3 blk(1024), grid(cdiv(rows, LL_ROWS));
+  LnDrop dr{y_drop, ld_yd, nullptr, 0, p, 1.0f / (1.0f - p), seed, offset};
+#define LLF(NV) hipLaunchKernelGGL((k_ln_drop_lora_fwd<NV>), grid, blk, 0, s, x, ld_x, w, b, eps, (bf16_t*)y, ld_y, stats, rows, (int)C, dr, (bf16_t*)t, ld_t, (const bf16_t*)a, ld_a, alpha)
+  if (nv == 1) LLF(1); else if (nv == 2) LLF(2); else if (nv == 3) LLF(3); else if (nv == 4) LLF(4); else LLF(5);
+#undef LLF
+  VFM_LAUNCH_CHECK();
+  return VFM_OK;
+}
+
+template <int NV>
+__global__ __launch_bounds__(1024) void k_ln_bwd_lora(const bf16_t* __restrict__ dy, long ld_dy, const bf16_t* __restrict__ dT, long ld_dt,
+                                                      const bf16_t* __restrict__ At, long ld_at, float alpha, float p, float keep_scale,
+                                                      uint64_t seed, uint64_t offset, const float* __restrict__ x, long ld_x,
+                                                      const float* __restrict__ w, const float* __restrict__ stats, float* __restrict__ dx,
+                                                      long ld_dx, int accumulate_dx, const bf16_t* __restrict__ tap, long ld_tap, long tap_rows,
+                                                      bf16_t* __restrict__ t_out, long ld_t, const float* __restrict__ t_scale, long rows, int C) {
+  constexpr int CC = NV * 256, LDL = CC + 4;
+  __shared__ __attribute__((aligned(16))) float sl[LL_ROWS * LDL];
+  const int lane = threadIdx.x & 63, wv = threadIdx.x >> 6;
+  const long row0 = (long)blockIdx.x * LL_ROWS;
+  const bool live = row0 + wv < rows;
+  const long row = live ? row0 + wv : rows - 1;
+  const bool has_tap = tap != nullptr && row < tap_rows;
+  ushort4 pq[NV], tp[NV];
+  float4 xv[NV], od[NV];
+#pragma unroll
+  for (int i = 0; i < NV; ++i) {
+    const int c0 = (i * 64 + lane) * 4;
+    pq[i] = *reinterpret_cast<const ushort4*>(dy + row * ld_dy + c0);
+    xv[i] = *reinterpret_cast<const float4*>(x + row * ld_x + c0);
+    od[i] = accumulate_dx ? *reinterpret_cast<const float4*>(dx + row * ld_dx + c0) : make_float4(0.f, 0.f, 0.f, 0.f);
+    tp[i] = has_tap ? *reinterpret_cast<const ushort4*>(tap + row * ld_tap + c0) : make_ushort4(0, 0, 0, 0);
+  }
+  {
+    const int fr = lane & 15, fq = lane >> 4;
+    long ar = row0 + fr;
+    if (ar >= rows) ar = rows - 1;
+    const bf16_t* ap = dT + ar * ld_dt + 8 * fq;
+    const h16x8 a0 = *reinterpret_cast<const h16x8*>(ap), a1 = *reinterpret_cast<const h16x8*>(ap + 32);
+#pragma unroll
+    for (int nt = 0; nt < NV; ++nt) {
+      const int col = wv * (CC / 16) + nt * 16 + fr;
+      const bf16_t* bp = At + (long)col * ld_at + 8 * fq;
+      f32x4m acc = {0.f, 0.f, 0.f, 0.f};
+      acc = VFM_MFMA16S(a0, *reinterpret_cast<const h16x8*>(bp), acc);
+      acc = VFM_MFMA16S(a1, *reinterpret_cast<const h16x8*>(bp + 32), acc);
+#pragma unroll
+      for (int r = 0; r < 4; ++r) sl[(fq * 4 + r) * LDL + col] = alpha * acc[r];
+    }
+  }
+  __syncthreads();
+  if (!live) return;
+  const float ksf = bf16_to_f32(f32_to_bf16(keep_scale));
+  const float mean = stats[row * 2], rstd = stats[row * 2 + 1];
+  float4 g[NV], xh[NV];
+  float s1 = 0.f, s2 = 0.f;
+#pragma unroll
+  for (int i = 0; i < NV; ++i) {
+    const int c0 = (i * 64 + lane) * 4;
+    const float4 lo = *reinterpret_cast<const float4*>(sl + wv * LDL + c0);
+    const uint64_t e0 = offset + (uint64_t)row * C + c0;
+    const float m0 = drop_keep(seed, e0, p) ? ksf : 0.f, m1 = drop_keep(seed, e0 + 1, p) ? ksf : 0.f;
+    const float m2 = drop_keep(seed, e0 + 2, p) ? ksf : 0.f, m3 = drop_keep(seed, e0 + 3, p) ? ksf : 0.f;
+    const float4 d = make_float4(bf16_to_f32(pq[i].x) + m0 * lo.x, bf16_to_f32(pq[i].y) + m1 * lo.y, bf16_to_f32(pq[i].z) + m2 * lo.z,
+                                 bf16_to_f32(pq[i].w) + m3 * lo.w);
+    const float4 ww = *reinterpret_cast<const float4*>(w + c0);
+    xh[i] = make_float4((xv[i].x - mean) * rstd, (xv[i].y - mean) * rstd, (xv[i].z - mean) * rstd, (xv[i].w - mean) * rstd);
+    g[i] = make_float4(d.x * ww.x, d.y * ww.y, d.z * ww.z, d.w * ww.w);
+    s1 += (g[i].x + g[i].y) + (g[i].z + g[i].w);
+    s2 += (g[i].x * xh[i].x + g[i].y * xh[i].y) + (g[i].z * xh[i].z + g[i].w * xh[i].w);
+  }
+  s1 = wave_sum(s1) / C;
+  s2 = wave_sum(s2) / C;
+#pragma unroll
+  for (int i = 0; i < NV; ++i) {
+    const int c0 = (i * 64 + lane) * 4;
+    float4 o = make_float4(rstd * (g[i].x - s1 - xh[i].x * s2), rstd * (g[i].y - s1 - xh[i].y * s2),
+                           rstd * (g[i].z - s1 - xh[i].z * s2), rstd * (g[i].w - s1 - xh[i].w * s2));
+    if (accumulate_dx) {
+      float4 old = od[i];
+      if (has_tap) old.x += bf16_to_f32(tp[i].x), old.y += bf16_to_f32(tp[i].y), old.z += bf16_to_f32(tp[i].z), old.w += bf16_to_f32(tp[i].w);
+      o.x += old.x, o.y += old.y, o.z += old.z, o.w += old.w;
+    }
+    *reinterpret_cast<float4*>(dx + row * ld_dx + c0) = o;
+    const float4 ts = *reinterpret_cast<const float4*>(t_scale + c0);
+    const ushort4 tv = {f32_to_bf16(o.x * ts.x), f32_to_bf16(o.y * ts.y), f32_to_bf16(o.z * ts.z), f32_to_bf16(o.w * ts.w)};
+    *reinterpret_cast<ushort4*>(t_out + row * ld_t + c0) = tv;
+  }
+}
+
+extern "C" int vfm_layernorm_bwd_lora(const void* dy, long ld_dy, const void* dt, long ld_dt, const void* at, long ld_at, float alpha,
+                                      float p, uint64_t seed, uint64_t offset, const float* x, long ld_x, const float* w,
+                                      const float* stats, float* dx, long ld_dx, int accumulate_dx, const void* tap, long ld_tap,
+                                      long tap_rows, void* t_out, long ld_t, const float* t_scale, long rows, long C, void* stream) {
+  VFM_CHECK(p >= 0.f && p < 1.f, VFM_E_INVAL, "vfm_layernorm_bwd_lora: p");
+  const long nv = C / 256;
+  VFM_CHECK(C > 0 && C % 256 == 0 && nv <= 5, VFM_E_SHAPE, "vfm_layernorm_bwd_lora: C=%ld must be a multiple of 256 up to 1280", C);
+  VFM_CHECK(dy && dt && at && x && w && stats && dx && t_out && t_scale && rows >= 0 && ld_dy >= C && ld_dt >= 64 && ld_at >= 64 &&
+                ld_x >= C && ld_dx >= C && ld_t >= C,
+            VFM_E_INVAL, "vfm_layernorm_bwd_lora: null operand or pitch below the row width");
+  VFM_CHECK(!tap || (accumulate_dx && tap_rows >= 0 && tap_rows <= rows && ld_tap >= C && ld_tap % 4 == 0 && (uintptr_t)tap % 8 == 0),
+            VFM_E_INVAL, "vfm_layernorm_bwd_lora: the tap operand needs accumulate_dx, tap_rows <= rows and 8-byte aligned rows");
+  VFM_CHECK(ld_dy % 4 == 0 && ld_dt % 8 == 0 && ld_at % 8 == 0 && ld_x % 4 == 0 && ld_dx % 4 == 0 && ld_t % 4 == 0 && (uintptr_t)dy % 8 == 0 &&
+                (uintptr_t)dt % 16 == 0 && (uintptr_t)at % 16 == 0 && (uintptr_t)x % 16 == 0 && (uintptr_t)dx % 16 == 0 &&
+                (uintptr_t)w % 16 == 0 && (uintptr_t)t_out % 8 == 0 && (uintptr_t)t_scale % 16 == 0,
+            VFM_E_ALIGN, "vfm_layernorm_bwd_lora: alignment");
+  if (rows == 0) return VFM_OK;
+  hipStream_t s = (hipStream_t)stream;
+  dim3 blk(1024), grid(cdiv(rows, LL_ROWS));
+#define LLB(NV) hipLaunchKernelGGL((k_ln_bwd_lora<NV>), grid, blk, 0, s, (const bf16_t*)dy, ld_dy, (const bf16_t*)dt, ld_dt, (const bf16_t*)at, ld_at, alpha, p, 1.0f / (1.0f - p), seed, offset, x, ld_x, w, stats, dx, ld_dx, accumulate_dx, (const bf16_t*)tap, ld_tap, tap_rows, (bf16_t*)t_out, ld_t, t_scale, rows, (int)C)
+  if (nv == 1) LLB(1); else if (nv == 2) LLB(2); else if (nv == 3) LLB(3); else if (nv == 4) LLB(4); else LLB(5);
+#undef LLB
   VFM_LAUNCH_CHECK();
   return VFM_OK;
 }
diff --git a/vfmseg_amd/csrc/plan.hip b/vfmseg_amd/csrc/plan.hip
--- a/vfmseg_amd/csrc/plan.hip
+++ b/vfmseg_amd/csrc/plan.hip
@@ -52,6 +52,17 @@
       return vfm_strided_copy(a.src, a.src_dt, a.dst, a.dst_dt, a.n[0], a.n[1], a.n[2], a.n[3], a.ss[0], a.ss[1], a.ss[2], a.ss[3], a.ds[0],
                               a.ds[1], a.ds[2], a.ds[3], a.accumulate, s);
     }
+    case VFM_OP_LN_DROPOUT_LORA_FWD: {
+      const auto& a = o.u.ln_lora_fwd;
+      return vfm_layernorm_dropout_lora_fwd(a.x, a.ld_x, a.w, a.b, a.eps, a.y, a.ld_y, a.stats, a.y_drop, a.ld_yd, a.t, a.ld_t, a.a, a.ld_a,
+                                            a.alpha, a.p, seed, rng_base + a.offset, a.rows, a.C, s);
+    }
+    case VFM_OP_LN_BWD_LORA: {
+      const auto& a = o.u.ln_lora_bwd;
+      return vfm_layernorm_bwd_lora(a.dy, a.ld_dy, a.dt, a.ld_dt, a.at, a.ld_at, a.alpha, a.p, seed, rng_base + a.offset, a.x, a.ld_x, a.w,
+                                    a.stats, a.dx, a.ld_dx, a.accumulate_dx, a.tap, a.ld_tap, a.tap_rows, a.t_out, a.ld_t, a.t_scale,
+                                    a.rows, a.C, s);
+    }
     default: VFM_FAIL(VFM_E_INVAL, "vfm_run_plan: unknown op kind %d", o.kind);
   }
 }
diff --git a/vfmseg_amd/lib.py b/vfmseg_amd/lib.py
--- a/vfmseg_amd/lib.py
+++ b/vfmseg_amd/lib.py
@@ -8,7 +8,7 @@
 LIB_PATH_F16 = os.path.join(_HERE, "csrc", "libvfmseg_hip_f16.so")
 
 F32, BF16, U8, I64, SPLIT3 = 0, 1, 2, 3, 4
-ABI_VERSION = 4
+ABI_VERSION = 5
 EP_NONE, EP_GELU, EP_RELU, EP_MUL_GELU_GRAD, EP_MUL, EP_QGELU, EP_MUL_QGELU_GRAD, EP_GELU_DGELU = 0, 1, 2, 3, 4, 5, 6, 7
 ACT_NONE, ACT_GELU, ACT_RELU, ACT_QGELU = 0, 1, 2, 3
 
@@ -71,16 +71,29 @@
     _fields_ = [("src", vp), ("src_dt", ci), ("dst", vp), ("dst_dt", ci), ("n", cl * 4), ("ss", cl * 4), ("ds", cl * 4), ("accumulate", ci)]
 
 
+class _LnLoraFwd(C.Structure):
+    _fields_ = [("x", vp), ("ld_x", cl), ("w", vp), ("b", vp), ("eps", cf), ("y", vp), ("ld_y", cl), ("stats", vp), ("y_drop", vp),
+                ("ld_yd", cl), ("t", vp), ("ld_t", cl), ("a", vp), ("ld_a", cl), ("alpha", cf), ("p", cf), ("offset", u64), ("rows", cl),
+                ("C", cl)]
+
+
+class _LnLoraBwd(C.Structure):
+    _fields_ = [("dy", vp), ("ld_dy", cl), ("dt", vp), ("ld_dt", cl), ("at", vp), ("ld_at", cl), ("alpha", cf), ("p", cf), ("offset", u64),
+                ("x", vp), ("ld_x", cl), ("w", vp), ("stats", vp), ("dx", vp), ("ld_dx", cl), ("accumulate_dx", ci), ("tap", vp),
+                ("ld_tap", cl), ("tap_rows", cl), ("t_out", vp), ("ld_t", cl), ("t_scale", vp), ("rows", cl), ("C", cl)]
+
+
 class _PlanU(C.Union):
     _fields_ = [("gemm", GemmDesc), ("attn", AttnDesc), ("ln_fwd", _LnFwd), ("ln_drop", _LnDrop), ("ln_bwd", _LnBwd), ("cast", _CastOp),
-                ("copy", _CopyOp)]
+                ("copy", _CopyOp), ("ln_lora_fwd", _LnLoraFwd), ("ln_lora_bwd", _LnLoraBwd)]
 
 
 class PlanOp(C.Structure):
     _fields_ = [("kind", ci), ("prof_kind", ci), ("flops", C.c_double), ("u", _PlanU)]
 
 
-OP_GEMM, OP_LN_FWD, OP_LN_DROPOUT_FWD, OP_LN_BWD_SCALED, OP_ATTN_FWD, OP_ATTN_BWD, OP_CAST, OP_STRIDED_COPY = range(8)
+(OP_GEMM, OP_LN_FWD, OP_LN_DROPOUT_FWD, OP_LN_BWD_SCALED, OP_ATTN_FWD, OP_ATTN_BWD, OP_CAST, OP_STRIDED_COPY, OP_LN_DROPOUT_LORA_FWD,
+ OP_LN_BWD_LORA) = range(10)
 PROF_NONE, PROF_GEMM, PROF_GEMM_TN, PROF_ATTN_FWD, PROF_ATTN_BWD = range(5)
 PROF_NAMES = {PROF_GEMM: "gemm", PROF_GEMM_TN: "gemm_tn", PROF_ATTN_FWD: "attn_fwd", PROF_ATTN_BWD: "attn_bwd"}
 
@@ -116,6 +129,8 @@
     "vfm_layernorm_dropout_fwd": [vp, cl, vp, vp, cf, vp, cl, vp, vp, cl, vp, cl, cf, u64, u64, cl, cl, vp],
     "vfm_layernorm_bwd_scaled": [vp, ci, cl, vp, cl, vp, vp, vp, cl, ci, vp, cl, vp, cl, cl, vp],
     "vfm_layernorm_bwd": [vp, ci, cl, vp, cl, vp, vp, vp, cl, ci, vp, vp, vp, cl, cl, vp],
+    "vfm_layernorm_dropout_lora_fwd": [vp, cl, vp, vp, cf, vp, cl, vp, vp, cl, vp, cl, vp, cl, cf, cf, u64, u64, cl, cl, vp],
+    "vfm_layernorm_bwd_lora": [vp, cl, vp, cl, vp, cl, cf, cf, u64, u64, vp, cl, vp, vp, vp, cl, ci, vp, cl, cl, vp, cl, vp, cl, cl, vp],
     "vfm_groupnorm_fwd": [vp, vp, vp, cf, ci, ci, vp, ci, vp, vp, cl, cl, cl, vp],
     "vfm_groupnorm_bwd": [vp, ci, vp, vp, vp, vp, ci, ci, vp, vp, vp, vp, cl, cl, cl, vp],
     "vfm_bn_moments": [vp, cl, cl, vp, vp, vp],
diff --git a/vfmseg_amd/ops.py b/vfmseg_amd/ops.py
--- a/vfmseg_amd/ops.py
+++ b/vfmseg_amd/ops.py
@@ -254,6 +254,39 @@
     L.check(lib.vfm_layernorm_bwd_scaled(L.ptr(dy), L.dt_of(dy), _ld(dy), L.ptr(x), _ld(x), L.ptr(w), L.ptr(stats), L.ptr(dx),
                                          _ld(dx), int(accumulate_dx), L.ptr(t_out), _ld(t_out), L.ptr(t_scale), rows, c,
                                          L.stream()), "vfm_layernorm_bwd_scaled")
+    return dx
+
+
+LORA_LN_WIDTHS = (256, 512, 768, 1024, 1280)
+
+
+def lora_ln_fused():
+    try:
+        v = int(os.environ.get("VFMSEG_LORA_LN_FUSED", "7"))
+    except ValueError:
+        v = 7
+    return v & 7 if v & 2 else v & 1
+
+
+def layernorm_dropout_lora_fwd(x, w, b, eps, y, stats, y_drop, t, a, alpha, p, seed, offset=0):
+    lib = L.load()
+    rows, c = x.shape
+    assert is_half(y.dtype) and is_half(y_drop.dtype) and is_half(t.dtype) and is_half(a.dtype) and t.shape[1] == 64 and a.shape == (64, c)
+    L.check(lib.vfm_layernorm_dropout_lora_fwd(L.ptr(x), _ld(x), L.ptr(w), L.ptr(b), float(eps), L.ptr(y), _ld(y), L.ptr(stats),
+                                               L.ptr(y_drop), _ld(y_drop), L.ptr(t), _ld(t), L.ptr(a), _ld(a), float(alpha), float(p),
+                                               int(seed), int(offset), rows, c, L.stream()), "vfm_layernorm_dropout_lora_fwd")
+    return y
+
+
+def layernorm_bwd_lora(dy, dt, at, alpha, p, seed, offset, x, w, stats, dx, t_out, t_scale, accumulate_dx=False, tap=None):
+    lib = L.load()
+    rows, c = x.shape
+    assert is_half(dy.dtype) and is_half(dt.dtype) and is_half(at.dtype) and is_half(t_out.dtype) and t_scale.dtype == torch.float32
+    assert dt.shape[1] == 64 and at.shape == (c, 64) and (tap is None or (is_half(tap.dtype) and tap.shape[1] == c))
+    L.check(lib.vfm_layernorm_bwd_lora(L.ptr(dy), _ld(dy), L.ptr(dt), _ld(dt), L.ptr(at), _ld(at), float(alpha), float(p), int(seed),
+                                       int(offset), L.ptr(x), _ld(x), L.ptr(w), L.ptr(stats), L.ptr(dx), _ld(dx), int(accumulate_dx),
+                                       L.ptr(tap), _ld(tap) if tap is not None else 0, tap.shape[0] if tap is not None else 0,
+                                       L.ptr(t_out), _ld(t_out), L.ptr(t_scale), rows, c, L.stream()), "vfm_layernorm_bwd_lora")
     return dx
 
 
@@ -467,6 +500,29 @@
         u.rows, u.C = x.shape
         return len(self.ops) - 1
 
+    def layernorm_dropout_lora_fwd(self, x, w, b, eps, y, stats, y_drop, t, a, alpha, p, offset):
+        assert is_half(y.dtype) and is_half(y_drop.dtype) and is_half(t.dtype) and is_half(a.dtype) and t.shape[1] == 64
+        op = self._new(L.OP_LN_DROPOUT_LORA_FWD, L.PROF_NONE, 0.0, x, w, b, y, stats, y_drop, t, a)
+        u = op.u.ln_lora_fwd
+        u.x, u.ld_x, u.w, u.b, u.eps, u.y, u.ld_y, u.stats = L.ptr(x), _ld(x), L.ptr(w), L.ptr(b), float(eps), L.ptr(y), _ld(y), L.ptr(stats)
+        u.y_drop, u.ld_yd, u.t, u.ld_t, u.a, u.ld_a = L.ptr(y_drop), _ld(y_drop), L.ptr(t), _ld(t), L.ptr(a), _ld(a)
+        u.alpha, u.p, u.offset = float(alpha), float(p), int(offset)
+        u.rows, u.C = x.shape
+        return len(self.ops) - 1
+
+    def layernorm_bwd_lora(self, dy, dt, at, alpha, p, offset, x, w, stats, dx, t_out, t_scale, accumulate_dx=False, tap=None):
+        assert is_half(dy.dtype) and is_half(dt.dtype) and is_half(at.dtype) and is_half(t_out.dtype) and t_scale.dtype == torch.float32
+        op = self._new(L.OP_LN_BWD_LORA, L.PROF_NONE, 0.0, dy, dt, at, x, w, stats, dx, t_out, t_scale, tap)
+        u = op.u.ln_lora_bwd
+        u.dy, u.ld_dy, u.dt, u.ld_dt, u.at, u.ld_at = L.ptr(dy), _ld(dy), L.ptr(dt), _ld(dt), L.ptr(at), _ld(at)
+        u.alpha, u.p, u.offset = float(alpha), float(p), int(offset)
+        u.x, u.ld_x, u.w, u.stats, u.dx, u.ld_dx, u.accumulate_dx = L.ptr(x), _ld(x), L.ptr(w), L.ptr(stats), L.ptr(dx), _ld(dx), int(accumulate_dx)
+        if tap is not None:
+            u.tap, u.ld_tap, u.tap_rows = L.ptr(tap), _ld(tap), tap.shape[0]
+        u.t_out, u.ld_t, u.t_scale = L.ptr(t_out), _ld(t_out), L.ptr(t_scale)
+        u.rows, u.C = x.shape
+        return len(self.ops) - 1
+
     def attn_fwd(self, q, k, v, o, lse, B, H, d, nq_main, nq_extra, nk_main, nk_extra, scale):
         fl = 4.0 * B * H * (nq_main + nq_extra) * (nk_main + nk_extra) * d
         op = self._new(L.OP_ATTN_FWD, L.PROF_ATTN_FWD if is_half(q.dtype) else L.PROF_NONE, fl, q, k, v, o, lse)
```

Result: no change. 129.7 images/s, median of 6 (+0.9%).
